# AIML-IfI/openset-imagenet

Hardware: AMD Instinct MI355X
Metric: images/sec (whole node) ResNet-50 + entropic-open-set, Protocol 2, 1/2/4/8 GPUs (higher is better)
Workload: dtype f32; 1 GPU; Protocol 2, ResNet-50, entropic open-set loss, batch 128/GPU; workload_key=p2, classes=30, batch_per_gpu=128, global_batch=128, image=3x224x224, loss=entropic, optimizer=adam lr=1e-3, parallelism=dp1

## Files before the change

__graft_entry__.py:

```python
import os
import subprocess
import sys

ROOT = os.path.dirname(os.path.abspath(__file__))
PKG = os.path.join(ROOT, "openset-imagenet_amd")
CSRC = os.path.join(PKG, "csrc")
for p in (ROOT, PKG):
    if p not in sys.path:
        sys.path.insert(0, p)


def build():
    subprocess.run(["make", "-C", CSRC, "-j8"], check=True)
    import openset_imagenet
    from openset_imagenet import _native
    lib = _native.lib()
    assert lib.osi_build_arch() == b"gfx950"
    assert lib.osi_abi_version() >= 7
    ops = _native.ops()
    assert hasattr(ops, "resnet50_forward") and hasattr(ops, "loss_fwd_bwd") and hasattr(ops, "adam_step") and hasattr(ops, "resnet50_grads_ready")
    assert hasattr(lib, "osi_conv_fwd_epilogue") and hasattr(lib, "osi_bn_eval_coeffs_multi")
    assert hasattr(ops, "resnet50_backward_adv") and hasattr(ops, "grad_accumulate") and hasattr(lib, "osi_stem_dgrad_fgsm")
    assert hasattr(ops, "adam_step_groups") and hasattr(ops, "sgd_step_groups") and hasattr(lib, "osi_adam_step_groups")
    assert hasattr(ops, "resnet50_forward_frozen") and hasattr(lib, "osi_conv_dgrad_fused_frozen") and hasattr(lib, "osi_bn_backward_frozen")
    assert lib.osi_abi_version() >= 13 and hasattr(lib, "osi_resnet50_set_trainable") and hasattr(lib, "osi_resnet50_tensor_unit")
    assert lib.osi_abi_version() >= 16 and hasattr(lib, "osi_auc_binary_f32") and hasattr(lib, "osi_auc_ovr_f32")
    assert lib.osi_abi_version() >= 17 and hasattr(lib, "osi_grad_clip_scale") and hasattr(ops, "grad_clip_scale")
    assert hasattr(ops, "adam_step_groups_dev") and hasattr(ops, "sgd_step_groups_dev")
    assert lib.osi_abi_version() >= 18 and hasattr(lib, "osi_eval_values_f32") and hasattr(lib, "osi_hist_f32")
    assert lib.osi_abi_version() >= 19 and hasattr(lib, "osi_stem_dgrad_pgd") and hasattr(ops, "resnet50_backward_attack")
    assert lib.osi_abi_version() >= 20 and hasattr(lib, "osi_average_update") and hasattr(lib, "osi_resnet50_set_bn_momentum")
    assert hasattr(ops, "average_update") and hasattr(ops, "resnet50_set_bn_momentum")
    assert lib.osi_abi_version() >= 21 and hasattr(lib, "osi_openmax_fit_tails") and hasattr(ops, "openmax_recalibrate")
    assert lib.osi_abi_version() >= 22 and hasattr(lib, "osi_evm_distances") and hasattr(ops, "evm_probs")
    assert lib.osi_abi_version() >= 23 and hasattr(lib, "osi_mix_rows_pairs") and hasattr(ops, "proser_loss_fwd_bwd")
    assert lib.osi_abi_version() >= 24 and hasattr(lib, "osi_knn_topk") and hasattr(ops, "knn_class_kth")
    assert lib.osi_abi_version() >= 25 and hasattr(lib, "osi_maha_scatter") and hasattr(ops, "maha_factor")
    assert lib.osi_abi_version() >= 26 and hasattr(lib, "osi_eigh_sweep") and hasattr(ops, "vim_scores")
    assert lib.osi_abi_version() >= 27 and hasattr(lib, "osi_shape_rows") and hasattr(ops, "order_stats") and hasattr(ops, "resnet50_pooled")


def smoke():
    import torch
    from openset_imagenet import ResNet50, EntropicOpensetLoss, optim, tools
    from oracle import resnet50_oracle as R, losses_oracle as L
    tools.set_device_gpu(0)
    torch.manual_seed(0)
    B, HW, C = 8, 96, 10
    model = tools.device(ResNet50(C, C, False))
    sd = {k: v.detach().cpu().clone() for k, v in model.state_dict().items()}
    x = torch.rand(B, 3, HW, HW)
    y = torch.tensor([0, -1, 3, 9, -1, 5, 2, 7])
    opt = optim.Adam(model.parameters(), lr=1e-3)
    model.train()
    opt.zero_grad()
    logits, feats = model(tools.device(x))
    j = EntropicOpensetLoss(C, 1.0)(logits, tools.device(y))
    j.backward()
    ref_logits, ref_feats, ref_loss, _ = R.forward_backward({k: v.clone() for k, v in sd.items()}, x, y,
                                                            lambda lg, t, f: L.entropic_openset_loss(lg, t, 1.0))
    sys.path.insert(0, os.path.join(ROOT, "tests"))
    from osi_testlib import hip_gates
    gates = hip_gates(model)
    sd64 = {k: (v.double() if v.is_floating_point() else v.clone()) for k, v in sd.items()}
    _, _, _, g64 = R.forward_backward(sd64, x.double(), y, lambda lg, t, f: L.entropic_openset_loss(lg, t, 1.0), gates=gates)
    opt.step()
    torch.cuda.synchronize()
    err = float((logits.detach().cpu() - ref_logits).abs().max())
    lerr = abs(float(j.detach()) - float(ref_loss))
    named = dict(model.named_parameters())
    gerr = max(float((named[k].grad.cpu().double() - g).norm() / (g.norm() + 1e-30)) for k, g in g64.items())
    print(f"smoke: max|dlogit|={err:.2e} |dloss|={lerr:.2e} max rel-L2 gradient error over {len(g64)} tensors (pinned gates)={gerr:.2e}")
    assert err < 1e-4 and lerr < 1e-4 and gerr < 5e-4, "HIP path disagrees with the CPU oracle"
    sd2 = {k: v.detach().cpu().clone() for k, v in model.state_dict().items()}
    model.eval()
    with torch.no_grad():
        lg_e, _ = model(tools.device(x))
    ref_e, _ = R.forward({k: (v.double() if v.is_floating_point() else v.clone()) for k, v in sd2.items()}, x.double(), False)
    eerr = float((lg_e.cpu().double() - ref_e).abs().max())
    print(f"smoke: inference forward max|dlogit|={eerr:.2e} (|logit| <= {float(ref_e.abs().max()):.2f})")
    assert eerr < 1e-4 * max(1.0, float(ref_e.abs().max())), "inference forward disagrees with the CPU oracle"


if __name__ == "__main__":
    build()
    print("build ok")
```

include/osi.h:

```cpp
#ifndef OSI_H
#define OSI_H

#include <stddef.h>

#ifdef __cplusplus
extern "C" {
#endif

#define OSI_OK 0
#define OSI_ERR_ARG (-1)
#define OSI_ERR_LAUNCH (-2)
#define OSI_ERR_STATE (-3)

typedef void* osi_stream_t;

int osi_abi_version(void);
const char* osi_build_arch(void);
const char* osi_strerror(int code);
int osi_set_tuning(const char* name, int value);
int osi_get_tuning(const char* name, int* value);
int osi_tuning_info(int i, const char** name, int* def, int* lo, int* hi, int* plan_relevant);

typedef struct {
    int B, H, W, Cin;
    int Ho, Wo, Cout;
    int R, S, stride, pad;
} osi_conv_desc;

enum { OSI_TILE_AUTO = 0, OSI_TILE_128x128 = 1, OSI_TILE_128x64 = 2, OSI_TILE_64x128 = 3, OSI_TILE_64x64 = 4,
       OSI_TILE_64x64_S1 = 5, OSI_TILE_64x128_S1 = 6, OSI_TILE_128x128_S1 = 7, OSI_TILE_128x64_S1 = 8  };

int osi_conv_fwd(const osi_conv_desc* d, const float* x, const float* w, float* y, int tile, osi_stream_t stream);
size_t osi_conv_fwd_bnstats_workspace(const osi_conv_desc* d);
int osi_conv_fwd_bnstats(const osi_conv_desc* d, const float* x, const float* w, float* y, int tile, float* pstats,
                         size_t pstats_bytes, int* P, int* rows_per_block, osi_stream_t stream);
int osi_conv_fwd_act(const osi_conv_desc* d, const float* x, const float* in_scale, const float* in_shift, const float* w, float* y,
                     int tile, float* pstats, size_t pstats_bytes, int* P, int* rows_per_block, osi_stream_t stream);
int osi_conv_fwd_act2(const osi_conv_desc* d, const float* x, const float* in_scale, const float* in_shift, const float* res,
                      const float* w, float* y, int tile, float* pstats, size_t pstats_bytes, int* P, int* rows_per_block,
                      osi_stream_t stream);
int osi_conv_wino_eligible(const osi_conv_desc* d, int input_gradient);
size_t osi_conv_wino_workspace(const osi_conv_desc* d);
size_t osi_conv_wino_weights_bytes(const osi_conv_desc* d);
size_t osi_conv_wino_slab_bytes(void);
int osi_conv_wino_transform_weights(const osi_conv_desc* d, const float* w, int input_gradient, float* u, size_t u_bytes, osi_stream_t stream);
int osi_conv_fwd_wino_pre(const osi_conv_desc* d, const float* x, const float* in_scale, const float* in_shift, const float* u, float* y,
                          void* slab, size_t slab_bytes, float* pstats, size_t pstats_bytes, int* P, int* rows_per_block, osi_stream_t stream);
int osi_conv_fwd_wino(const osi_conv_desc* d, const float* x, const float* in_scale, const float* in_shift, const float* w, float* y,
                      void* ws, size_t ws_bytes, float* pstats, size_t pstats_bytes, int* P, int* rows_per_block, osi_stream_t stream);
typedef struct {
    const float* scale;
    const float* shift;
    const float* residual;
    int relu;
} osi_conv_epilogue;
size_t osi_conv_fwd_epilogue_workspace(const osi_conv_desc* d);
int osi_conv_fwd_epilogue(const osi_conv_desc* d, const float* x, const float* w, float* out, const osi_conv_epilogue* e, void* ws,
                          size_t ws_bytes, osi_stream_t stream);
int osi_conv_fwd_wino_epilogue_pre(const osi_conv_desc* d, const float* x, const float* u, float* out, const osi_conv_epilogue* e, void* slab,
                                   size_t slab_bytes, osi_stream_t stream);
int osi_conv_dgrad(const osi_conv_desc* d, const float* dy, const float* w, float* dx, int accumulate, int tile,
                   osi_stream_t stream);
typedef struct {
    const void* relu_mask;
    const float* y0;
    const float* mean0;
    const float* invstd0;
    const float* y1;
    const float* mean1;
    const float* invstd1;
    float* partials;
    size_t partials_bytes;
    const float* scale0;
    const float* shift0;
    const void* pool_idx;
    int pool_H, pool_W;
    int addend_stride;
} osi_dgrad_fusion;
size_t osi_conv_dgrad_fused_workspace(const osi_conv_desc* d);
int osi_conv_dgrad_fused(const osi_conv_desc* d, const float* dy, const float* w, float* dx, const float* addend,
                         const osi_dgrad_fusion* f, int tile, int* P, osi_stream_t stream);
int osi_conv_dgrad_fused_frozen(const osi_conv_desc* d, const float* dy, const float* w, float* dx, const osi_dgrad_fusion* f, int tile,
                                int* P, osi_stream_t stream);
int osi_conv_dgrad_fused_wino(const osi_conv_desc* d, const float* dy, const float* w, float* dx, const osi_dgrad_fusion* f, void* ws,
                              size_t ws_bytes, int* P, osi_stream_t stream);
int osi_conv_dgrad_fused_wino_pre(const osi_conv_desc* d, const float* dy, const float* u, float* dx, const osi_dgrad_fusion* f, void* slab,
                                  size_t slab_bytes, int* P, osi_stream_t stream);
size_t osi_conv_wgrad_workspace(const osi_conv_desc* d);
int osi_conv_wgrad(const osi_conv_desc* d, const float* dy, const float* x, float* dw, void* ws, size_t ws_bytes,
                   osi_stream_t stream);
int osi_conv_wgrad_act(const osi_conv_desc* d, const float* dy, const float* x, const float* in_scale, const float* in_shift, float* dw,
                       void* ws, size_t ws_bytes, osi_stream_t stream);
size_t osi_conv_wgrad_wino_workspace(const osi_conv_desc* d);
int osi_conv_wgrad_wino(const osi_conv_desc* d, const float* dy, const float* x, const float* in_scale, const float* in_shift, float* dw,
                        void* ws, size_t ws_bytes, osi_stream_t stream);
int osi_stem_weight_pack(const float* w_krsc3, float* w_packed, int Cout, osi_stream_t stream);
size_t osi_stem_wgrad_direct_workspace(const osi_conv_desc* d);
int osi_stem_wgrad_direct(const osi_conv_desc* d, const float* dy, const float* x4, float* dw_krsc3, void* ws, size_t ws_bytes,
                          osi_stream_t stream);
size_t osi_stem_wgrad_fused_workspace(const osi_conv_desc* d);
int osi_stem_wgrad_fused(const osi_conv_desc* d, const float* gpool, const void* pool_idx, const float* y, const float* x4,
                         const float* gamma, const float* mean, const float* invstd, const float* dgamma, const float* dbeta,
                         float* dw_krsc3, void* ws, size_t ws_bytes, osi_stream_t stream);
int osi_stem_grad_unpack(const float* g_packed, float* g_krsc3, int Cout, osi_stream_t stream);
int osi_stem_dgrad(const float* dy, const float* w_krsc3, float* dx_nchw, int B, int H, int W, osi_stream_t stream);
int osi_stem_dgrad_fgsm(const float* dy, const float* w_krsc3, const float* x_nhwc4, float* x_adv_nhwc4, float eps, float lo, float hi,
                        int B, int H, int W, osi_stream_t stream);
int osi_stem_dgrad_pgd(const float* dy, const float* w_krsc3, const float* x_cur_nhwc4, const float* x_anchor_nhwc4, float* x_next_nhwc4,
                       float alpha, float eps, float lo, float hi, int B, int H, int W, osi_stream_t stream);

size_t osi_bn_workspace(int M, int C);
int osi_bn_train_stats(const float* y, int M, int C, const float* gamma, const float* beta, float eps, float momentum,
                       float* running_mean, float* running_var, float* mean, float* invstd, float* scale, float* shift,
                       void* ws, size_t ws_bytes, osi_stream_t stream);
int osi_bn_finalize_stats(float* pstats, size_t pstats_bytes, int P, int rows_per_block, int M, int C, const float* gamma,
                          const float* beta, float eps, float momentum, float* running_mean, float* running_var, float* mean,
                          float* invstd, float* scale, float* shift, osi_stream_t stream);
int osi_bn_eval_coeffs(const float* running_mean, const float* running_var, const float* gamma, const float* beta, float eps,
                       int C, float* scale, float* shift, osi_stream_t stream);
#define OSI_BN_MULTI_MAX 64
typedef struct {
    const float *running_mean, *running_var, *gamma, *beta;
    float *scale, *shift;
    int C;
} osi_bn_eval_layer;
int osi_bn_eval_coeffs_multi(const osi_bn_eval_layer* layers, int n, float eps, osi_stream_t stream);
#define OSI_BN_FROZEN_MAX 54
typedef struct {
    const float *running_mean, *running_var, *gamma, *beta;
    float *scale, *shift, *mean, *invstd;
    int C;
} osi_bn_frozen_layer;
int osi_bn_frozen_coeffs_multi(const osi_bn_frozen_layer* layers, int n, float eps, osi_stream_t stream);
int osi_bn_apply(const float* y, const float* residual, const float* scale, const float* shift, float* out, int M, int C,
                 int relu, osi_stream_t stream);
size_t osi_bn_backward_workspace(int M, int C);
int osi_bn_backward(const float* dout, const float* act, const float* y, const float* mean, const float* invstd,
                    const float* gamma, float* dy, float* gmasked, float* dgamma, float* dbeta, int M, int C, void* ws,
                    size_t ws_bytes, osi_stream_t stream);

size_t osi_bn_relu_mask_bytes(int M, int C);
int osi_bn_apply_relu_mask(const float* y, const float* residual, const float* scale, const float* shift, float* out,
                           void* relu_mask, int M, int C, osi_stream_t stream);
int osi_bn_apply_relu_mask2(const float* y, const float* scale, const float* shift, const float* res_y, const float* res_scale,
                            const float* res_shift, float* out, void* relu_mask, int M, int C, osi_stream_t stream);
int osi_bn_backward_relu_mask(const float* dout, const void* relu_mask, const float* y, const float* mean, const float* invstd,
                              const float* gamma, float* dy, float* gmasked, float* dgamma, float* dbeta, int M, int C, void* ws,
                              size_t ws_bytes, osi_stream_t stream);

int osi_bn_backward_fused(const float* g, const float* y, const float* mean, const float* invstd, const float* gamma,
                          const float* psum_g, const float* psum_gx, int P, float* dy, float* dgamma, float* dbeta, int M, int C,
                          void* ws, size_t ws_bytes, osi_stream_t stream);

typedef struct {
    const float *y, *mean, *invstd, *gamma;
    const float* psum_gx;
    float* dy;
    float *dgamma, *dbeta;
} osi_bn_fused_consumer;
size_t osi_bn_backward_fused2_workspace(int C);
int osi_bn_backward_fused2(const float* g, const osi_bn_fused_consumer* consumers, const float* psum_g, int P, int M, int C, void* ws,
                           size_t ws_bytes, osi_stream_t stream);

typedef struct {
    const float *y, *mean, *invstd;
    const float* scale;
    float* dy;
    float *dgamma, *dbeta;
} osi_bn_frozen_consumer;
int osi_bn_backward_frozen(const float* dout, const void* relu_mask, const osi_bn_frozen_consumer* consumers, int n, float* gmasked, int M,
                           int C, void* ws, size_t ws_bytes, osi_stream_t stream);

int osi_nchw3_to_nhwc4(const float* x_nchw, float* y_nhwc4, int B, int H, int W, osi_stream_t stream);
int osi_u8hwc3_to_nhwc4(const unsigned char* x_u8_nhwc, const unsigned char* flip, float* y_nhwc4, int B, int H, int W,
                        osi_stream_t stream);
// ... 275 lines not shown
```

openset-imagenet_amd/csrc/abi.hip:

```cpp
#include "osi_common.h"

#include <cstring>

OsiTuning g_osi_tuning;

namespace {
struct Knob { const char* name; int OsiTuning::*slot; int def, lo, hi, plan; };
const Knob kKnobs[] = {
#define OSI_KNOB_ROW(name, def, lo, hi, plan) {#name, &OsiTuning::name, def, lo, hi, plan},
    OSI_TUNING_KNOBS(OSI_KNOB_ROW)
#undef OSI_KNOB_ROW
};
const int kNumKnobs = (int)(sizeof(kKnobs) / sizeof(kKnobs[0]));
const Knob* find_knob(const char* name) {
    if (!name) return nullptr;
    for (const Knob& k : kKnobs)
        if (!strcmp(name, k.name)) return &k;
    return nullptr;
}
}

extern "C" {
int osi_abi_version(void) { return 27; }
int osi_set_tuning(const char* name, int value) {
    const Knob* k = find_knob(name);
    if (!k) return OSI_ERR_ARG;
    if (value < k->lo || value > k->hi) return OSI_ERR_ARG;
    if (k->slot == &OsiTuning::wgrad_tile && value != 0 && value != 64) return OSI_ERR_ARG;
    g_osi_tuning.*(k->slot) = value;
    return OSI_OK;
}
int osi_get_tuning(const char* name, int* value) {
    const Knob* k = find_knob(name);
    if (!k || !value) return OSI_ERR_ARG;
    *value = g_osi_tuning.*(k->slot);
    return OSI_OK;
}
int osi_tuning_info(int i, const char** name, int* def, int* lo, int* hi, int* plan_relevant) {
    if (i < 0 || i >= kNumKnobs) return OSI_ERR_ARG;
    const Knob& k = kKnobs[i];
    if (name) *name = k.name;
    if (def) *def = k.def;
    if (lo) *lo = k.lo;
    if (hi) *hi = k.hi;
    if (plan_relevant) *plan_relevant = k.plan;
    return OSI_OK;
}
const char* osi_build_arch(void) { return "gfx950"; }
const char* osi_strerror(int code) {
    switch (code) {
        case OSI_OK: return "ok";
        case OSI_ERR_ARG: return "invalid argument (shape, pointer or alignment precondition)";
        case OSI_ERR_LAUNCH: return "HIP launch failed";
        case OSI_ERR_STATE: return "executor called out of order, or a plan-relevant tuning knob changed after osi_resnet50_create";
        default: return "unknown error";
    }
}
}
```

openset-imagenet_amd/csrc/bn.hip:

```cpp
#include "osi_common.h"

namespace {

constexpr int NT = 256;

struct RowSplit { int CV, RL, G; };
__host__ __device__ inline RowSplit row_split(int C) {
    RowSplit s;
    int c4 = C / 4;
    s.CV = c4 < NT ? c4 : NT;
    s.RL = NT / s.CV;
    s.G = (c4 + s.CV - 1) / s.CV;
    return s;
}

__global__ __launch_bounds__(NT) void k_bn_stats_partial(const float* __restrict__ y, int M, int C, int rows_per_blk,
                                                        float* __restrict__ pmean, float* __restrict__ pm2) {
    const int P = gridDim.x;
    __shared__ f32x4 red[2][NT];
    const RowSplit sp = row_split(C);
    const int tid = threadIdx.x;
    const int cv = tid % sp.CV, rl = tid / sp.CV;
    const int r0 = blockIdx.x * rows_per_blk;
    const int r1 = min(M, r0 + rows_per_blk);
    const float n = (float)(r1 - r0);
    const bool active = rl < sp.RL;
    for (int g = 0; g < sp.G; ++g) {
        const int c4 = g * sp.CV + cv;
        const bool colok = active && c4 * 4 < C;
        f32x4 s1 = {0, 0, 0, 0}, s2 = {0, 0, 0, 0}, shift = {0, 0, 0, 0};
        if (colok) {
            const f32x4* base = reinterpret_cast<const f32x4*>(y) + c4;
            const size_t ld = C / 4;
            shift = base[(size_t)r0 * ld];
            int r = r0 + rl;
            for (; r + 3 * sp.RL < r1; r += 4 * sp.RL) {
                f32x4 v0 = base[(size_t)r * ld], v1 = base[(size_t)(r + sp.RL) * ld];
                f32x4 v2 = base[(size_t)(r + 2 * sp.RL) * ld], v3 = base[(size_t)(r + 3 * sp.RL) * ld];
                v0 -= shift; v1 -= shift; v2 -= shift; v3 -= shift;
                s1 += (v0 + v1) + (v2 + v3);
                s2 += (v0 * v0 + v1 * v1) + (v2 * v2 + v3 * v3);
            }
            for (; r < r1; r += sp.RL) {
                f32x4 v = base[(size_t)r * ld] - shift;
                s1 += v; s2 += v * v;
            }
        }
        red[0][tid] = s1; red[1][tid] = s2;
        __syncthreads();
        if (colok && rl == 0) {
            for (int k = 1; k < sp.RL; ++k) { s1 += red[0][k * sp.CV + cv]; s2 += red[1][k * sp.CV + cv]; }
            f32x4 mean = shift + s1 / n;
            f32x4 m2 = s2 - s1 * s1 / n;
#pragma unroll
            for (int k = 0; k < 4; ++k) {
                pmean[(size_t)(c4 * 4 + k) * P + blockIdx.x] = mean[k];
                pm2[(size_t)(c4 * 4 + k) * P + blockIdx.x] = m2[k];
            }
        }
        __syncthreads();
    }
}

__device__ __forceinline__ void bn_finish(int c, float mean, float m2, int M, const float* gamma, const float* beta, float eps,
                                          float momentum, float* running_mean, float* running_var, float* mean_out,
                                          float* invstd_out, float* scale_out, float* shift_out) {
    float var = m2 / (float)M;
    float invstd = 1.0f / sqrtf(var + eps);
    mean_out[c] = mean; invstd_out[c] = invstd;
    float sc = invstd * gamma[c];
    scale_out[c] = sc; shift_out[c] = beta[c] - mean * sc;
    if (running_mean) {
        float unb = M > 1 ? m2 / (float)(M - 1) : var;
        running_mean[c] = (1.f - momentum) * running_mean[c] + momentum * mean;
        running_var[c] = (1.f - momentum) * running_var[c] + momentum * unb;
    }
}
__global__ __launch_bounds__(NT) void k_bn_stats_final_rows(const float* __restrict__ pmean, const float* __restrict__ pm2, int P,
                                                           int rows_per_blk, int M, int C, const float* __restrict__ gamma,
                                                           const float* __restrict__ beta, float eps, float momentum,
                                                           float* running_mean, float* running_var, float* __restrict__ mean_out,
                                                           float* __restrict__ invstd_out, float* __restrict__ scale_out,
                                                           float* __restrict__ shift_out) {
// ... 418 lines not shown
    }
}

struct BwdCoef { f32x4 mu, is, c1, c2, gis; };
__device__ __forceinline__ BwdCoef bwd_coef(const f32x4* __restrict__ mean, const f32x4* __restrict__ invstd, const f32x4* __restrict__ gamma,
                                            const f32x4* __restrict__ c1, const f32x4* __restrict__ c2, int c4) {
    BwdCoef k;
    k.mu = mean[c4]; k.is = invstd[c4]; k.c1 = c1[c4]; k.c2 = c2[c4];
    k.gis = gamma[c4] * k.is;
    return k;
}
__device__ __forceinline__ f32x4 bwd_elem(f32x4 gv, f32x4 yv, const BwdCoef& k) {
    const f32x4 xh = (yv - k.mu) * k.is;
    return (gv - k.c1 - xh * k.c2) * k.gis;
}
template <int MODE, bool EMITG, int GEO>
__global__ __launch_bounds__(NT) void k_bn_bwd_apply(const f32x4* dA , const void* __restrict__ msk,
                                                    const f32x4* __restrict__ y, const f32x4* __restrict__ mean,
                                                    const f32x4* __restrict__ invstd, const f32x4* __restrict__ gamma,
                                                    const f32x4* __restrict__ c1, const f32x4* __restrict__ c2,
                                                    f32x4* dy, f32x4* __restrict__ gout, size_t n4, int c4n, PoolSrc ps) {
    const size_t nq = (n4 + NT - 1) / NT;
    const int tid = threadIdx.x;
    BwdCoef k0 = {}, k1 = {};
    if (GEO == 1) k0 = bwd_coef(mean, invstd, gamma, c1, c2, tid % c4n);
    if (GEO == 2) { k0 = bwd_coef(mean, invstd, gamma, c1, c2, tid); k1 = bwd_coef(mean, invstd, gamma, c1, c2, NT + tid); }
    for (size_t q = blockIdx.x; q < nq; q += gridDim.x) {
        const size_t t = (OSI_BN_REVERSE & 2) ? nq - 1 - q : q;
        const size_t i = t * NT + tid;
        if (i >= n4) continue;
        const int c4 = GEO == 1 ? tid % c4n : GEO == 2 ? (int)(t & 1) * NT + tid : (int)(i % (size_t)c4n);
        f32x4 gv = MODE == 3 ? pool_gather(dA, ps, (uint32_t)(i / (size_t)c4n), c4, c4n) : masked<MODE>(__builtin_nontemporal_load(dA + i), msk, i);
        const BwdCoef k = GEO == 1 ? k0 : GEO == 2 ? ((t & 1) ? k1 : k0) : bwd_coef(mean, invstd, gamma, c1, c2, c4);
        f32x4 r = bwd_elem(gv, __builtin_nontemporal_load(y + i), k);
        if (EMITG) gout[i] = gv;
        dy[i] = r;
    }
}

struct BwdApplyCons { const f32x4 *y, *mean, *invstd, *gamma, *c1, *c2; f32x4* dy; };
template <int GEO>
__global__ __launch_bounds__(NT) void k_bn_bwd_apply2(const f32x4* g, BwdApplyCons a, BwdApplyCons b, size_t n4, int c4n) {
    const size_t nq = (n4 + NT - 1) / NT;
    const int tid = threadIdx.x;
    const size_t tfirst = (OSI_BN_REVERSE & 2) ? nq - 1 - blockIdx.x : blockIdx.x;
    const int ck = GEO == 1 ? tid % c4n : (int)(tfirst & 1) * NT + tid;
    BwdCoef a0 = {}, b0 = {};
    if (GEO != 0) { a0 = bwd_coef(a.mean, a.invstd, a.gamma, a.c1, a.c2, ck); b0 = bwd_coef(b.mean, b.invstd, b.gamma, b.c1, b.c2, ck); }
    for (size_t q = blockIdx.x; q < nq; q += gridDim.x) {
        const size_t t = (OSI_BN_REVERSE & 2) ? nq - 1 - q : q;
        const size_t i = t * NT + tid;
        if (i >= n4) continue;
        const f32x4 gv = __builtin_nontemporal_load(g + i);
        const f32x4 ya = __builtin_nontemporal_load(a.y + i), yb = __builtin_nontemporal_load(b.y + i);
        const BwdCoef ka = GEO != 0 ? a0 : bwd_coef(a.mean, a.invstd, a.gamma, a.c1, a.c2, (int)(i % (size_t)c4n));
        const BwdCoef kb = GEO != 0 ? b0 : bwd_coef(b.mean, b.invstd, b.gamma, b.c1, b.c2, (int)(i % (size_t)c4n));
        const f32x4 ra = bwd_elem(gv, ya, ka), rb = bwd_elem(gv, yb, kb);
        b.dy[i] = rb;
        a.dy[i] = ra;
    }
}

template <int MODE, bool EMITG, bool TWO, int GEO>
__global__ __launch_bounds__(NT) void k_bn_frozen_apply(const f32x4* dA, const void* __restrict__ msk, const f32x4* __restrict__ scale0,
                                                       const f32x4* __restrict__ scale1, f32x4* dy0, f32x4* __restrict__ dy1,
                                                       f32x4* __restrict__ gout, size_t n4, int c4n, PoolSrc ps) {
    const size_t nq = (n4 + NT - 1) / NT;
    const int tid = threadIdx.x;
    f32x4 s00 = {}, s01 = {}, s10 = {}, s11 = {};
    if (GEO == 1) { s00 = scale0[tid % c4n]; if (TWO) s10 = scale1[tid % c4n]; }
    if (GEO == 2) { s00 = scale0[tid]; s01 = scale0[NT + tid]; if (TWO) { s10 = scale1[tid]; s11 = scale1[NT + tid]; } }
    for (size_t q = blockIdx.x; q < nq; q += gridDim.x) {
        const size_t t = (OSI_BN_REVERSE & 2) ? nq - 1 - q : q;
        const size_t i = t * NT + tid;
        if (i >= n4) continue;
        const int c4 = GEO == 1 ? tid % c4n : GEO == 2 ? (int)(t & 1) * NT + tid : (int)(i % (size_t)c4n);
        const f32x4 gv = MODE == 3 ? pool_gather(dA, ps, (uint32_t)(i / (size_t)c4n), c4, c4n) : masked<MODE>(__builtin_nontemporal_load(dA + i), msk, i);
        if (EMITG) gout[i] = gv;
        if (TWO) dy1[i] = gv * (GEO == 1 ? s10 : GEO == 2 ? ((t & 1) ? s11 : s10) : scale1[c4]);
        dy0[i] = gv * (GEO == 1 ? s00 : GEO == 2 ? ((t & 1) ? s01 : s00) : scale0[c4]);
    }
}

static int stream_geo(int c4n) { return NT % c4n == 0 ? 1 : c4n == 2 * NT ? 2 : 0; }

static int rows_per_block(int M, int C, int& P) {
    long rows = (256l * 1024) / ((long)C * 4);
    if (rows < 8) rows = 8;
    long minrows = (M + 1023) / 1024;
    if (rows < minrows) rows = minrows;
    if (rows > M) rows = M;
    P = (int)((M + rows - 1) / rows);
    return (int)rows;
}
static int stream_grid(size_t n4, bool backward = false) {
    const size_t cap = (size_t)(backward ? g_osi_tuning.bn_grid_bwd : g_osi_tuning.bn_grid);
    size_t g = (n4 + NT - 1) / NT;
    return (int)(g > cap ? cap : g);
}

static void bwd_groups(int P, int& S, int& Pc) {
    S = osi_cdiv(P, 64);
    if (S > OSI_BN_GROUPS) S = OSI_BN_GROUPS;
    Pc = osi_cdiv(P, S);
    S = osi_cdiv(P, Pc);
}
struct BwdWs { float *a, *b, *c1, *c2; };
static size_t ws_floats(int rows, int C, bool coef = true) { return (size_t)2 * rows * C + (coef ? 2 * (size_t)C : 0); }
static BwdWs carve_ws(void* ws, int rows, int C) {
    float* a = (float*)ws;
    const size_t n = (size_t)rows * C;
    return BwdWs{a, a + n, a + 2 * n, a + 2 * n + C};
}
static PoolSrc make_pool_src(const void* idx, int H, int W) {
    PoolSrc ps;
    ps.idx = (const uint32_t*)idx;
    ps.dW = make_fastdiv((uint32_t)W); ps.dH = make_fastdiv((uint32_t)H);
    ps.H = H; ps.W = W; ps.Ho = (H + 2 - 3) / 2 + 1; ps.Wo = (W + 2 - 3) / 2 + 1;
    return ps;
}

}

extern "C" {

size_t osi_bn_workspace(int M, int C) {
    if (M <= 0 || C <= 0) return 0;
    int P;
    rows_per_block(M, C, P);
    return ws_floats(P, C, false) * sizeof(float);
}

int osi_bn_train_stats(const float* y, int M, int C, const float* gamma, const float* beta, float eps, float momentum,
                       float* running_mean, float* running_var, float* mean, float* invstd, float* scale, float* shift,
                       void* ws, size_t ws_bytes, osi_stream_t stream) {
    OSI_REQUIRE(y && gamma && beta && mean && invstd && scale && shift && ws);
    OSI_REQUIRE(M > 0 && C > 0 && C % 4 == 0);
    OSI_REQUIRE((running_mean == nullptr) == (running_var == nullptr));
    int P;
    int rpb = rows_per_block(M, C, P);
    OSI_REQUIRE(ws_bytes >= ws_floats(P, C, false) * sizeof(float));
    hipStream_t st = (hipStream_t)stream;
    float* pmean = (float*)ws;
    float* pm2 = pmean + (size_t)P * C;
    hipLaunchKernelGGL(k_bn_stats_partial, dim3(P), dim3(NT), 0, st, y, M, C, rpb, pmean, pm2);
    OSI_LAUNCH_CHECK();
    hipLaunchKernelGGL(k_bn_stats_final, dim3(osi_cdiv(C, NT / 64)), dim3(NT), 0, st, pmean, pm2, P, rpb, M, C, gamma, beta, eps,
                       momentum, running_mean, running_var, mean, invstd, scale, shift);
    OSI_LAUNCH_CHECK();
    return OSI_OK;
}

int osi_bn_finalize_stats(float* pstats, size_t pstats_bytes, int P, int rows_per_block, int M, int C, const float* gamma,
                          const float* beta, float eps, float momentum, float* running_mean, float* running_var, float* mean,
                          float* invstd, float* scale, float* shift, osi_stream_t stream) {
    OSI_REQUIRE(pstats && gamma && beta && mean && invstd && scale && shift);
    OSI_REQUIRE(P > 0 && rows_per_block > 0 && M > 0 && C > 0 && (long)(P - 1) * rows_per_block < M && (long)P * rows_per_block >= M);
    OSI_REQUIRE((running_mean == nullptr) == (running_var == nullptr));
    OSI_REQUIRE(pstats_bytes >= bn_pstats_floats(P, C) * sizeof(float));
    hipStream_t st = (hipStream_t)stream;
    const float* pmean = pstats;
    const float* pm2 = pstats + (size_t)P * C;
    if (P <= g_osi_tuning.bn_single_p) {
        hipLaunchKernelGGL(k_bn_stats_final_rows, dim3(osi_cdiv(C, 16)), dim3(NT), 0, st, pmean, pm2, P, rows_per_block, M, C, gamma,
                           beta, eps, momentum, running_mean, running_var, mean, invstd, scale, shift);
        OSI_LAUNCH_CHECK();
// ... 106 lines not shown
    OSI_REQUIRE(relu_mask && res_y && res_scale && res_shift);
    return bn_apply_impl(y, res_y, scale, shift, out, relu_mask, M, C, 1, (hipStream_t)stream, res_scale, res_shift);
}

static BwdConsTable one_cons(const float* pa, const float* pb, float* ga, float* gb, float* dgamma, float* dbeta, float* c1, float* c2) {
    BwdConsTable t{};
    t.k[0] = BwdCons{pa, pb, ga, gb, dgamma, dbeta, c1, c2};
    return t;
}

static int launch_bwd_partial(int mode, const float* dout, const void* msk, const float* y, const float* mean, const float* invstd, float* dgamma,
                              float* dbeta, int M, int C, int rpb, int P, const BwdWs& w, const PoolSrc& ps, hipStream_t st) {
    if (int e = pick<0, 1, 2, 3>(mode, [&](auto MODE) -> int {
            hipLaunchKernelGGL(k_bn_bwd_partial<decltype(MODE)::value>, dim3(P), dim3(NT), 0, st, dout, msk, y, mean, invstd, M, C, rpb, w.a, w.b, ps);
            OSI_LAUNCH_CHECK();
            return OSI_OK;
        })) return e;
    hipLaunchKernelGGL(k_bn_bwd_final, dim3(osi_cdiv(C, NT / 64)), dim3(NT), 0, st, one_cons(w.a, w.b, nullptr, nullptr, dgamma, dbeta, w.c1, w.c2), false, P, M, C);
    OSI_LAUNCH_CHECK();
    return OSI_OK;
}
static int launch_bwd_apply(int mode, const float* dout, const void* msk, const float* y, const float* mean, const float* invstd, const float* gamma,
                            const BwdWs& w, float* dy, float* gmasked, int M, int C, const PoolSrc& ps, hipStream_t st) {
    const size_t n4 = (size_t)M * C / 4;
    const int grid = stream_grid(n4, true), c4n = C / 4;
    auto go = [&](auto MODE, auto EMITG, auto GEO) -> int {
        constexpr int md = decltype(MODE)::value, geo = decltype(GEO)::value;
        constexpr bool emit = decltype(EMITG)::value != 0;
        if constexpr (md != 3 || (geo == 0 && !emit)) {
            hipLaunchKernelGGL((k_bn_bwd_apply<md, emit, geo>), dim3(grid), dim3(NT), 0, st, (const f32x4*)dout, msk, (const f32x4*)y, (const f32x4*)mean,
                               (const f32x4*)invstd, (const f32x4*)gamma, (const f32x4*)w.c1, (const f32x4*)w.c2, (f32x4*)dy, (f32x4*)gmasked, n4, c4n, ps);
            OSI_LAUNCH_CHECK();
            return OSI_OK;
        } else return OSI_ERR_ARG;
    };
    return pick<0, 1, 2, 3>(mode, [&](auto MODE) {
        return pick<0, 1>(gmasked && mode != 3, [&](auto EMITG) {
            return pick<0, 1, 2>(mode == 3 ? 0 : stream_geo(c4n), [&](auto GEO) { return go(MODE, EMITG, GEO); });
        });
    });
}

static int bn_backward_impl(const float* dout, const void* msk, int mode, const float* y, const float* mean, const float* invstd,
                            const float* gamma, float* dy, float* gmasked, float* dgamma, float* dbeta, int M, int C, void* ws,
                            size_t ws_bytes, hipStream_t st, PoolSrc ps = PoolSrc{}) {
    OSI_REQUIRE(dout && y && mean && invstd && gamma && (dy || mode == 3) && dgamma && dbeta && ws);
    OSI_REQUIRE(M > 0 && C > 0 && C % 4 == 0);
    int P;
    const int rpb = rows_per_block(M, C, P);
    OSI_REQUIRE(ws_bytes >= ws_floats(P, C) * sizeof(float));
    const BwdWs w = carve_ws(ws, P, C);
    if (int e = launch_bwd_partial(mode, dout, msk, y, mean, invstd, dgamma, dbeta, M, C, rpb, P, w, ps, st)) return e;
    if (!dy) return OSI_OK;
    return launch_bwd_apply(mode, dout, msk, y, mean, invstd, gamma, w, dy, gmasked, M, C, ps, st);
}

static int bwd_reduce_partials(const BwdConsTable& t, int n, int P, int M, int C, int S, int Pc, hipStream_t st) {
    if (P <= g_osi_tuning.bn_wide_p) {
        hipLaunchKernelGGL(k_bn_bwd_final_wide, dim3(osi_cdiv(C, 16), n), dim3(16 * WPL), 0, st, t, P, M, C);
        OSI_LAUNCH_CHECK();
        return OSI_OK;
    }
    hipLaunchKernelGGL(k_colsum2_group, dim3(osi_cdiv(C, 16), S, n), dim3(NT), 0, st, t, P, Pc, C, S);
    OSI_LAUNCH_CHECK();
    hipLaunchKernelGGL(k_bn_bwd_final, dim3(osi_cdiv(C, NT / 64), n), dim3(NT), 0, st, t, true, S, M, C);
    OSI_LAUNCH_CHECK();
    return OSI_OK;
}

int osi_bn_backward_fused(const float* g, const float* y, const float* mean, const float* invstd, const float* gamma,
                          const float* psum_g, const float* psum_gx, int P, float* dy, float* dgamma, float* dbeta, int M, int C,
                          void* ws, size_t ws_bytes, osi_stream_t stream) {
    OSI_REQUIRE(g && y && mean && invstd && gamma && psum_g && psum_gx && dy && dgamma && dbeta && ws);
    OSI_REQUIRE(M > 0 && C > 0 && C % 4 == 0 && P > 0);
    int S, Pc;
    bwd_groups(P, S, Pc);
    OSI_REQUIRE(ws_bytes >= ws_floats(S, C) * sizeof(float));
    hipStream_t st = (hipStream_t)stream;
    const BwdWs w = carve_ws(ws, S, C);
    if (int e = bwd_reduce_partials(one_cons(psum_g, psum_gx, w.a, w.b, dgamma, dbeta, w.c1, w.c2), 1, P, M, C, S, Pc, st)) return e;
    return launch_bwd_apply(0, g, nullptr, y, mean, invstd, gamma, w, dy, nullptr, M, C, PoolSrc{}, st);
}

size_t osi_bn_backward_fused2_workspace(int C) {
    if (C <= 0) return 0;
    return 2 * ws_floats(OSI_BN_GROUPS, C) * sizeof(float);
}

int osi_bn_backward_fused2(const float* g, const osi_bn_fused_consumer* consumers, const float* psum_g, int P, int M, int C, void* ws,
                           size_t ws_bytes, osi_stream_t stream) {
    OSI_REQUIRE(g && consumers && psum_g && ws && M > 0 && C > 0 && C % 4 == 0 && P > 0);
    for (int k = 0; k < 2; ++k) {
        const osi_bn_fused_consumer& c = consumers[k];
        OSI_REQUIRE(c.y && c.mean && c.invstd && c.gamma && c.psum_gx && c.dy && c.dgamma && c.dbeta);
    }
    OSI_REQUIRE(consumers[1].dy != consumers[0].dy && consumers[1].dy != g);
    OSI_REQUIRE(ws_bytes >= osi_bn_backward_fused2_workspace(C));
    int S, Pc;
    bwd_groups(P, S, Pc);
    hipStream_t st = (hipStream_t)stream;
    const size_t per = ws_floats(OSI_BN_GROUPS, C);
    BwdConsTable t{};
    BwdApplyCons a[2];
    for (int k = 0; k < 2; ++k) {
        const osi_bn_fused_consumer& c = consumers[k];
        const BwdWs w = carve_ws((float*)ws + k * per, S, C);
        t.k[k] = BwdCons{psum_g, c.psum_gx, w.a, w.b, c.dgamma, c.dbeta, w.c1, w.c2};
        a[k] = BwdApplyCons{(const f32x4*)c.y, (const f32x4*)c.mean, (const f32x4*)c.invstd, (const f32x4*)c.gamma, (const f32x4*)w.c1,
                            (const f32x4*)w.c2, (f32x4*)c.dy};
    }
    if (int e = bwd_reduce_partials(t, 2, P, M, C, S, Pc, st)) return e;
    const size_t n4 = (size_t)M * C / 4;
    const int c4n = C / 4;
    const int grid = stream_grid(n4, true);
    int geo = stream_geo(c4n);
    if (geo == 2 && (grid & 1) && (size_t)grid < (n4 + NT - 1) / NT) geo = 0;
    return pick<0, 1, 2>(geo, [&](auto GEO) -> int {
        hipLaunchKernelGGL((k_bn_bwd_apply2<decltype(GEO)::value>), dim3(grid), dim3(NT), 0, st, (const f32x4*)g, a[0], a[1], n4, c4n);
        OSI_LAUNCH_CHECK();
        return OSI_OK;
    });
}

int osi_bn_backward_reduce(const float* psum_g, const float* psum_gx, int P, float* dgamma, float* dbeta, int M, int C, void* ws,
                           size_t ws_bytes, osi_stream_t stream) {
    OSI_REQUIRE(psum_g && psum_gx && dgamma && dbeta && ws && M > 0 && C > 0 && P > 0);
    int S, Pc;
    bwd_groups(P, S, Pc);
    OSI_REQUIRE(ws_bytes >= ws_floats(S, C) * sizeof(float));
    const BwdWs w = carve_ws(ws, S, C);
    return bwd_reduce_partials(one_cons(psum_g, psum_gx, w.a, w.b, dgamma, dbeta, w.c1, w.c2), 1, P, M, C, S, Pc, (hipStream_t)stream);
}

static int bn_frozen_impl(const float* dout, const void* msk, int mode, const osi_bn_frozen_consumer* cs, int n, float* gmasked, int M, int C,
                          void* ws, size_t ws_bytes, hipStream_t st, PoolSrc ps = PoolSrc{}) {
    OSI_REQUIRE(dout && cs && (n == 1 || n == 2) && M > 0 && C > 0 && C % 4 == 0);
    OSI_REQUIRE(mode != 3 || (n == 1 && !gmasked));
    for (int k = 0; k < n; ++k) {
        OSI_REQUIRE(cs[k].scale && cs[k].dy && (cs[k].dgamma == nullptr) == (cs[k].dbeta == nullptr));
        if (cs[k].dgamma) {
            int P;
            rows_per_block(M, C, P);
            OSI_REQUIRE(cs[k].y && cs[k].mean && cs[k].invstd && ws && ws_bytes >= ws_floats(P, C) * sizeof(float));
        }
    }
    OSI_REQUIRE(n == 1 || (cs[1].dy != cs[0].dy && cs[1].dy != dout));
    for (int k = 0; k < n; ++k) {
        if (!cs[k].dgamma) continue;
        int P;
        const int rpb = rows_per_block(M, C, P);
        if (int e = launch_bwd_partial(mode, dout, msk, cs[k].y, cs[k].mean, cs[k].invstd, cs[k].dgamma, cs[k].dbeta, M, C, rpb, P, carve_ws(ws, P, C),
                                       ps, st)) return e;
    }
    const size_t n4 = (size_t)M * C / 4;
    const int grid = stream_grid(n4, true), c4n = C / 4;
    auto D = (const f32x4*)dout; auto S0 = (const f32x4*)cs[0].scale; auto S1 = (const f32x4*)(n == 2 ? cs[1].scale : nullptr);
    auto DY0 = (f32x4*)cs[0].dy; auto DY1 = (f32x4*)(n == 2 ? cs[1].dy : nullptr); auto GO = (f32x4*)gmasked;
    auto go = [&](auto MODE, auto EMITG, auto TWO, auto GEO) -> int {
        constexpr int md = decltype(MODE)::value, geo = decltype(GEO)::value;
        constexpr bool emit = decltype(EMITG)::value != 0, two = decltype(TWO)::value != 0;
        if constexpr (md != 3 || (geo == 0 && !emit && !two)) {
            hipLaunchKernelGGL((k_bn_frozen_apply<md, emit, two, geo>), dim3(grid), dim3(NT), 0, st, D, msk, S0, S1, DY0, DY1, GO, n4, c4n, ps);
            OSI_LAUNCH_CHECK();
            return OSI_OK;
        } else return OSI_ERR_ARG;
    };
// ... 54 lines not shown
```

openset-imagenet_amd/csrc/conv_common.h:

```cpp
#pragma once
#include "osi_common.h"

namespace osi_conv {

__device__ __forceinline__ f32x4 ld4(const float* p) { return *reinterpret_cast<const f32x4*>(p); }

constexpr uint32_t OOB = 0x80000000u;
__device__ __forceinline__ __amdgpu_buffer_rsrc_t make_rsrc(const float* p, int bytes) {
    return __builtin_amdgcn_make_buffer_rsrc((void*)p, 0, bytes, 0x00020000);
}
__device__ __forceinline__ f32x4 bld4(__amdgpu_buffer_rsrc_t r, uint32_t voff, uint32_t soff) {
    return __builtin_bit_cast(f32x4, __builtin_amdgcn_raw_buffer_load_b128(r, voff, soff, 0));
}
typedef uint32_t u32x4 __attribute__((ext_vector_type(4)));
__device__ __forceinline__ u32x4 bld4u(__amdgpu_buffer_rsrc_t r, uint32_t voff, uint32_t soff) {
    return __builtin_bit_cast(u32x4, __builtin_amdgcn_raw_buffer_load_b128(r, voff, soff, 0));
}
__device__ __forceinline__ void bst4(__amdgpu_buffer_rsrc_t r, f32x4 v, uint32_t voff, uint32_t soff) {
    __builtin_amdgcn_raw_buffer_store_b128(__builtin_bit_cast(u32x4, v), r, voff, soff, 0);
}
typedef float f32x3 __attribute__((ext_vector_type(3)));
typedef float f32x4acc __attribute__((ext_vector_type(4)));
__device__ __forceinline__ f32x3 bld3(__amdgpu_buffer_rsrc_t r, uint32_t voff, uint32_t soff) {
    return __builtin_bit_cast(f32x3, __builtin_amdgcn_raw_buffer_load_b96(r, voff, soff, 0));
}

__device__ __forceinline__ int acc_row(int r, int lane) { return (r & 3) + 8 * (r >> 2) + 4 * (lane >> 5); }


int hw_cus();
int chip_cus();
bool conv_desc_ok(const osi_conv_desc* d);
bool conv_is_stem(const osi_conv_desc* d);
int launch_slab_reduce(const float* slab, float* out, size_t n4, size_t stride4, int splits, hipStream_t st);
bool stem_direct_geometry(const osi_conv_desc* d);
int launch_stem_fwd_direct(const osi_conv_desc* d, const float* x4, const float* wpacked, float* y, float* pmean, float* pm2, int ntiles,
                           hipStream_t st);
constexpr int STEM_TILE_PIXELS = 128;

}
```

openset-imagenet_amd/csrc/conv_igemm.hip:

```cpp
#include "conv_common.h"
#include <algorithm>
#include <type_traits>

using namespace osi_conv;

namespace {

constexpr int BK = 32;
constexpr int LDR = BK + 4;

struct ConvP {
    const float* x;
    const float* w;
    float* y;
    int B, H, W, Cin, Ho, Wo, Cout, R, S, stride, pad;
    int M;
    int Ktot;
    int MT, NT;
    int accumulate;
    int x_bytes, w_bytes;
    FastDiv dHoWo, dWo;
    FastDiv cHW[4], cW[4];
    int unit;
    float* pmean;
    float* pm2;
    const float* addend;
    const unsigned long long* ebits;
    const float* ey0;
    const float* ey1;
    const float *emean0, *einv0, *emean1, *einv1;
    const float *escale0, *eshift0;
    int skip_empty;
    int eadd_even;
    const uint32_t* epool;
    int epH, epW;
    float* esum;
    int eP;
    int kchunk;
    int wtbl;
    int wgroup, splits;
    int gkind, gkeys, ginner;
    const float* in_scale;
    const float* in_shift;
    const float* res;
    const float* osc;
    const float* osh;
    const float* ores;
    int orelu;
    size_t slab_stride;
    int MT1, g1, ks_S, ks_T;
    float* ks_slab;
#ifdef OSI_STAMPS
    unsigned long long* stamps;
#endif
};

#ifdef OSI_STAMPS
#define OSI_STAMP(p, idx, slot)                                                                                        \
    do {                                                                                                               \
        if (threadIdx.x == 0 && (p).stamps) (p).stamps[(size_t)(idx) * 8 + (slot)] = __builtin_amdgcn_s_memrealtime(); \
    } while (0)
#define OSI_STAMP_ID(p, idx)                                                                   \
    do {                                                                                       \
        if (threadIdx.x == 0 && (p).stamps) {                                                  \
            (p).stamps[(size_t)(idx) * 8 + 4] = __builtin_amdgcn_s_getreg(63492);   \
            (p).stamps[(size_t)(idx) * 8 + 5] = __builtin_amdgcn_s_getreg(63508);  \
        }                                                                                      \
    } while (0)
unsigned long long* g_osi_stamps = nullptr;
#else
#define OSI_STAMP(p, idx, slot) do {} while (0)
#define OSI_STAMP_ID(p, idx) do {} while (0)
#endif

__device__ __forceinline__ bool tile_of_block(int bid, int MT, int NT, int& mt, int& nt) {
    int xcd = bid & 7, slot = bid >> 3;
    nt = slot % NT;
    mt = (slot / NT) * 8 + xcd;
    return mt < MT;
}

__device__ __forceinline__ bool tile_of_block_split(const ConvP& p, int bid, int& mt, int& nt, int& ks) {
    ks = -1;
    if (p.ks_S <= 1) return tile_of_block(bid, p.MT, p.NT, mt, nt);
    if (bid < p.g1) return tile_of_block(bid, p.MT1, p.NT, mt, nt);
    const int pb = bid - p.g1;
    const int xcd = pb & 7, slot = pb >> 3;
    nt = slot % p.NT;
    const int key = (slot / p.NT) * 8 + xcd;
    const int mt2 = key / p.ks_S;
    ks = key - mt2 * p.ks_S;
    mt = p.MT1 + mt2;
    return mt < p.MT;
}

#ifndef OSI_ABLATE
#define OSI_ABLATE 0
#endif

template <int WM, int WN, int J0 = 0, int J1 = 4>
__device__ __forceinline__ void mma_RR(const float* sA, const float* sB, int arow, int brow, int lane,
                                       f32x16 (&acc)[WM][WN]) {
    const int h4 = (lane >> 5) * 4, l31 = lane & 31;
#pragma unroll
    for (int j = J0; j < J1; ++j) {
        f32x4 a[WM], b[WN];
#pragma unroll
        for (int i = 0; i < WM; ++i) a[i] = *reinterpret_cast<const f32x4*>(sA + (arow + i * 32 + l31) * LDR + 8 * j + h4);
#pragma unroll
        for (int i = 0; i < WN; ++i) b[i] = *reinterpret_cast<const f32x4*>(sB + (brow + i * 32 + l31) * LDR + 8 * j + h4);
#pragma unroll
        for (int e = 0; e < 4; ++e)
#pragma unroll
            for (int i = 0; i < WM; ++i)
#pragma unroll
                for (int n = 0; n < WN; ++n)
                    acc[i][n] = __builtin_amdgcn_mfma_f32_32x32x2f32(a[i][e], b[n][e], acc[i][n], 0, 0, 0);
    }
}
template <int WM, int WN, int LDC>
__device__ __forceinline__ void mma_RC(const float* sA, const float* sB, int arow, int bcol, int lane,
                                       f32x16 (&acc)[WM][WN]) {
    const int h4 = (lane >> 5) * 4, l31 = lane & 31;
#pragma unroll
    for (int j = 0; j < 4; ++j) {
        f32x4 a[WM];
#pragma unroll
        for (int i = 0; i < WM; ++i) a[i] = *reinterpret_cast<const f32x4*>(sA + (arow + i * 32 + l31) * LDR + 8 * j + h4);
#pragma unroll
        for (int e = 0; e < 4; ++e) {
            float b[WN];
#pragma unroll
            for (int n = 0; n < WN; ++n) b[n] = sB[(8 * j + h4 + e) * LDC + bcol + n * 32 + l31];
#pragma unroll
            for (int i = 0; i < WM; ++i)
#pragma unroll
                for (int n = 0; n < WN; ++n)
                    acc[i][n] = __builtin_amdgcn_mfma_f32_32x32x2f32(a[i][e], b[n], acc[i][n], 0, 0, 0);
        }
    }
}
template <int WM, int WN, int LDA, int LDB, int K0 = 0, int K1 = BK / 2>
__device__ __forceinline__ void mma_CC(const float* sA, const float* sB, int acol, int bcol, int lane,
                                       f32x16 (&acc)[WM][WN]) {
    static_assert(WM <= 2 && WN <= 2 && LDA % 2 == 0 && LDB % 2 == 0, "interleaved pairs");
    const int h = lane >> 5, l31 = lane & 31;
    const float* pa = sA + h * LDA + acol + (WM == 2 ? 2 * l31 : l31);
    const float* pb = sB + h * LDB + bcol + (WN == 2 ? 2 * l31 : l31);
#pragma unroll
    for (int ks = K0; ks < K1; ++ks) {
        float a[WM], b[WN];
        if constexpr (WM == 2) { const f32x2 v = *reinterpret_cast<const f32x2*>(pa + 2 * ks * LDA); a[0] = v[0]; a[1] = v[1]; }
        else a[0] = pa[2 * ks * LDA];
        if constexpr (WN == 2) { const f32x2 v = *reinterpret_cast<const f32x2*>(pb + 2 * ks * LDB); b[0] = v[0]; b[1] = v[1]; }
        else b[0] = pb[2 * ks * LDB];
#pragma unroll
        for (int i = 0; i < WM; ++i)
#pragma unroll
            for (int n = 0; n < WN; ++n)
                acc[i][n] = __builtin_amdgcn_mfma_f32_32x32x2f32(a[i], b[n], acc[i][n], 0, 0, 0);
    }
}

constexpr int LDT = 64 + 4;

template <bool LIVE = false>
__device__ __forceinline__ void tile64_to_lds(float* tile, const f32x16& acc, int wm, int wn, int lane, int m0 = 0, int M = 0) {
#pragma unroll
    for (int rr = 0; rr < 16; ++rr) {
        const bool live = !LIVE || m0 + wm * 32 + acc_row(rr, lane) < M;
        tile[(wm * 32 + acc_row(rr, lane)) * LDT + wn * 32 + (lane & 31)] = live ? acc[rr] : 0.f;
    }
}
__device__ __forceinline__ void tile64_to_slab(const ConvP& p, const float* tile, int mt, int nt, int ks) {
    float* dst = p.ks_slab + ((size_t)((mt - p.MT1) * p.NT + nt) * p.ks_S + ks) * 4096;
    const int tid = threadIdx.x, c4 = tid & 15, rg = tid >> 4;
#pragma unroll
    for (int k = 0; k < 4; ++k) {
        const int rl = rg + 16 * k;
        *reinterpret_cast<f32x4*>(dst + rl * 64 + c4 * 4) = *reinterpret_cast<const f32x4*>(tile + rl * LDT + c4 * 4);
    }
}
template <typename RD>
__device__ __forceinline__ void fwd_store64(const ConvP& p, int m0, int n0, bool oe, RD rd) {
    const int tid = threadIdx.x, c4 = tid & 15, rg = tid >> 4;
    float* const y = p.y + n0 + c4 * 4;
    if (oe) {
        const __amdgpu_buffer_rsrc_t ro = make_rsrc(p.ores ? p.ores : p.y, p.ores ? p.M * p.Cout * 4 : 0);
        const f32x4 sc = ld4(p.osc + n0 + c4 * 4), sh = ld4(p.osh + n0 + c4 * 4);
        f32x4 rv[4];
#pragma unroll
        for (int k = 0; k < 4; ++k) {
            const int m = m0 + rg + 16 * k;
            rv[k] = bld4(ro, m < p.M ? (uint32_t)((m * p.Cout + n0 + c4 * 4) * 4) : OOB, 0);
        }
#pragma unroll
        for (int k = 0; k < 4; ++k) {
            const int rl = rg + 16 * k, m = m0 + rl;
            const f32x4 a = rd(rl, c4);
            f32x4 v;
#pragma unroll
            for (int e = 0; e < 4; ++e) { const float t = __builtin_fmaf(a[e], sc[e], sh[e]) + rv[k][e]; v[e] = p.orelu ? osi_relu(t) : t; }
            if (m < p.M) *reinterpret_cast<f32x4*>(y + (size_t)m * p.Cout) = v;
        }
    } else {
#pragma unroll
        for (int k = 0; k < 4; ++k) {
            const int rl = rg + 16 * k, m = m0 + rl;
            if (m < p.M) *reinterpret_cast<f32x4*>(y + (size_t)m * p.Cout) = rd(rl, c4);
        }
    }
}

struct BnPart { float cnt, mu, q; };
template <bool FULL>
__device__ __forceinline__ BnPart bn_block32(const f32x16& acc, int row0, int M, int lane) {
    const float cnt = FULL ? 32.f : (float)min(32, max(0, M - row0));
    float s = 0.f;
#pragma unroll
    for (int rr = 0; rr < 16; ++rr) s += (FULL || row0 + acc_row(rr, lane) < M) ? acc[rr] : 0.f;
    s += __shfl_xor(s, 32, 64);
    const float mu = cnt > 0.f ? s / cnt : 0.f;
    float q = 0.f;
#pragma unroll
    for (int rr = 0; rr < 16; ++rr) {
        const float dlt = acc[rr] - mu;
        if constexpr (FULL) q = __builtin_fmaf(dlt, dlt, q);
        else q += (row0 + acc_row(rr, lane) < M) ? dlt * dlt : 0.f;
    }
    q += __shfl_xor(q, 32, 64);
    return {cnt, mu, q};
}
__device__ __forceinline__ void bn_put(float* st, int slot, float cnt, float mu, float q) {
    float* dst = st + slot * 3;
    dst[0] = cnt; dst[1] = mu; dst[2] = q;
}
template <int BN>
__device__ __forceinline__ void bn_merge_rows(const ConvP& p, const float* st, int mt, int n0) {
    const int tid = threadIdx.x;
    if (tid < BN) {
        const float* a = st + tid * 3;
        const float* b = st + (BN + tid) * 3;
        float cn = a[0], cm = a[1], cs = a[2];
        chan_merge(cn, cm, cs, b[0], b[1], b[2]);
        p.pmean[(size_t)mt * p.Cout + n0 + tid] = cm;
        p.pm2[(size_t)mt * p.Cout + n0 + tid] = cs;
    }
}

__device__ __forceinline__ void load_in_tables(const ConvP& p, float* s_sc, float* s_sh) {
    const int tid = threadIdx.x;
    for (int c = tid * 4; c < p.Cin; c += 1024) {
        *reinterpret_cast<f32x4*>(s_sc + c) = ld4(p.in_scale + c);
        *reinterpret_cast<f32x4*>(s_sh + c) = ld4(p.in_shift + c);
// ... 369 lines not shown
            s0 += (v * (y0v[k] - mu0)) * is0;
            if constexpr (FUSED == 4) v *= gsc;
            bst4(r_out, v, offb[k], 0);
        }
    } else {
        const __amdgpu_buffer_rsrc_t r_add = make_rsrc(p.addend, (USE_ADD && p.addend) ? FULL : 0);
        const __amdgpu_buffer_rsrc_t r_bits = make_rsrc(reinterpret_cast<const float*>(p.ebits), has_bits ? FULL : 0);
        const __amdgpu_buffer_rsrc_t r_y1 = make_rsrc(p.ey1, has_y1 ? FULL : 0);
#pragma unroll
        for (int k = 0; k < 4; ++k) {
            const int rl = rg + 16 * k;
            f32x4 v = rd(rl, c4);
            const uint32_t apix = (uint32_t)(m0 + rl), ab = fdiv(apix, dHW), arem = apix - ab * dHW.d, ah = fdiv(arem, dW), aw = arem - ah * dW.d;
            const uint32_t aoff = (((ah | aw) & (uint32_t)p.eadd_even) != 0u) ? OOB : offb[k];
            v += bld4(r_add, aoff, 0);
            if constexpr (FUSED && POOL) {
                if (offb[k] != OOB) {
                    const uint32_t pix = pixv[k], off = offb[k] >> 2;
                    const uint32_t bb = fdiv(pix, dHW), rem = pix - bb * dHW.d, ho = fdiv(rem, dW), wo = rem - ho * dW.d;
                    const uint32_t idw = p.epool[off >> 2];
#pragma unroll
                    for (int e = 0; e < 4; ++e) {
                        const uint32_t byte = (idw >> (8 * e)) & 0xffu, t = byte & 0x7fu, r = t / 3u, sx = t - 3u * r;
                        const uint32_t apix = (bb * p.epH + 2u * ho - 1u + r) * p.epW + 2u * wo - 1u + sx;
                        const float gv = (byte & 0x80u) ? v[e] : 0.f;
                        sg[e] += gv;
                        s0[e] += (gv * (p.ey0[(size_t)apix * p.Cin + col + e] - mu0[e])) * is0[e];
                    }
                }
            } else if constexpr (FUSED != 0) {
                const uint32_t i4 = offb[k] >> 4, bit = i4 & 63u;
                const uint32_t boff = offb[k] != OOB ? (i4 >> 6) * 32u + (bit >> 5) * 4u : OOB;
                uint32_t wb[4];
#pragma unroll
                for (int e = 0; e < 4; ++e) wb[e] = __builtin_amdgcn_raw_buffer_load_b32(r_bits, boff, 8 * e, 0);
                const f32x4 y0v = bld4(r_y0, offb[k], 0), y1v = bld4(r_y1, offb[k], 0);
#pragma unroll
                for (int e = 0; e < 4; ++e) {
                    const bool keep = (((wb[e] >> (bit & 31u)) & 1u) != 0) | !has_bits;
                    const bool open = !USE_GATE || (__builtin_fmaf(y0v[e], gsc[e], gsh[e]) > 0.f) | !has_gate;
                    v[e] = (keep & open) ? v[e] : 0.f;
                }
                sg += v;
                s0 += (v * (y0v - mu0)) * is0;
                s1 += v * y1v;
            }
            bst4(r_out, v, offb[k], 0);
            if (FUSED == 1) __builtin_amdgcn_sched_barrier(0);
        }
        if (USE_Y1) {
            const uint32_t cb = (uint32_t)col * 4u;
            const f32x4 mu1 = bld4(make_rsrc(p.emean1, has_y1 ? FULL : 0), cb, 0), is1 = bld4(make_rsrc(p.einv1, has_y1 ? FULL : 0), cb, 0);
            s1 = (s1 - mu1 * sg) * is1;
        }
    }
    if (FUSED && p.esum) {
#pragma unroll
        for (int e = 0; e < 4; ++e) {
            sg[e] += __shfl_xor(sg[e], 16, 64); s0[e] += __shfl_xor(s0[e], 16, 64); s1[e] += __shfl_xor(s1[e], 16, 64);
            sg[e] += __shfl_xor(sg[e], 32, 64); s0[e] += __shfl_xor(s0[e], 32, 64); s1[e] += __shfl_xor(s1[e], 32, 64);
        }
        __syncthreads();
        if (lane < 16) {
#pragma unroll
            for (int e = 0; e < 4; ++e) {
                float* dst = smem + (wave * BN + c4 * 4 + e) * 3;
                dst[0] = sg[e]; dst[1] = s0[e]; dst[2] = s1[e];
            }
        }
        __syncthreads();
        if (tid < BN) {
            float a0 = 0.f, a1 = 0.f, a2 = 0.f;
#pragma unroll
            for (int wv = 0; wv < 4; ++wv) { const float* s = smem + (wv * BN + tid) * 3; a0 += s[0]; a1 += s[1]; a2 += s[2]; }
            const size_t prow = (size_t)(cls * p.MT + mt) * p.Cin + n0 + tid;
            const size_t pstride = (size_t)p.eP * p.Cin;
            p.esum[prow] = a0;
            p.esum[pstride + prow] = a1;
            if (p.ey1) p.esum[2 * pstride + prow] = a2;
        }
    }
}

template <int WM, int WN, int NST, int FUSED, bool KS = false, bool POOL = false, bool W3 = false>
__global__ __launch_bounds__(256, NST == 1 ? (WM * WN >= 4 ? 3 : (WM * WN == 1 ? 8 : 4)) : 2) void k_conv_dgrad(ConvP p, int Hc0, int Wc0) {
    static_assert(!KS || (WM == 1 && WN == 1 && NST == 1), "the K-split tail is built for the single-buffered 64x64 tile");
    static_assert(!W3 || (WM == 1 && WN == 1 && NST == 1 && !POOL), "row windows: the single-buffered 64x64 tile");
    constexpr int BM = 64 * WM, BN = 64 * WN;
    constexpr int AROWS = W3 ? W3_WROWS : BM;
    constexpr int AR = W3 ? 3 : BM / 32;
    constexpr int LDC = BN + 4;
    constexpr int BV = BN / 4;
    constexpr int BRP = 256 / BV;
    constexpr int BRN = BK / BRP;
    constexpr int STAGE = AROWS * LDR + BK * LDC;
    extern __shared__ __attribute__((aligned(16))) float smem[];
#ifdef OSI_STAMPS
    const size_t sidx = (size_t)blockIdx.y * gridDim.x + blockIdx.x;
#endif
    OSI_STAMP(p, sidx, 0); OSI_STAMP_ID(p, sidx);

    int mt, nt, ks = -1;
    if (KS) { if (!tile_of_block_split(p, blockIdx.x, mt, nt, ks)) return; }
    else if (!tile_of_block(blockIdx.x, p.MT, p.NT, mt, nt)) return;
    const int st = p.stride;
    const int cls = blockIdx.y, ph = cls / st, pw = cls - ph * st;
    const int Hc = (p.H - ph + st - 1) / st, Wc = (p.W - pw + st - 1) / st;
    const int Mc = p.B * Hc * Wc;
    const int tid = threadIdx.x, lane = tid & 63, wave = tid >> 6;
    const int wm = wave >> 1, wn = wave & 1;
    const int m0 = mt * BM, n0 = nt * BN;
    if (m0 >= Mc) {
        if (p.esum && tid < BN) {
            const size_t prow = (size_t)(cls * p.MT + mt) * p.Cin + n0 + tid, pstride = (size_t)p.eP * p.Cin;
            p.esum[prow] = 0.f; p.esum[pstride + prow] = 0.f;
            if (p.ey1) p.esum[2 * pstride + prow] = 0.f;
        }
        return;
    }
    const int kq = tid & 7, lr = tid >> 3;

    const int rb = (ph + p.pad) % st, sb = (pw + p.pad) % st;
    const int nR = rb < p.R ? (p.R - rb + st - 1) / st : 0;
    const int nS = sb < p.S ? (p.S - sb + st - 1) / st : 0;
    if (p.skip_empty && nR * nS == 0) return;

    const FastDiv dHW = p.cHW[cls], dW = p.cW[cls];
    int a_base[AR];
    unsigned a_taps[AR];
    bool a_ok[AR];
    const __amdgpu_buffer_rsrc_t rx = make_rsrc(p.x, p.x_bytes), rw = make_rsrc(p.w, p.w_bytes);
    if constexpr (W3) {
        w3_slots<2>(a_base, a_ok, m0, lr, kq, p.H, p.W, p.Cout, Mc, p.cW[1], dHW, dW);
#pragma unroll
        for (int i = 0; i < AR; ++i) a_taps[i] = 0;
    } else
#pragma unroll
    for (int i = 0; i < AR; ++i) {
        int m = m0 + lr + 32 * i;
        a_ok[i] = m < Mc;
        uint32_t mm = a_ok[i] ? (uint32_t)m : 0u;
        if (p.unit) {
            a_base[i] = a_ok[i] ? ((int)mm * p.Cout + kq * 4) * 4 : (int)OOB; a_taps[i] = a_ok[i] ? 1u : 0u;
        } else {
            uint32_t b = fdiv(mm, dHW);
            uint32_t rem = mm - b * dHW.d;
            uint32_t h2 = fdiv(rem, dW), w2 = rem - h2 * dW.d;
            const int hb = (ph + st * (int)h2 + p.pad - rb) / st, wb = (pw + st * (int)w2 + p.pad - sb) / st;
            a_base[i] = ((((int)b * p.Ho + hb) * p.Wo + wb) * p.Cout + kq * 4) * 4;
            a_taps[i] = 0;
            for (int j = 0; j < nR; ++j)
                for (int k = 0; k < nS; ++k)
                    if ((unsigned)(hb - j) < (unsigned)p.Ho && (unsigned)(wb - k) < (unsigned)p.Wo) a_taps[i] |= 1u << (j * nS + k);
            if (!a_ok[i]) a_taps[i] = 0;
        }
    }
    (void)Hc0; (void)Wc0;

    f32x16 acc[WM][WN];
#pragma unroll
    for (int i = 0; i < WM; ++i)
#pragma unroll
        for (int n = 0; n < WN; ++n)
#pragma unroll
            for (int r = 0; r < 16; ++r) acc[i][n][r] = 0.f;

    const int KC = p.Cout / BK;
    const int Tall = nR * nS * KC;
    const int t0 = (!KS || ks < 0) ? 0 : ks * p.ks_T;
    const int T = (!KS || ks < 0) ? Tall : min(Tall, t0 + p.ks_T);
    int jr = 0, js = 0, c0 = 0;
    if (KS && ks > 0) ksplit_start<W3>(t0, KC, nS, jr, js, c0);
    int cjs = js;
    bool ld_new = false, first = true;
    int prow = 0;
    if constexpr (W3) prow = w3_prow(m0, wm, lane, Mc, dW);
    f32x4 ra[AR], rbv[BRN];
    const int bk_row = tid / BV, bk_col = (tid % BV) * 4;

    auto gload = [&]() {
        const int r = rb + st * jr, s = sb + st * js;
        if constexpr (W3) {
            ld_new = js == 0 || first;
            first = false;
            if (ld_new) {
#pragma unroll
                for (int i = 0; i < AR; ++i) {
                    const bool ok = ((uint32_t)a_base[i] >> jr) & 1;
                    ra[i] = bld4(rx, ok ? (uint32_t)((a_base[i] & ~15) + ((1 - jr) * p.W * p.Cout + c0) * 4) : OOB, 0);
                }
            }
        } else
        if (p.unit) {
#pragma unroll
            for (int i = 0; i < AR; ++i) ra[i] = bld4(rx, (uint32_t)a_base[i], (uint32_t)(c0 * 4));
        } else {
#pragma unroll
            for (int i = 0; i < AR; ++i) {
                const bool ok = (a_taps[i] >> (jr * nS + js)) & 1;
                ra[i] = bld4(rx, ok ? (uint32_t)(a_base[i] + (c0 - (jr * p.Wo + js) * p.Cout) * 4) : OOB, 0);
            }
        }
        const uint32_t wsoff = (uint32_t)((c0 * p.Ktot + (r * p.S + s) * p.Cin) * 4);
#pragma unroll
        for (int i = 0; i < BRN; ++i)
            rbv[i] = bld4(rw, (uint32_t)(((bk_row + BRP * i) * p.Ktot + n0 + bk_col) * 4), wsoff);
    };
    auto advance = [&]() {
        if constexpr (W3) {
            if (++js == 3) { js = 0; c0 += BK; if (c0 == p.Cout) { c0 = 0; ++jr; } }
        } else {
            c0 += BK;
            if (c0 == p.Cout) { c0 = 0; if (++js == nS) { js = 0; ++jr; } }
        }
    };
    auto sstore = [&](int buf) {
        float* sA = smem + buf * STAGE;
        float* sB = sA + AROWS * LDR;
        if constexpr (W3) {
            if (ld_new) {
#pragma unroll
                for (int i = 0; i < AR; ++i)
                    if (lr + 32 * i < W3_WROWS) *reinterpret_cast<f32x4*>(sA + (lr + 32 * i) * LDR + kq * 4) = ra[i];
            }
        } else
#pragma unroll
        for (int i = 0; i < AR; ++i) *reinterpret_cast<f32x4*>(sA + (lr + 32 * i) * LDR + kq * 4) = ra[i];
#pragma unroll
        for (int i = 0; i < BRN; ++i) *reinterpret_cast<f32x4*>(sB + (bk_row + BRP * i) * LDC + bk_col) = rbv[i];
    };

    if (T > t0) {
        gload(); advance();
        sstore(0);
        __syncthreads();
        OSI_STAMP(p, sidx, 1);
            for (int t = t0; t < T; ++t) {
            const int buf = NST == 2 ? ((t - t0) & 1) : 0;
                if (!(OSI_ABLATE & 1)) if (t + 1 < T) { gload(); advance(); }
            const float* sA = smem + buf * STAGE;
            if (OSI_ABLATE & 16) {
#pragma unroll
                for (int j = 0; j < 16; ++j)
#pragma unroll
                    for (int i = 0; i < WM; ++i)
#pragma unroll
                        for (int n = 0; n < WN; ++n) acc[i][n] = __builtin_amdgcn_mfma_f32_32x32x2f32(ra[i % AR][j & 3], rbv[n % BRN][j & 3], acc[i][n], 0, 0, 0);
            } else if constexpr (W3) {
                const int h4 = (lane >> 5) * 4;
                const float* pa = sA + (prow + 2 - cjs) * LDR + h4;
                const float* pb = sA + AROWS * LDR + h4 * LDC + wn * 32 + (lane & 31);
#pragma unroll
                for (int j = 0; j < 4; ++j) {
                    const f32x4 a = *reinterpret_cast<const f32x4*>(pa + 8 * j);
#pragma unroll
                    for (int e = 0; e < 4; ++e) acc[0][0] = __builtin_amdgcn_mfma_f32_32x32x2f32(a[e], pb[(8 * j + e) * LDC], acc[0][0], 0, 0, 0);
                }
                if (++cjs == 3) cjs = 0;
            } else
            mma_RC<WM, WN, LDC>(sA, sA + BM * LDR, wm * 32 * WM, wn * 32 * WN, lane, acc);
            if (!(OSI_ABLATE & 4)) if (NST == 1) __syncthreads();
            if (!(OSI_ABLATE & 2)) if (t + 1 < T) sstore(NST == 2 ? (buf ^ 1) : 0);
            if (!(OSI_ABLATE & 4)) __syncthreads();
        }
        OSI_STAMP(p, sidx, 2);
    }
    if (OSI_ABLATE & 32) { if (acc[0][0][0] == 123.456f) p.y[tid] = acc[0][0][1]; return; }

    if constexpr (WM == 1 && WN == 1) {
        static_assert(BM * LDT <= STAGE, "transposed tile must fit the operand stage");
        float* tile = smem;
        tile64_to_lds<W3>(tile, acc[0][0], wm, wn, lane, m0, Mc);
        __syncthreads();
        if (KS && ks >= 0) {
            tile64_to_slab(p, tile, mt, nt, ks);
            OSI_STAMP(p, sidx, 3);
            return;
        }
        dgrad_epilogue64<FUSED, POOL>(p, smem, cls, mt, m0, n0, Mc, st, ph, pw, dHW, dW,
                                [&](int rl, int c4) { return *reinterpret_cast<const f32x4*>(tile + rl * LDT + c4 * 4); });
        OSI_STAMP(p, sidx, 3);
        return;
    }

    float esg[WN], es0[WN], es1[WN];
#pragma unroll
    for (int n = 0; n < WN; ++n) { esg[n] = 0.f; es0[n] = 0.f; es1[n] = 0.f; }
#pragma unroll
    for (int i = 0; i < WM; ++i) {
#pragma unroll
        for (int q = 0; q < 4; ++q) {
            uint32_t roff[4];
            bool rok[4];
#pragma unroll
            for (int e = 0; e < 4; ++e) {
                int m = m0 + wm * 32 * WM + i * 32 + acc_row(4 * q + e, lane);
                rok[e] = m < Mc;
                uint32_t mm = rok[e] ? (uint32_t)m : 0u;
                uint32_t pix;
                if (st == 1) pix = mm;
                else {
                    uint32_t b = fdiv(mm, dHW);
                    uint32_t rem = mm - b * dHW.d;
                    uint32_t h2 = fdiv(rem, dW), w2 = rem - h2 * dW.d;
                    pix = (b * p.H + (ph + st * h2)) * p.W + (pw + st * w2);
                }
                roff[e] = pix * p.Cin;
            }
#pragma unroll
            for (int n = 0; n < WN; ++n) {
                const int col = n0 + wn * 32 * WN + n * 32 + (lane & 31);
                float v[4];
#pragma unroll
                for (int e = 0; e < 4; ++e) v[e] = acc[i][n][4 * q + e];
                if (p.addend) {
#pragma unroll
                    for (int e = 0; e < 4; ++e) v[e] += rok[e] ? p.addend[roff[e] + col] : 0.f;
                }
                if (FUSED) {
                    if (p.ebits) {
#pragma unroll
                        for (int e = 0; e < 4; ++e) {
                            const uint32_t i4 = (roff[e] + col) >> 2;
                            const unsigned long long w = rok[e] ? p.ebits[(size_t)(i4 >> 6) * 4 + (col & 3)] : 0ull;
                            v[e] = (w >> (i4 & 63)) & 1 ? v[e] : 0.f;
                        }
                    }
                    if (p.escale0) {
                        const float gsc = p.escale0[col], gsh = p.eshift0[col];
#pragma unroll
                        for (int e = 0; e < 4; ++e)
                            v[e] = (rok[e] && __builtin_fmaf(p.ey0[roff[e] + col], gsc, gsh) > 0.f) ? v[e] : 0.f;
                    }
                    if (p.esum) {
                        const float mu0 = p.emean0[col], is0 = p.einv0[col];
#pragma unroll
                        for (int e = 0; e < 4; ++e) {
                            const float gv = rok[e] ? v[e] : 0.f;
                            esg[n] += gv;
                            es0[n] += gv * ((rok[e] ? p.ey0[roff[e] + col] : mu0) - mu0) * is0;
                        }
                        if (p.ey1) {
                            const float mu1 = p.emean1[col], is1 = p.einv1[col];
#pragma unroll
                            for (int e = 0; e < 4; ++e)
                                es1[n] += (rok[e] ? v[e] : 0.f) * ((rok[e] ? p.ey1[roff[e] + col] : mu1) - mu1) * is1;
                        }
                    }
                }
#pragma unroll
                for (int e = 0; e < 4; ++e)
                    if (rok[e]) p.y[roff[e] + col] = v[e];
            }
        }
// ... 539 lines not shown
            for (int k = 0; k < 4; ++k) t[j][k] = bld4(rs, off + (uint32_t)k * 4096u + (uint32_t)(s0 + j) * 16384u, 0);
#pragma unroll
        for (int j = 0; j < 4; ++j)
#pragma unroll
            for (int k = 0; k < 4; ++k) v[k] += t[j][k];
    }
    fwd_store64(p, m0, n0, p.osc != nullptr, [&](int rl, int) { return v[(rl - rg) >> 4]; });
    if (!p.pmean) return;
    const float cnt = (float)min(64, p.M - m0);
    f32x4 sm = {0, 0, 0, 0};
#pragma unroll
    for (int k = 0; k < 4; ++k) if (m0 + rg + 16 * k < p.M) sm += v[k];
#pragma unroll
    for (int e = 0; e < 4; ++e) red[rg][c4 * 4 + e] = sm[e];
    __syncthreads();
    if (tid < 64) {
        float a = 0.f;
#pragma unroll
        for (int g = 0; g < 16; ++g) a += red[g][tid];
        smean[tid] = a / cnt;
    }
    __syncthreads();
    const f32x4 mu = *reinterpret_cast<const f32x4*>(smean + c4 * 4);
    f32x4 q = {0, 0, 0, 0};
#pragma unroll
    for (int k = 0; k < 4; ++k) if (m0 + rg + 16 * k < p.M) { const f32x4 d = v[k] - mu; q += d * d; }
#pragma unroll
    for (int e = 0; e < 4; ++e) red[rg][c4 * 4 + e] = q[e];
    __syncthreads();
    if (tid < 64) {
        float a = 0.f;
#pragma unroll
        for (int g = 0; g < 16; ++g) a += red[g][tid];
        p.pmean[(size_t)mt * p.Cout + n0 + tid] = smean[tid];
        p.pm2[(size_t)mt * p.Cout + n0 + tid] = a;
    }
}

template <int FUSED>
__global__ __launch_bounds__(256) void k_conv_dgrad_tail_fixup(ConvP p) {
    __shared__ float red[4 * 64 * 3];
    const int tile = blockIdx.x;
    const int mt = p.MT1 + tile / p.NT, nt = tile - (tile / p.NT) * p.NT;
    const int nsp = p.ks_S;
    const __amdgpu_buffer_rsrc_t rs = make_rsrc(p.ks_slab + (size_t)tile * nsp * 4096, nsp * 16384);
    dgrad_epilogue64<FUSED, false>(p, red, 0, mt, mt * 64, nt * 64, p.B * p.H * p.W, 1, 0, 0, p.cHW[0], p.cW[0], [&](int rl, int c4) {
        const uint32_t off = (uint32_t)(rl * 64 + c4 * 4) * 4u;
        f32x4 a = bld4(rs, off, 0);
        for (int s0 = 1; s0 < nsp; s0 += 8) {
            f32x4 t[8];
#pragma unroll
            for (int j = 0; j < 8; ++j) t[j] = bld4(rs, off + (uint32_t)(s0 + j) * 16384u, 0);
#pragma unroll
            for (int j = 0; j < 8; ++j) a += t[j];
        }
        return a;
    });
}

__global__ __launch_bounds__(256) void k_slab_reduce(const float* slab, float* out, size_t n4, size_t stride4, int splits) {
    __shared__ f32x4 red[16][16];
    const int o = threadIdx.x & 15, l = threadIdx.x >> 4;
    const size_t i = (size_t)blockIdx.x * 16 + o;
    const f32x4* s = reinterpret_cast<const f32x4*>(slab);
    f32x4 a0 = {0, 0, 0, 0}, a1 = a0, a2 = a0, a3 = a0;
    if (i < n4) {
        int k = l;
        for (; k + 48 < splits; k += 64) {
            a0 += s[i + (size_t)k * stride4]; a1 += s[i + (size_t)(k + 16) * stride4];
            a2 += s[i + (size_t)(k + 32) * stride4]; a3 += s[i + (size_t)(k + 48) * stride4];
        }
        for (; k < splits; k += 16) a0 += s[i + (size_t)k * stride4];
    }
    red[l][o] = (a0 + a1) + (a2 + a3);
    __syncthreads();
    if (l == 0 && i < n4) {
        f32x4 a = red[0][o];
#pragma unroll
        for (int k = 1; k < 16; ++k) a += red[k][o];
        reinterpret_cast<f32x4*>(out)[i] = a;
    }
}

__global__ void k_stem_pack(const float* w, float* wp, int Cout) {
    int i = blockIdx.x * blockDim.x + threadIdx.x;
    if (i >= Cout * 224) return;
    int n = i / 224, k = i - n * 224, tap = k >> 2, c = k & 3;
    wp[i] = (tap < 49 && c < 3) ? w[(n * 49 + tap) * 3 + c] : 0.f;
}
__global__ void k_stem_unpack(const float* gp, float* g, int Cout) {
    int i = blockIdx.x * blockDim.x + threadIdx.x;
    if (i >= Cout * 147) return;
    int n = i / 147, k = i - n * 147, tap = k / 3, c = k - tap * 3;
    g[i] = gp[n * 224 + tap * 4 + c];
}

template <typename K>
static int set_smem(K kern, size_t bytes) {
    if (bytes > 64 * 1024) {
        if (hipFuncSetAttribute(reinterpret_cast<const void*>(kern), hipFuncAttributeMaxDynamicSharedMemorySize, (int)bytes) != hipSuccess)
            return OSI_ERR_LAUNCH;
    }
    return OSI_OK;
}

static bool desc_ok(const osi_conv_desc* d) {
    if (!d) return false;
    if (d->B <= 0 || d->H <= 0 || d->W <= 0 || d->Cin <= 0 || d->Cout <= 0) return false;
    if (d->R <= 0 || d->S <= 0 || d->stride <= 0 || d->pad < 0) return false;
    if (d->Ho != (d->H + 2 * d->pad - d->R) / d->stride + 1) return false;
    if (d->Wo != (d->W + 2 * d->pad - d->S) / d->stride + 1) return false;
    if (d->Ho <= 0 || d->Wo <= 0) return false;
    if ((long)d->B * d->H * d->W * d->Cin >= (1l << 29)) return false;
    if ((long)d->B * d->Ho * d->Wo * d->Cout >= (1l << 29)) return false;
    if ((long)d->Cout * d->R * d->S * (d->Cin < 4 ? 4 : d->Cin) >= (1l << 29)) return false;
    return true;
}
static bool is_stem(const osi_conv_desc* d) { return d->Cin == 4 && d->R == 7 && d->S == 7; }

enum ConvDir { DIR_FWD , DIR_DGRAD , DIR_WGRAD  };
static ConvP make_p(const osi_conv_desc* d, ConvDir dir) {
    ConvP p{};
    p.B = d->B; p.H = d->H; p.W = d->W; p.Cin = d->Cin; p.Ho = d->Ho; p.Wo = d->Wo; p.Cout = d->Cout;
    p.R = d->R; p.S = d->S; p.stride = d->stride; p.pad = d->pad;
    p.M = d->B * d->Ho * d->Wo;
    p.Ktot = is_stem(d) ? 224 : d->R * d->S * d->Cin;
    p.dHoWo = make_fastdiv((uint32_t)(d->Ho * d->Wo));
    p.dWo = make_fastdiv((uint32_t)d->Wo);
    p.unit = (d->R == 1 && d->S == 1 && d->stride == 1 && d->pad == 0) ? 1 : 0;
    const int in_bytes = (int)((size_t)d->B * d->H * d->W * d->Cin * 4), out_bytes = (int)((size_t)d->B * d->Ho * d->Wo * d->Cout * 4);
    p.x_bytes = dir == DIR_DGRAD ? out_bytes : in_bytes;
    p.w_bytes = dir == DIR_WGRAD ? out_bytes : (int)((size_t)d->Cout * p.Ktot * 4);
#ifdef OSI_STAMPS
    p.stamps = g_osi_stamps;
#endif
    return p;
}

struct TailPlan { int MT1, S, ksT, tiles; };
static TailPlan plan_tail_split(long MT, int NT, int T) {
    TailPlan t{(int)MT, 1, T, 0};
    if (!g_osi_tuning.tail_split || T < 4 || g_osi_tuning.tail_mint < 1) return t;
    const long ncu = chip_cus(), V = MT * NT;
    const long q = V / ncu, r = V - q * ncu;
    if (r == 0 || q > g_osi_tuning.tail_qmax) return t;
    if ((double)(ncu - r) / (double)ncu / (double)(q + 1) * 100.0 < (double)g_osi_tuning.tail_gain) return t;
    long MT1 = q * ncu / NT;
    long rem = (MT - MT1) * NT;
    long S = ncu / rem;
    if (S > T / g_osi_tuning.tail_mint) S = T / g_osi_tuning.tail_mint;
    if (S > g_osi_tuning.tail_smax) S = g_osi_tuning.tail_smax;
    if (q <= 2) {
        const long smax = std::min<long>(g_osi_tuning.tail_smax, T / g_osi_tuning.tail_mint);
        double best = S >= 2 ? 1.0 / (double)S : 1.0;
        for (long c = 2; c <= smax; ++c) {
            const double cost = (double)((rem * c + ncu - 1) / ncu) / (double)c;
            if (cost < best - 1e-9) { best = cost; S = c; }
        }
        if ((1.0 - best) / (double)(q + 1) * 100.0 < (double)g_osi_tuning.tail_gain) return t;
    }
    if (S <= 1) return t;
    const int ksT = (int)((T + S - 1) / S);
    S = (T + ksT - 1) / ksT;
    if (S <= 1) return t;
    t.MT1 = (int)MT1; t.S = (int)S; t.ksT = ksT; t.tiles = (int)rem;
    return t;
}
static size_t tail_slab_floats(const TailPlan& t) { return t.S > 1 ? (size_t)t.tiles * t.S * 4096 : 0; }

static int set_tail_split(ConvP& p, const TailPlan& tp, float* slab) {
    p.MT1 = tp.MT1; p.ks_S = tp.S; p.ks_T = tp.ksT; p.ks_slab = slab;
    p.g1 = osi_cdiv(p.MT1, 8) * 8 * p.NT;
    const int keys = (p.MT - p.MT1) * tp.S;
    return p.g1 + osi_cdiv(keys, 8) * 8 * p.NT;
}

template <int WM, int WN, bool STEM, int NST = 2, int XF = 0, bool W3 = false, bool OE = false, bool SPLIT = false>
static int launch_fwd(ConvP p, hipStream_t st, const TailPlan* tp = nullptr, float* slab = nullptr) {
    constexpr int BM = 64 * WM, BN = 64 * WN;
    p.MT = osi_cdiv(p.M, BM); p.NT = p.Cout / BN;
    size_t smem = NST * (size_t)((W3 ? W3_WROWS : BM) + BN) * LDR * sizeof(float);
    if (XF) smem += (size_t)2 * p.Cin * sizeof(float);
    if (W3) p.cW[0] = make_fastdiv((uint32_t)p.W + 1);
    if (int e = set_smem(k_conv_fwd<WM, WN, STEM, NST, XF, SPLIT, W3, OE>, smem)) return e;
    const int grid = SPLIT ? set_tail_split(p, *tp, slab) : osi_cdiv(p.MT, 8) * 8 * p.NT;
    hipLaunchKernelGGL((k_conv_fwd<WM, WN, STEM, NST, XF, SPLIT, W3, OE>), dim3(grid), dim3(256), smem, st, p);
    OSI_LAUNCH_CHECK();
    if constexpr (SPLIT) {
        hipLaunchKernelGGL(k_conv_fwd_tail_fixup, dim3(tp->tiles), dim3(256), 0, st, p);
        OSI_LAUNCH_CHECK();
    }
    return OSI_OK;
}
template <int KT, int XF, bool OE = false>
static int launch_fwd_rows(ConvP p, hipStream_t st) {
    p.MT = osi_cdiv(p.M, 64); p.NT = p.Cout / 64;
    int walkers = (4 * hw_cus() / p.NT + 7) / 8 * 8;
    if (walkers < 8) walkers = 8;
    if (walkers > p.MT) walkers = (p.MT + 7) / 8 * 8;
    const size_t smem = ((size_t)2 * KT * 64 * LDR + 2 * p.Cin + 2 * 64 * 3) * sizeof(float);
    if (int e = set_smem(k_conv1x1_rows<KT, XF, OE>, smem)) return e;
    hipLaunchKernelGGL((k_conv1x1_rows<KT, XF, OE>), dim3(walkers * p.NT), dim3(256), smem, st, p, walkers);
    OSI_LAUNCH_CHECK();
    return OSI_OK;
}
static bool rows_rule(const osi_conv_desc* d, bool shortcut) {
    const int m = g_osi_tuning.fwd_rows;
    const bool unit = d->R == 1 && d->S == 1 && d->stride == 1 && d->pad == 0;
    if (!m || !unit || shortcut || d->Cout % 64 || (d->Cin != 64 && d->Cin != 128)) return false;
    return m == 2 || (d->Cin == 64 && (long)d->B * d->Ho * d->Wo >= 64L * 8 * hw_cus());
}

template <int WM, int WN, int NST, int FUSED, bool POOL = false, bool W3 = false, bool SPLIT = false>
static int launch_dgrad(ConvP p, hipStream_t st, const TailPlan* tp = nullptr, float* slab = nullptr) {
    constexpr int BM = 64 * WM, BN = 64 * WN;
    const int s = p.stride;
    for (int ph = 0; ph < s; ++ph)
        for (int pw = 0; pw < s; ++pw) {
            const int hc = (p.H - ph + s - 1) / s, wc = (p.W - pw + s - 1) / s;
            p.cHW[ph * s + pw] = make_fastdiv((uint32_t)(hc * wc > 0 ? hc * wc : 1));
            p.cW[ph * s + pw] = make_fastdiv((uint32_t)(wc > 0 ? wc : 1));
        }
    p.unit = (p.R == 1 && p.S == 1 && s == 1 && p.pad == 0) ? 1 : 0;
    const int Hc = osi_cdiv(p.H, s), Wc = osi_cdiv(p.W, s);
    p.MT = osi_cdiv((long)p.B * Hc * Wc, BM); p.NT = p.Cin / BN;
    size_t smem = 2 * (size_t)((W3 ? W3_WROWS : BM) * LDR + BK * (BN + 4)) * sizeof(float);
    smem = smem / 2 * NST;
    if (W3) p.cW[1] = make_fastdiv((uint32_t)p.W + 1);
    if (int e = set_smem(k_conv_dgrad<WM, WN, NST, FUSED, SPLIT, POOL, W3>, smem)) return e;
    const int grid = SPLIT ? set_tail_split(p, *tp, slab) : osi_cdiv(p.MT, 8) * 8 * p.NT;
    hipLaunchKernelGGL((k_conv_dgrad<WM, WN, NST, FUSED, SPLIT, POOL, W3>), dim3(grid, s * s), dim3(256), smem, st, p, Hc, Wc);
    OSI_LAUNCH_CHECK();
    if constexpr (SPLIT) {
        hipLaunchKernelGGL(k_conv_dgrad_tail_fixup<FUSED>, dim3(tp->tiles), dim3(256), 0, st, p);
        OSI_LAUNCH_CHECK();
    }
    return OSI_OK;
}

template <int WM, int WN, bool STEM, int NST = 2, bool XF = false>
static int launch_wgrad(ConvP p, int splits, hipStream_t st) {
    constexpr int BM = 64 * WM, BN = 64 * WN;
    p.MT = p.Cout / BM;
    p.NT = STEM ? osi_cdiv(p.Ktot, BN) : p.R * p.S * (p.Cin / BN);
    size_t smem = 2 * (size_t)BK * (BM + 4 + BN + 4) * sizeof(float);
    smem = smem / 2 * NST;
    p.wtbl = (!STEM && !p.unit) ? 1 : 0;
    smem += 32 * BK * sizeof(uint32_t);
    if (XF) smem += 2 * BN * sizeof(float);
    if (int e = set_smem(k_conv_wgrad<WM, WN, STEM, NST, XF>, smem)) return e;
    p.splits = splits;
    p.wgroup = g_osi_tuning.wgrad_group;
    if (p.wgroup) {
        const int taps = STEM ? 1 : p.R * p.S;
        const int ctiles = p.NT / taps;
        if (p.wgroup == 1) { p.gkind = 3; p.gkeys = p.MT * ctiles * splits; p.ginner = taps; }
        else if (splits >= 8) { p.gkind = 0; p.gkeys = splits; p.ginner = p.MT * ctiles * taps; }
        else {
            const double dy_bytes = (double)p.Cout, x_bytes = (double)p.Cin;
            const double cost_rows = x_bytes * (p.MT < 8 ? p.MT : 8) + dy_bytes, cost_cols = dy_bytes * (ctiles < 8 ? ctiles : 8) + x_bytes;
            if (cost_rows <= cost_cols) { p.gkind = 1; p.gkeys = splits * p.MT; p.ginner = ctiles * taps; }
            else { p.gkind = 2; p.gkeys = splits * ctiles; p.ginner = p.MT * taps; }
        }
        const long grid = ((long)p.gkeys + 7) / 8 * 8 * p.ginner;
        hipLaunchKernelGGL((k_conv_wgrad<WM, WN, STEM, NST, XF>), dim3((unsigned)grid), dim3(256), smem, st, p);
    } else {
        hipLaunchKernelGGL((k_conv_wgrad<WM, WN, STEM, NST, XF>), dim3(p.MT * p.NT, splits), dim3(256), smem, st, p);
    }
    OSI_LAUNCH_CHECK();
    return OSI_OK;
}

static bool wgrad3_ok(const osi_conv_desc* d) {
    if (!g_osi_tuning.wgrad3 || d->R != 3 || d->S != 3 || d->pad != 1 || d->Cin % 32 || d->Cout % 64) return false;
    if (d->stride == 1) return d->W <= 63;
    return d->stride == 2 && g_osi_tuning.wgrad3 >= 2 && d->H % 2 == 0 && d->W % 2 == 0 && 130 + 2 * d->Wo <= 192;
}
template <int NWIN, bool XF, bool S2 = false>
static int launch_wgrad3_n(ConvP p, int splits, hipStream_t st) {
    p.MT = p.Cout / 64;
    const int ctiles = p.Cin / 32;
    p.splits = splits;
    if (splits >= 8) { p.gkind = 0; p.gkeys = splits; p.ginner = p.MT * ctiles; }
    else { p.gkind = 3; p.gkeys = p.MT * ctiles * splits; p.ginner = 1; }
    const size_t smem = ((size_t)W3_BKP * W3_LDA + (size_t)NWIN * 32 * W3_LDB + 32) * sizeof(float);
    if (int e = set_smem(k_conv_wgrad3<NWIN, XF, S2>, smem)) return e;
    const long grid = ((long)p.gkeys + 7) / 8 * 8 * p.ginner;
    hipLaunchKernelGGL((k_conv_wgrad3<NWIN, XF, S2>), dim3((unsigned)grid), dim3(256), smem, st, p);
    OSI_LAUNCH_CHECK();
    return OSI_OK;
}
template <bool XF>
static int launch_wgrad3(const ConvP& p, int splits, hipStream_t st) {
    if (p.stride == 2) return 130 + 2 * p.Wo <= 160 ? launch_wgrad3_n<5, XF, true>(p, splits, st) : launch_wgrad3_n<6, XF, true>(p, splits, st);
    const int win = W3_BKP + 2 * p.W + 2;
    if (win <= 64) return launch_wgrad3_n<2, XF>(p, splits, st);
    if (win <= 96) return launch_wgrad3_n<3, XF>(p, splits, st);
    return launch_wgrad3_n<5, XF>(p, splits, st);
}

struct TileShape { int wm, wn, nst; };
static TileShape tile_shape(int tile) {
    static const TileShape ids[9] = {{0, 0, 0}, {2, 2, 2}, {2, 1, 2}, {1, 2, 2}, {1, 1, 2}, {1, 1, 1}, {1, 2, 1}, {2, 2, 1}, {2, 1, 1}};
    return tile >= 1 && tile <= 8 ? ids[tile] : ids[0];
}
static int tile_rows(int tile) { return tile_shape(tile).wm == 2 ? 128 : 64; }
template <class F>
static int with_shape(TileShape s, F&& f) {
    return pick<1, 2>(s.wm, [&](auto WM) {
        return pick<1, 2>(s.wn, [&](auto WN) {
            return pick<1, 2>(s.nst, [&](auto NST) { return f(WM, WN, NST); });
        });
    });
}
// ... 295 lines not shown
            OSI_REQUIRE(f->partials_bytes >= (size_t)3 * p.eP * d->Cin * sizeof(float));
            p.ey0 = f->y0; p.ey1 = f->y1; p.esum = f->partials;
            *P = p.eP;
        }
    }
    return launch_dgrad_plan(pl, p, pl.split ? f->partials + dgrad_partial_floats(d) : nullptr, (hipStream_t)stream);
}

int osi_conv_dgrad(const osi_conv_desc* d, const float* dy, const float* w, float* dx, int accumulate, int tile,
                   osi_stream_t stream) {
    OSI_REQUIRE(accumulate >= 0 && accumulate <= 2);
    return conv_dgrad_impl(d, dy, w, dx, accumulate == 1 ? dx : nullptr, nullptr, tile, nullptr, stream, accumulate == 2);
}

size_t osi_conv_dgrad_fused_workspace(const osi_conv_desc* d) {
    if (!desc_ok(d)) return 0;
    return (dgrad_partial_floats(d) + tail_slab_floats(tail_plan(d, true))) * sizeof(float);
}

int osi_conv_dgrad_fused(const osi_conv_desc* d, const float* dy, const float* w, float* dx, const float* addend,
                         const osi_dgrad_fusion* f, int tile, int* P, osi_stream_t stream) {
    OSI_REQUIRE(f && P);
    return conv_dgrad_impl(d, dy, w, dx, addend, f, tile, P, stream);
}

int osi_conv_dgrad_fused_frozen(const osi_conv_desc* d, const float* dy, const float* w, float* dx, const osi_dgrad_fusion* f, int tile,
                                int* P, osi_stream_t stream) {
    OSI_REQUIRE(f && f->scale0 && f->shift0 && f->y0 && !f->relu_mask && !f->y1 && !f->pool_idx && f->addend_stride <= 1);
    OSI_REQUIRE(!f->partials || P);
    OSI_REQUIRE(tile == OSI_TILE_AUTO || tile == OSI_TILE_64x64_S1);
    return conv_dgrad_impl(d, dy, w, dx, nullptr, f, OSI_TILE_64x64_S1, P, stream, false, true);
}

static bool wgrad_shape_ok(const osi_conv_desc* d) {
    return d->Cout % 64 == 0 && (is_stem(d) || d->Cin % 64 == 0 || wgrad3_ok(d));
}

size_t osi_conv_wgrad_workspace(const osi_conv_desc* d) {
    if (!desc_ok(d) || !wgrad_shape_ok(d)) return 0;
    const WgradPlan w = plan_wgrad(d);
    const size_t n = (size_t)d->Cout * (is_stem(d) ? 224 : d->R * d->S * d->Cin);
    return w.splits > 1 ? (size_t)w.splits * n * sizeof(float) : 0;
}

static int conv_wgrad_impl(const osi_conv_desc* d, const float* dy, const float* x, float* dw, void* ws, size_t ws_bytes,
                           osi_stream_t stream, const float* in_scale, const float* in_shift) {
    OSI_REQUIRE(desc_ok(d) && dy && x && dw);
    OSI_REQUIRE(!in_scale || !is_stem(d));
    OSI_REQUIRE(wgrad_shape_ok(d));
    hipStream_t st = (hipStream_t)stream;
    const WgradPlan w = plan_wgrad(d);
    ConvP p = make_p(d, DIR_WGRAD);
    const size_t n = (size_t)d->Cout * p.Ktot;
    OSI_REQUIRE(n % 4 == 0);
    if (w.splits > 1) OSI_REQUIRE(ws && ws_bytes >= (size_t)w.splits * n * sizeof(float));
    p.x = x; p.w = dy; p.y = w.splits > 1 ? (float*)ws : dw;
    p.kchunk = w.kchunk; p.slab_stride = n;
    p.in_scale = in_scale; p.in_shift = in_shift;
    int e;
    if (w.all_taps) e = in_scale ? launch_wgrad3<true>(p, w.splits, st) : launch_wgrad3<false>(p, w.splits, st);
    else if (is_stem(d)) e = launch_wgrad<1, 1, true>(p, w.splits, st);
    else {
        e = with_shape({w.wm, w.wn, in_scale ? 1 : g_osi_tuning.wgrad_nst}, [&](auto WM, auto WN, auto NST) -> int {
            constexpr int wm = decltype(WM)::value, wn = decltype(WN)::value, nst = decltype(NST)::value;
            if constexpr (nst == 1) { if (in_scale) return launch_wgrad<wm, wn, false, 1, true>(p, w.splits, st); }
            return launch_wgrad<wm, wn, false, nst>(p, w.splits, st);
        });
    }
    if (e) return e;
    return w.splits > 1 ? launch_slab_reduce((const float*)ws, dw, n / 4, n / 4, w.splits, st) : OSI_OK;
}

int osi_conv_wgrad(const osi_conv_desc* d, const float* dy, const float* x, float* dw, void* ws, size_t ws_bytes,
                   osi_stream_t stream) {
    return conv_wgrad_impl(d, dy, x, dw, ws, ws_bytes, stream, nullptr, nullptr);
}

int osi_conv_wgrad_act(const osi_conv_desc* d, const float* dy, const float* x, const float* in_scale, const float* in_shift, float* dw,
                       void* ws, size_t ws_bytes, osi_stream_t stream) {
    OSI_REQUIRE(in_scale && in_shift);
    return conv_wgrad_impl(d, dy, x, dw, ws, ws_bytes, stream, in_scale, in_shift);
}

int osi_stem_weight_pack(const float* w_krsc3, float* w_packed, int Cout, osi_stream_t stream) {
    OSI_REQUIRE(w_krsc3 && w_packed && Cout > 0);
    hipLaunchKernelGGL(k_stem_pack, dim3(osi_cdiv(Cout * 224, 256)), dim3(256), 0, (hipStream_t)stream, w_krsc3, w_packed, Cout);
    OSI_LAUNCH_CHECK();
    return OSI_OK;
}
int osi_stem_grad_unpack(const float* g_packed, float* g_krsc3, int Cout, osi_stream_t stream) {
    OSI_REQUIRE(g_packed && g_krsc3 && Cout > 0);
    hipLaunchKernelGGL(k_stem_unpack, dim3(osi_cdiv(Cout * 147, 256)), dim3(256), 0, (hipStream_t)stream, g_packed, g_krsc3, Cout);
    OSI_LAUNCH_CHECK();
    return OSI_OK;
}

}
```

openset-imagenet_amd/csrc/osi_common.h:

```cpp
#pragma once
#include <hip/hip_runtime.h>
#include <stdint.h>
#include <type_traits>
#include "../../include/osi.h"

typedef float f32x4 __attribute__((ext_vector_type(4)));
typedef float f32x2 __attribute__((ext_vector_type(2)));
typedef float f32x16 __attribute__((ext_vector_type(16)));

#define OSI_LAUNCH_CHECK()                                     \
    do {                                                       \
        hipError_t e__ = hipGetLastError();                    \
        if (e__ != hipSuccess) return OSI_ERR_LAUNCH;          \
    } while (0)

#define OSI_REQUIRE(cond)                                      \
    do {                                                       \
        if (!(cond)) return OSI_ERR_ARG;                       \
    } while (0)

#define OSI_TUNING_KNOBS(X)                                                                                                              \
    X(wgrad_tile, 0, 0, 64, 1)         \
    X(wgrad_blocks, 2048, 1, 1 << 20, 1)          \
    X(wgrad_nst, 1, 1, 2, 0)                                                     \
    X(bn_grid, 1024, 1, 1 << 20, 0)                                                       \
    X(bn_single_p, 128, 1, 1 << 20, 0)      \
    X(wgrad3, 2, 0, 2, 1)              \
    X(wgrad3_blocks, 768, 1, 1 << 20, 1)                         \
    X(fwd_wide, 0, 0, 1, 0)                 \
    X(dgrad_wide, 0, 0, 1, 0)                                                                 \
    X(wgrad_group, 2, 0, 2, 1)         \
    X(tail_split, 1, 0, 1, 1)          \
    X(tail_cus, 0, 0, 4096, 1)                             \
    X(tail_smax, 8, 1, 64, 1)                                                           \
    X(tail_mint, 16, 1, 4096, 1)                                                              \
    X(stem_direct, 1, 0, 1, 1)         \
    X(tail_gain, 8, 0, 100, 1)         \
    X(tail_qmax, 8, 0, 4096, 1)                                                         \
    X(bn_grid_bwd, 1024, 1, 1 << 20, 0)     \
    X(bn_wide_p, 2048, 0, 2048, 0)     \
    X(fwd_rows, 1, 0, 2, 0)            \
    X(fwd_w3, 1, 0, 1, 0)              \
    X(dgrad_w3, 1, 0, 1, 0)            \
    X(fwd_wino, 1, 0, 1, 1)            \
    X(dgrad_wino, 1, 0, 1, 1)                                  \
    X(wgrad_wino, 1, 0, 1, 1)          \
    X(wino_wide, 1, 0, 1, 0)           \
    X(wino_streamk, 2, 0, 3, 0)        \
    X(dp_reserved_cus, 0, 0, 128, 1)

struct OsiTuning {
#define OSI_KNOB_FIELD(name, def, lo, hi, plan) int name = def;
    OSI_TUNING_KNOBS(OSI_KNOB_FIELD)
#undef OSI_KNOB_FIELD
};
extern OsiTuning g_osi_tuning;

static inline int osi_cdiv(long a, long b) { return (int)((a + b - 1) / b); }

template <int V> using Int = std::integral_constant<int, V>;
template <int... Vs, class F>
static int pick(int v, F&& f) {
    int r = OSI_ERR_ARG;
    (void)((v == Vs && ((r = f(Int<Vs>{})), true)) || ...);
    return r;
}

constexpr int OSI_BN_GROUPS = 32;
static inline size_t bn_pstats_floats(int P, int C) { return (size_t)2 * P * C + (size_t)2 * OSI_BN_GROUPS * C; }

struct FastDiv {
    uint32_t mul, sh, d;
};
static inline FastDiv make_fastdiv(uint32_t d) {
    FastDiv f;
    f.d = d;
    if (d == 1) { f.mul = 0; f.sh = 0; return f; }
    uint32_t l = 0;
    while ((1ull << l) < d) ++l;
    uint64_t m = ((1ull << (32 + l)) + d - 1) / d;
    f.mul = (uint32_t)(m - (1ull << 32));
    f.sh = l;
    return f;
}
__device__ __forceinline__ uint32_t fdiv(uint32_t n, const FastDiv& f) {
    uint32_t t = __umulhi(n, f.mul);
    const uint32_t q = (((n - t) >> 1) + t) >> ((f.sh - 1) & 31);
    return f.d == 1 ? n : q;
}

__device__ __forceinline__ void chan_merge(float& na, float& ma, float& sa, float nb, float mb, float sb) {
    if (nb == 0.f) return;
    if (na == 0.f) { na = nb; ma = mb; sa = sb; return; }
    const float n = na + nb, d = mb - ma;
    ma += d * (nb / n);
    sa += sb + d * d * (na * nb / n);
    na = n;
}

__device__ __forceinline__ float osi_max(float a, float b) { return __builtin_elementwise_maximum(a, b); }
__device__ __forceinline__ float osi_relu(float t) { return __builtin_elementwise_maximum(t, 0.f); }
__device__ __forceinline__ f32x4 osi_relu(f32x4 t) { return __builtin_elementwise_maximum(t, f32x4{0.f, 0.f, 0.f, 0.f}); }

__device__ __forceinline__ float wave_sum(float v) {
#pragma unroll
    for (int o = 32; o > 0; o >>= 1) v += __shfl_xor(v, o, 64);
    return v;
}
__device__ __forceinline__ double wave_sum(double v) {
#pragma unroll
    for (int o = 32; o > 0; o >>= 1) v += __shfl_xor(v, o, 64);
    return v;
}
__device__ __forceinline__ unsigned wave_sum(unsigned v) {
#pragma unroll
    for (int o = 32; o > 0; o >>= 1) v += __shfl_xor(v, o, 64);
    return v;
}
__device__ __forceinline__ float wave_max(float v) {
#pragma unroll
    for (int o = 32; o > 0; o >>= 1) v = osi_max(v, __shfl_xor(v, o, 64));
    return v;
}
__device__ __forceinline__ double wave_fmax(double v) {
#pragma unroll
    for (int o = 32; o > 0; o >>= 1) v = fmax(v, __shfl_xor(v, o, 64));
    return v;
}
__device__ __forceinline__ double wave_fmin(double v) {
#pragma unroll
    for (int o = 32; o > 0; o >>= 1) v = fmin(v, __shfl_xor(v, o, 64));
    return v;
// ... 2 lines not shown
```

openset-imagenet_amd/csrc/resnet50_exec.hip:

```cpp
#include "osi_common.h"
#include <string>
#include <vector>
#include <cstring>
#include <cstdio>

#define OSI_TRY(x)                 \
    do {                           \
        int e__ = (x);             \
        if (e__ != OSI_OK) return e__; \
    } while (0)

namespace {

constexpr size_t WS_NONE = (size_t)-1;

struct Tensor {
    std::string name;
    int ndim; int shape[4];
    size_t off, numel;
    int unit;
};
struct BN {
    std::string prefix;
    int C, M;
    size_t g_off, b_off;
    size_t rm_off, rv_off;
    size_t mean, invstd, scale, shift;
    size_t dsink;
    int unit;
};
struct Conv {
    osi_conv_desc d;
    size_t w_off;
    int bn;
    size_t y;
    size_t a;
    size_t mask;
    size_t u_fw = WS_NONE, u_bw = WS_NONE;
    int unit;
};
struct Block {
    int c1, c2, c3, ds;
    size_t x_in;
    size_t out;
    int stage;
};

constexpr size_t ALIGN_F = 64;
constexpr unsigned EV_FLAGS = hipEventDisableTiming | hipEventDisableSystemFence;
constexpr unsigned EV_FLAGS_HANDOFF = hipEventDisableTiming;
static size_t up(size_t v, size_t a) { return (v + a - 1) / a * a; }
static void grow(size_t& m, size_t v) { if (v > m) m = v; }
static int device_cus() {
    int v = 0, dev = 0;
    if (hipGetDevice(&dev) != hipSuccess || hipDeviceGetAttribute(&v, hipDeviceAttributeMultiprocessorCount, dev) != hipSuccess) return 0;
    return v;
}

struct BwRequest {
    float* dimage = nullptr;
    int param_grads = 1;
    float* x_adv = nullptr;
    float eps = 0.f, lo = 0.f, hi = 0.f;
    const float* x_anchor = nullptr;
    float alpha = 0.f;
    bool operator==(const BwRequest& o) const {
        return dimage == o.dimage && param_grads == o.param_grads && x_adv == o.x_adv && eps == o.eps && lo == o.lo && hi == o.hi &&
               x_anchor == o.x_anchor && alpha == o.alpha;
    }
};

}

struct osi_resnet50 {
    int B, H, W, F, O, logit_bias;
    std::vector<Tensor> tensors;
    std::vector<BN> bns;
    std::vector<Conv> convs;
    std::vector<Block> blocks;
    size_t param_floats = 0, buffer_floats = 0, ws_floats = 0;
    int t_fc_w, t_fc_b, t_lg_w, t_lg_b;
    int Hs, Ws, Hp, Wp;
    size_t x4, wpack, gpack, a_pool, pool_idx, pooled, feat;
// ... 20 lines not shown
    int cur_grad = -1;
    bool go_fused = false;
    int fused_P = 0;
    int stem_stats_P = 0;
    std::vector<int> free_list;
    bool prof_on = false;
    bool prof_timeline = false;
    std::vector<int> prof_side;
    std::vector<hipEvent_t> prof_ev;
    std::vector<int> prof_cls;
    int prof_n = 0;
    int mark(int cls, hipStream_t st) {
        if (!prof_on) return OSI_OK;
        if (prof_n == (int)prof_ev.size()) {
            hipEvent_t e;
            if (hipEventCreate(&e) != hipSuccess) return OSI_ERR_LAUNCH;
            prof_ev.push_back(e); prof_cls.push_back(0); prof_side.push_back(0);
        }
        prof_cls[prof_n] = cls;
        prof_side[prof_n] = (side != nullptr && st == side) ? 1 : 0;
        if (hipEventRecord(prof_ev[prof_n], st) != hipSuccess) return OSI_ERR_LAUNCH;
        ++prof_n;
        return OSI_OK;
    }

    static constexpr int NUNITS = 18;
    int cur_unit = 0;
    unsigned unit_mask = (1u << NUNITS) - 1;
    int eval_prefix = 0;
    float bn_momentum = 0.1f;
    bool trainable(int unit) const { return (unit_mask >> unit) & 1u; }
    int cut() const { int c = 0; while (!((unit_mask >> c) & 1u)) ++c; return c; }
    int bw_stop() const { return (rq.param_grads && !rq.dimage && !rq.x_adv) ? cut() : 0; }

    size_t add_tensor(const std::string& name, int ndim, const int* shape) {
        Tensor t; t.name = name; t.ndim = ndim; t.numel = 1;
        for (int i = 0; i < 4; ++i) t.shape[i] = i < ndim ? shape[i] : 1;
        for (int i = 0; i < ndim; ++i) t.numel *= (size_t)shape[i];
        t.off = param_floats;
        t.unit = cur_unit;
        param_floats = up(param_floats + t.numel, 4);
        tensors.push_back(t);
        return t.off;
    }
    size_t ws_alloc(size_t floats) {
        size_t o = ws_floats;
        ws_floats = up(ws_floats + floats, ALIGN_F);
        return o;
    }
    int add_conv_bn(const std::string& cname, const std::string& bname, int Bn, int Hin, int Win, int Cin, int Cout, int k, int s,
                    int pad, bool keep_act) {
        Conv c{};
        c.d.B = Bn; c.d.H = Hin; c.d.W = Win; c.d.Cin = Cin; c.d.Cout = Cout; c.d.R = k; c.d.S = k; c.d.stride = s; c.d.pad = pad;
        c.d.Ho = (Hin + 2 * pad - k) / s + 1; c.d.Wo = (Win + 2 * pad - k) / s + 1;
        int shp[4] = {Cout, Cin == 4 && k == 7 ? 3 : Cin, k, k};
        c.w_off = add_tensor(cname + ".weight", 4, shp);
        BN b; b.prefix = bname; b.C = Cout; b.M = Bn * c.d.Ho * c.d.Wo;
        int s1[1] = {Cout};
        b.g_off = add_tensor(bname + ".weight", 1, s1);
        b.b_off = add_tensor(bname + ".bias", 1, s1);
        b.rm_off = buffer_floats; buffer_floats += up(Cout, 4);
        b.rv_off = buffer_floats; buffer_floats += up(Cout, 4);
        b.mean = ws_alloc(Cout); b.invstd = ws_alloc(Cout); b.scale = ws_alloc(Cout); b.shift = ws_alloc(Cout);
        b.unit = c.unit = cur_unit;
        c.bn = (int)bns.size();
        bns.push_back(b);
        size_t n = (size_t)b.M * Cout;
        c.y = ws_alloc(n);
        c.a = keep_act ? ws_alloc(n) : WS_NONE;
        c.mask = keep_act ? ws_alloc(osi_bn_relu_mask_bytes(b.M, Cout) / sizeof(float)) : WS_NONE;
        convs.push_back(c);
        return (int)convs.size() - 1;
    }
    void* staged_ws = nullptr;
    bool overlap = true;
    bool fwd_fork = true;
    bool side_prio_normal = false;
    const float* x4_ext = nullptr;
    bool wants_grads(int unit) const { return rq.param_grads && trainable(unit); }
    float* dgam(float* grads, float* ws, const BN& b) const { return wants_grads(b.unit) ? grads + b.g_off : ws + b.dsink; }
    float* dbet(float* grads, float* ws, const BN& b) const { return wants_grads(b.unit) ? grads + b.b_off : ws + b.dsink + b.C; }
    const float* dg_col(const float* ws, int col, int P, int C) const { return ws + dg_ws + (size_t)col * P * C; }
    bool stem_tail_fused() const { return !frozen && !rq.dimage && !rq.x_adv && stem_ws_bytes > 0; }
    bool eval_fused = true;
    bool stage_join = true;
    OsiTuning plan_knobs;
    int plan_hw_cus = 0;
    bool plan_unchanged() const {
        const OsiTuning &a = plan_knobs, &b = g_osi_tuning;
        bool same = plan_hw_cus == device_cus();
#define OSI_KNOB_SAME(name, def, lo, hi, plan) same = same && (!(plan) || a.name == b.name);
        OSI_TUNING_KNOBS(OSI_KNOB_SAME)
#undef OSI_KNOB_SAME
        return same;
    }
    hipStream_t side = nullptr;
    hipEvent_t ev_fork = nullptr, ev_join = nullptr, ev_rmain = nullptr, ev_rside = nullptr, ev_wt = nullptr;
    bool wt_pending = false;
    hipEvent_t buf_ev[NSCR] = {};
    bool buf_pending[NSCR] = {};
    bool side_dirty = false;
    int ensure_side() {
        if (side) return OSI_OK;
        int lo = 0, hi = 0;
        if (hipDeviceGetStreamPriorityRange(&lo, &hi) != hipSuccess) return OSI_ERR_LAUNCH;
        const int prio = side_prio_normal ? 0 : lo;
        if (hipStreamCreateWithPriority(&side, hipStreamNonBlocking, prio) != hipSuccess) return OSI_ERR_LAUNCH;
        if (hipEventCreateWithFlags(&ev_fork, EV_FLAGS) != hipSuccess) return OSI_ERR_LAUNCH;
        if (hipEventCreateWithFlags(&ev_join, EV_FLAGS) != hipSuccess) return OSI_ERR_LAUNCH;
        if (hipEventCreateWithFlags(&ev_wt, EV_FLAGS) != hipSuccess) return OSI_ERR_LAUNCH;
        for (int i = 0; i < NSCR; ++i)
            if (hipEventCreateWithFlags(&buf_ev[i], EV_FLAGS) != hipSuccess) return OSI_ERR_LAUNCH;
        return OSI_OK;
    }
    bool wants_side() const { return overlap && (!prof_on || prof_timeline); }
    bool async_wgrad() const { return wants_side() && side != nullptr; }
    int take(hipStream_t st, int* idx) {
        if (free_list.empty()) return OSI_ERR_STATE;
        int i = free_list.front(); free_list.erase(free_list.begin());
        if (buf_pending[i]) {
            if (hipStreamWaitEvent(st, buf_ev[i], 0) != hipSuccess) return OSI_ERR_LAUNCH;
            buf_pending[i] = false;
        }
        *idx = i;
        return OSI_OK;
    }
    void give(int i) { free_list.push_back(i); }
    int fork_side(hipStream_t st) {
        if (hipEventRecord(ev_fork, st) != hipSuccess) return OSI_ERR_LAUNCH;
        if (hipStreamWaitEvent(side, ev_fork, 0) != hipSuccess) return OSI_ERR_LAUNCH;
        return OSI_OK;
    }
    int wait_weight_transforms(hipStream_t st) {
        if (!wt_pending) return OSI_OK;
        if (hipStreamWaitEvent(st, ev_wt, 0) != hipSuccess) return OSI_ERR_LAUNCH;
        wt_pending = false;
        return OSI_OK;
    }
    int join_side(hipStream_t st) {
        if (!side_dirty) return OSI_OK;
        if (hipEventRecord(ev_join, side) != hipSuccess) return OSI_ERR_LAUNCH;
        if (hipStreamWaitEvent(st, ev_join, 0) != hipSuccess) return OSI_ERR_LAUNCH;
        for (int i = 0; i < NSCR; ++i) buf_pending[i] = false;
        side_dirty = false;
        return OSI_OK;
    }
    ~osi_resnet50() {
        for (hipEvent_t e : prof_ev) (void)hipEventDestroy(e);
        if (side) {
            (void)hipStreamSynchronize(side);
            (void)hipEventDestroy(ev_fork); (void)hipEventDestroy(ev_join); (void)hipEventDestroy(ev_wt);
            for (int i = 0; i < NSCR; ++i) (void)hipEventDestroy(buf_ev[i]);
            (void)hipStreamDestroy(side);
        }
        if (ev_rmain) (void)hipEventDestroy(ev_rmain);
        if (ev_rside) (void)hipEventDestroy(ev_rside);
    }
};

extern "C" {

int osi_resnet50_create(osi_resnet50_t* out, int B, int H, int W, int fc_dim, int out_features, int logit_bias) {
    OSI_REQUIRE(out && B > 0 && H >= 32 && W >= 32 && fc_dim > 0 && out_features > 0);
    osi_resnet50* n = new osi_resnet50();
    n->B = B; n->H = H; n->W = W; n->F = fc_dim; n->O = out_features; n->logit_bias = logit_bias ? 1 : 0;
    const std::string rb = "resnet_base.";
// ... 427 lines not shown
        n->fwd_done = true;
        n->next_stage = 0;
    }
    return n->mark(OSI_PROF_OTHER, st);
}

int osi_resnet50_forward(osi_resnet50_t n, const float* params, float* buffers, long long* nbt, const float* image,
                         void* workspace, float* logits, float* features, int training, osi_stream_t stream) {
    OSI_REQUIRE(n && params && buffers && workspace && logits && features);
    OSI_REQUIRE(!training || nbt);
    return forward_impl(n, params, buffers, nbt, image, workspace, logits, features, training ? BnMode::Batch : BnMode::Inference, stream);
}

int osi_resnet50_forward_frozen(osi_resnet50_t n, const float* params, const float* buffers, const float* image, void* workspace,
                                float* logits, float* features, osi_stream_t stream) {
    OSI_REQUIRE(n && params && buffers && workspace && logits && features);
    return forward_impl(n, params, const_cast<float*>(buffers), nullptr, image, workspace, logits, features, BnMode::Frozen, stream);
}

static int wgrad_launch(osi_resnet50* n, int ci, float* grads, float* ws, int gi, const float* conv_in, hipStream_t st, int in_bn,
                        bool async) {
    Conv& c = n->convs[ci];
    const float* dy = ws + n->scratch[gi];
    hipStream_t ws_st = st;
    if (async) {
        OSI_TRY(n->fork_side(st));
        ws_st = n->side;
    }
    if (ci == 0) {
        if (osi_stem_wgrad_direct_workspace(&c.d) > 0) {
            OSI_TRY(osi_stem_wgrad_direct(&c.d, dy, conv_in, grads + c.w_off, ws + n->wg_ws, n->wg_ws_bytes, ws_st));
        } else {
            OSI_TRY(osi_conv_wgrad(&c.d, dy, conv_in, ws + n->gpack, ws + n->wg_ws, n->wg_ws_bytes, ws_st));
            OSI_TRY(osi_stem_grad_unpack(ws + n->gpack, grads + c.w_off, 64, ws_st));
        }
    } else if (in_bn >= 0 && n->plan_knobs.wgrad_wino && osi_conv_wgrad_wino_workspace(&c.d) > 0) {
        OSI_TRY(osi_conv_wgrad_wino(&c.d, dy, conv_in, ws + n->bns[in_bn].scale, ws + n->bns[in_bn].shift, grads + c.w_off, ws + n->wg_ws,
                                    n->wg_ws_bytes, ws_st));
    } else if (in_bn >= 0) {
        OSI_TRY(osi_conv_wgrad_act(&c.d, dy, conv_in, ws + n->bns[in_bn].scale, ws + n->bns[in_bn].shift, grads + c.w_off, ws + n->wg_ws,
                                   n->wg_ws_bytes, ws_st));
    } else {
        OSI_TRY(osi_conv_wgrad(&c.d, dy, conv_in, grads + c.w_off, ws + n->wg_ws, n->wg_ws_bytes, ws_st));
    }
    if (async) {
        if (hipEventRecord(n->buf_ev[gi], n->side) != hipSuccess) return OSI_ERR_LAUNCH;
        n->buf_pending[gi] = true;
        n->side_dirty = true;
    }
    OSI_TRY(n->mark(OSI_PROF_CONV_WGRAD, ws_st));
    return OSI_OK;
}

static int wgrad(osi_resnet50* n, int ci, float* grads, float* ws, int gi, const float* conv_in, hipStream_t st, int in_bn = -1) {
    if (!n->wants_grads(n->convs[ci].unit)) return OSI_OK;
    return wgrad_launch(n, ci, grads, ws, gi, conv_in, st, in_bn, n->async_wgrad());
}

static int dgrad_plain(osi_resnet50* n, const osi_conv_desc* d, const float* dy, const float* w, float* dx, int accumulate, hipStream_t st) {
    OSI_TRY(osi_conv_dgrad(d, dy, w, dx, accumulate, OSI_TILE_AUTO, st));
    return n->mark(OSI_PROF_CONV_DGRAD, st);
}

static int bn_bwd_raw(osi_resnet50* n, int ci, const float* params, float* grads, float* ws, int gi, int gmasked, hipStream_t st) {
    Conv& c = n->convs[ci];
    BN& b = n->bns[c.bn];
    float* g = ws + n->scratch[gi];
    OSI_TRY(osi_bn_backward_relu_mask(g, ws + c.mask, ws + c.y, ws + b.mean, ws + b.invstd, params + b.g_off, g, ws + n->scratch[gmasked],
                                      n->dgam(grads, ws, b), n->dbet(grads, ws, b), b.M, b.C, ws + n->bn_ws, n->bn_ws_bytes, st));
    return n->mark(OSI_PROF_BN_BWD, st);
}

static int bn_bwd_fused(osi_resnet50* n, int ci, const float* params, float* grads, float* ws, int gi, int dyi, int which,
                        hipStream_t st) {
    Conv& c = n->convs[ci];
    BN& b = n->bns[c.bn];
    const int P = n->fused_P;
    OSI_TRY(osi_bn_backward_fused(ws + n->scratch[gi], ws + c.y, ws + b.mean, ws + b.invstd, params + b.g_off, n->dg_col(ws, 0, P, b.C),
                                  n->dg_col(ws, 1 + which, P, b.C), P, ws + n->scratch[dyi], n->dgam(grads, ws, b), n->dbet(grads, ws, b),
                                  b.M, b.C, ws + n->bn_ws, n->bn_ws_bytes, st));
    return n->mark(OSI_PROF_BN_BWD, st);
}

static int bn_bwd_fused_pair(osi_resnet50* n, int ci, int cj, const float* params, float* grads, float* ws, int gi, int dyi, int dyj,
                             hipStream_t st) {
    osi_bn_fused_consumer cs[2];
    const int idx[2] = {ci, cj}, out[2] = {dyi, dyj};
    for (int k = 0; k < 2; ++k) {
        Conv& c = n->convs[idx[k]];
        BN& b = n->bns[c.bn];
        cs[k] = osi_bn_fused_consumer{ws + c.y, ws + b.mean, ws + b.invstd, params + b.g_off, n->dg_col(ws, 1 + k, n->fused_P, b.C),
                                      ws + n->scratch[out[k]], n->dgam(grads, ws, b), n->dbet(grads, ws, b)};
    }
    BN& b = n->bns[n->convs[ci].bn];
    OSI_TRY(osi_bn_backward_fused2(ws + n->scratch[gi], cs, n->dg_col(ws, 0, n->fused_P, b.C), n->fused_P, b.M, b.C, ws + n->bn_ws,
                                   n->bn_ws_bytes, st));
    return n->mark(OSI_PROF_BN_BWD, st);
}

static int bn_reduce_frozen(osi_resnet50* n, int ci, float* grads, float* ws, int which, hipStream_t st) {
    BN& b = n->bns[n->convs[ci].bn];
    if (!n->wants_grads(b.unit)) return OSI_OK;
    const int P = n->fused_P;
    OSI_TRY(osi_bn_backward_reduce(n->dg_col(ws, 0, P, b.C), n->dg_col(ws, 1 + which, P, b.C), P, grads + b.g_off, grads + b.b_off, b.M, b.C,
                                   ws + n->bn_ws, n->bn_ws_bytes, st));
    return n->mark(OSI_PROF_BN_BWD, st);
}
static int bn_bwd_frozen(osi_resnet50* n, int ci, int cj, float* grads, float* ws, int gi, int dyi, int dyj, int gmasked, bool masked,
                         hipStream_t st) {
    osi_bn_frozen_consumer cs[2];
    const int idx[2] = {ci, cj}, out[2] = {dyi, dyj};
    const int nc = cj >= 0 ? 2 : 1;
    for (int k = 0; k < nc; ++k) {
        Conv& c = n->convs[idx[k]];
        BN& b = n->bns[c.bn];
        const bool red = masked && n->wants_grads(b.unit);
        cs[k] = osi_bn_frozen_consumer{ws + c.y, ws + b.mean, ws + b.invstd, ws + b.scale, ws + n->scratch[out[k]],
                                       red ? grads + b.g_off : nullptr, red ? grads + b.b_off : nullptr};
    }
    Conv& c = n->convs[ci];
    BN& b = n->bns[c.bn];
    OSI_TRY(osi_bn_backward_frozen(ws + n->scratch[gi], masked ? ws + c.mask : nullptr, cs, nc, gmasked >= 0 ? ws + n->scratch[gmasked] : nullptr,
                                   b.M, b.C, ws + n->bn_ws, n->bn_ws_bytes, st));
    return n->mark(OSI_PROF_BN_BWD, st);
}
static int dgrad_frozen(osi_resnet50* n, int ci, const float* params, float* grads, float* ws, int dyi, int dxi, int pc, hipStream_t st) {
    Conv& c = n->convs[ci];
    Conv& p0 = n->convs[pc];
    BN& b0 = n->bns[p0.bn];
    osi_dgrad_fusion f{};
    f.scale0 = ws + b0.scale; f.shift0 = ws + b0.shift;
    f.y0 = ws + p0.y; f.mean0 = ws + b0.mean; f.invstd0 = ws + b0.invstd;
    f.partials = ws + n->dg_ws; f.partials_bytes = n->dg_ws_bytes;
    int P = 0;
    OSI_TRY(osi_conv_dgrad_fused_frozen(&c.d, ws + n->scratch[dyi], params + c.w_off, ws + n->scratch[dxi], &f, OSI_TILE_AUTO, &P, st));
    n->fused_P = P;
    OSI_TRY(n->mark(OSI_PROF_CONV_DGRAD, st));
    return bn_reduce_frozen(n, pc, grads, ws, 0, st);
}

static int dgrad_fused(osi_resnet50* n, int ci, const float* params, float* ws, int dyi, int dxi, int addi, int pc, int pd,
                       hipStream_t st, bool add_even = false) {
    Conv& c = n->convs[ci];
    Conv& p0 = n->convs[pc];
    BN& b0 = n->bns[p0.bn];
    osi_dgrad_fusion f{};
    if (p0.mask != WS_NONE) f.relu_mask = ws + p0.mask;
    else { f.scale0 = ws + b0.scale; f.shift0 = ws + b0.shift; }
    f.y0 = ws + p0.y; f.mean0 = ws + b0.mean; f.invstd0 = ws + b0.invstd;
    if (pd >= 0) {
        Conv& p1 = n->convs[pd];
        BN& b1 = n->bns[p1.bn];
        f.y1 = ws + p1.y; f.mean1 = ws + b1.mean; f.invstd1 = ws + b1.invstd;
    }
    f.partials = ws + n->dg_ws; f.partials_bytes = n->dg_ws_bytes;
    f.addend_stride = add_even ? 2 : 1;
    int P = 0;
    OSI_TRY(n->wait_weight_transforms(st));
    if (n->plan_knobs.dgrad_wino && f.scale0 && pd < 0 && addi < 0 && c.u_bw != WS_NONE)
        OSI_TRY(osi_conv_dgrad_fused_wino_pre(&c.d, ws + n->scratch[dyi], ws + c.u_bw, ws + n->scratch[dxi], &f, ws + n->wino_ws,
                                              n->wino_ws_bytes, &P, st));
    else
    OSI_TRY(osi_conv_dgrad_fused(&c.d, ws + n->scratch[dyi], params + c.w_off, ws + n->scratch[dxi],
                                 addi >= 0 ? ws + n->scratch[addi] : nullptr, &f, OSI_TILE_AUTO, &P, st));
    n->fused_P = P;
    return n->mark(OSI_PROF_CONV_DGRAD, st);
}

static int dgrad_bn_inblock(osi_resnet50* n, int ci, int pc, const float* params, float* grads, float* ws, int dyi, int dxi, hipStream_t st) {
    if (n->frozen) return dgrad_frozen(n, ci, params, grads, ws, dyi, dxi, pc, st);
    OSI_TRY(dgrad_fused(n, ci, params, ws, dyi, dxi, -1, pc, -1, st));
    return bn_bwd_fused(n, pc, params, grads, ws, dxi, dxi, 0, st);
}

static int block_bwd_entry(osi_resnet50* n, const Block& k, const float* params, float* grads, float* ws, hipStream_t st, int* d3, int* t1,
                           int* dxbase) {
    const int go = n->cur_grad;
    const bool has_ds = k.ds >= 0;
    if (!n->go_fused) {
        if (has_ds) return OSI_ERR_STATE;
        OSI_TRY(n->take(st, dxbase));
        if (n->frozen) OSI_TRY(bn_bwd_frozen(n, k.c3, -1, grads, ws, go, go, -1, *dxbase, true, st));
        else OSI_TRY(bn_bwd_raw(n, k.c3, params, grads, ws, go, *dxbase, st));
        *d3 = go;
        return OSI_OK;
    }
    if (has_ds) OSI_TRY(n->take(st, t1));
    if (n->frozen) {
        OSI_TRY(bn_reduce_frozen(n, k.c3, grads, ws, 0, st));
        if (has_ds) OSI_TRY(bn_reduce_frozen(n, k.ds, grads, ws, 1, st));
    }
    OSI_TRY(n->take(st, d3));
    if (n->frozen) OSI_TRY(bn_bwd_frozen(n, k.c3, k.ds, grads, ws, go, *d3, *t1, -1, false, st));
    else if (has_ds) OSI_TRY(bn_bwd_fused_pair(n, k.c3, k.ds, params, grads, ws, go, *d3, *t1, st));
    else OSI_TRY(bn_bwd_fused(n, k.c3, params, grads, ws, go, *d3, 0, st));
    if (has_ds) n->give(go);
    else *dxbase = go;
    return OSI_OK;
}

static int block_bwd_exit(osi_resnet50* n, int bi, const float* params, float* ws, hipStream_t st, int t3, int dxbase, bool no_dx,
                          bool ds_sparse) {
    const Block& k = n->blocks[bi];
    Conv& c1 = n->convs[k.c1];
    auto S = [&](int i) { return ws + n->scratch[i]; };
    if (no_dx) {
        if (dxbase >= 0) n->give(dxbase);
        n->cur_grad = -1;
        n->go_fused = false;
    } else if (bi > 0) {
        const Block& pk = n->blocks[bi - 1];
        int dxn = dxbase;
        if (k.ds < 0) OSI_TRY(n->take(st, &dxn));
        OSI_TRY(dgrad_fused(n, k.c1, params, ws, t3, dxn, dxbase, pk.c3, pk.ds, st, ds_sparse));
        if (dxn != dxbase) n->give(dxbase);
        n->cur_grad = dxn;
        n->go_fused = true;
    } else {
        if (n->stem_tail_fused()) {
            Conv& c0 = n->convs[0];
            BN& b0 = n->bns[c0.bn];
            osi_dgrad_fusion f{};
            f.y0 = ws + c0.y; f.mean0 = ws + b0.mean; f.invstd0 = ws + b0.invstd;
            f.partials = ws + n->dg_ws; f.partials_bytes = n->dg_ws_bytes;
            f.pool_idx = ws + n->pool_idx; f.pool_H = n->Hs; f.pool_W = n->Ws;
            int P = 0;
            OSI_TRY(osi_conv_dgrad_fused(&c1.d, S(t3), params + c1.w_off, S(dxbase), S(dxbase), &f, OSI_TILE_AUTO, &P, st));
            n->stem_stats_P = P;
            OSI_TRY(n->mark(OSI_PROF_CONV_DGRAD, st));
        } else {
            OSI_TRY(dgrad_plain(n, &c1.d, S(t3), params + c1.w_off, S(dxbase), 1, st));
        }
        n->cur_grad = dxbase;
        n->go_fused = false;
    }
    return OSI_OK;
}

static int block_backward(osi_resnet50* n, int bi, const float* params, float* grads, float* ws, hipStream_t st, bool no_dx) {
    const Block& k = n->blocks[bi];
    Conv &c1 = n->convs[k.c1], &c2 = n->convs[k.c2];
    const float* x = ws + k.x_in;
    int d3 = -1, t1 = -1, dxbase = -1, t2 = -1, t3 = -1;
    OSI_TRY(block_bwd_entry(n, k, params, grads, ws, st, &d3, &t1, &dxbase));
    const bool ds_sparse = k.ds >= 0 && bi > 0 && n->convs[k.ds].d.stride == 2 && n->convs[k.ds].d.R == 1;
    if (k.ds >= 0) {
        Conv& cd = n->convs[k.ds];
        OSI_TRY(wgrad(n, k.ds, grads, ws, t1, x, st));
        if (!no_dx) {
            OSI_TRY(n->take(st, &dxbase));
            OSI_TRY(dgrad_plain(n, &cd.d, ws + n->scratch[t1], params + cd.w_off, ws + n->scratch[dxbase], ds_sparse ? 2 : 0, st));
        }
        n->give(t1);
    }
    OSI_TRY(wgrad(n, k.c3, grads, ws, d3, ws + c2.y, st, c2.bn));
    OSI_TRY(n->take(st, &t2));
    OSI_TRY(dgrad_bn_inblock(n, k.c3, k.c2, params, grads, ws, d3, t2, st));
    n->give(d3);
    OSI_TRY(wgrad(n, k.c2, grads, ws, t2, ws + c1.y, st, c1.bn));
    OSI_TRY(n->take(st, &t3));
    OSI_TRY(dgrad_bn_inblock(n, k.c2, k.c1, params, grads, ws, t2, t3, st));
    n->give(t2);
    OSI_TRY(wgrad(n, k.c1, grads, ws, t3, x, st));
    OSI_TRY(block_bwd_exit(n, bi, params, ws, st, t3, dxbase, no_dx, ds_sparse));
    n->give(t3);
    return OSI_OK;
}

static int head_backward(osi_resnet50* n, const float* params, float* grads, float* ws, const float* dlogits, const float* dfeatures,
                         hipStream_t st) {
    OSI_REQUIRE(dlogits);
    const int head = osi_resnet50::NUNITS - 1;
    n->free_list.clear();
    for (int i = 0; i < osi_resnet50::NSCR; ++i) { n->free_list.push_back(i); n->buf_pending[i] = false; }
    const Tensor& fw = n->tensors[n->t_fc_w]; const Tensor& fb = n->tensors[n->t_fc_b]; const Tensor& lw = n->tensors[n->t_lg_w];
    float* dfeat = ws + n->dfeat;
    int acc = 0;
    if (dfeatures) {
        if (hipMemcpyAsync(dfeat, dfeatures, (size_t)n->B * n->F * sizeof(float), hipMemcpyDeviceToDevice, st) != hipSuccess)
            return OSI_ERR_LAUNCH;
        acc = 1;
    }
    const bool pg = n->wants_grads(head);
    float* dlb = pg && n->t_lg_b >= 0 ? grads + n->tensors[n->t_lg_b].off : nullptr;
    OSI_TRY(osi_linear_bwd(dlogits, ws + n->feat, params + lw.off, dfeat, acc, pg ? grads + lw.off : nullptr, dlb, n->B, n->F, n->O, st));
    const bool below = n->bw_stop() < head;
    OSI_TRY(osi_linear_bwd(dfeat, ws + n->pooled, params + fw.off, below ? ws + n->dpooled : nullptr, 0, pg ? grads + fw.off : nullptr,
                           pg ? grads + fb.off : nullptr, n->B, 2048, n->F, st));
    n->cur_grad = -1;
    n->go_fused = false;
    if (below) {
        OSI_TRY(n->take(st, &n->cur_grad));
        OSI_TRY(osi_avgpool_bwd(ws + n->dpooled, ws + n->scratch[n->cur_grad], n->B, n->Hf * n->Wf, 2048, st));
    }
    return n->mark(OSI_PROF_OTHER, st);
}

static int stem_tail(osi_resnet50* n, const float* params, float* grads, float* ws, hipStream_t st) {
    auto S = [&](int i) { return ws + n->scratch[i]; };
    Conv& c0 = n->convs[0];
    BN& b0 = n->bns[c0.bn];
    const BwRequest& rq = n->rq;
    const int go = n->cur_grad;
    int t = -1;
    OSI_TRY(n->take(st, &t));
    const float* x4c = n->x4_cur ? n->x4_cur : ws + n->x4;
    if (n->stem_tail_fused()) {
        n->give(t);
        const int P = n->stem_stats_P;
        OSI_TRY(osi_bn_backward_reduce(n->dg_col(ws, 0, P, 64), n->dg_col(ws, 1, P, 64), P, grads + b0.g_off, grads + b0.b_off,
                                       n->B * n->Hs * n->Ws, 64, ws + n->bn_ws, n->bn_ws_bytes, st));
        OSI_TRY(n->mark(OSI_PROF_BN_BWD, st));
        OSI_TRY(osi_stem_wgrad_fused(&c0.d, S(go), ws + n->pool_idx, ws + c0.y, x4c, params + b0.g_off, ws + b0.mean, ws + b0.invstd,
                                     grads + b0.g_off, grads + b0.b_off, grads + c0.w_off, ws + n->stem_ws, n->stem_ws_bytes, st));
        OSI_TRY(n->mark(OSI_PROF_CONV_WGRAD, st));
        n->give(go);
        return OSI_OK;
    }
    if (n->frozen) {
        const bool red = n->wants_grads(0);
        OSI_TRY(osi_bn_relu_maxpool_bwd_frozen(S(go), ws + n->pool_idx, ws + c0.y, ws + b0.mean, ws + b0.invstd, ws + b0.scale, S(t),
                                               red ? grads + b0.g_off : nullptr, red ? grads + b0.b_off : nullptr, n->B, n->Hs, n->Ws, 64,
                                               ws + n->bn_ws, n->bn_ws_bytes, st));
    } else {
        OSI_TRY(osi_bn_relu_maxpool_bwd(S(go), ws + n->pool_idx, ws + c0.y, ws + b0.mean, ws + b0.invstd, params + b0.g_off, S(t),
                                        n->dgam(grads, ws, b0), n->dbet(grads, ws, b0), n->B, n->Hs, n->Ws, 64, ws + n->bn_ws,
                                        n->bn_ws_bytes, st));
    }
    OSI_TRY(n->mark(OSI_PROF_BN_BWD, st));
    n->give(go);
    OSI_TRY(wgrad(n, 0, grads, ws, t, x4c, st));
    if (rq.dimage) {
        OSI_TRY(osi_stem_dgrad(S(t), params + c0.w_off, rq.dimage, n->B, n->H, n->W, st));
        OSI_TRY(n->mark(OSI_PROF_CONV_DGRAD, st));
    } else if (rq.x_adv && !rq.x_anchor && rq.alpha == rq.eps) {
        OSI_TRY(osi_stem_dgrad_fgsm(S(t), params + c0.w_off, x4c, rq.x_adv, rq.eps, rq.lo, rq.hi, n->B, n->H, n->W, st));
        OSI_TRY(n->mark(OSI_PROF_CONV_DGRAD, st));
    } else if (rq.x_adv) {
        OSI_TRY(osi_stem_dgrad_pgd(S(t), params + c0.w_off, x4c, rq.x_anchor ? rq.x_anchor : x4c, rq.x_adv, rq.alpha, rq.eps, rq.lo, rq.hi,
                                   n->B, n->H, n->W, st));
// ... 221 lines not shown
```

openset-imagenet_amd/openset_imagenet/_native.py:

```python
import ctypes
import os
from ctypes import c_char_p, c_double, c_float, c_int, c_longlong, c_size_t, c_void_p, POINTER, Structure

_HERE = os.path.dirname(os.path.abspath(__file__))
CSRC_DIR = os.path.normpath(os.path.join(_HERE, "..", "csrc"))
LIB_PATH = os.path.join(CSRC_DIR, "libosi_hip.so")
TORCH_LIB_PATH = os.path.join(CSRC_DIR, "libosi_torch.so")

OSI_OK = 0
TILE_AUTO, TILE_128x128, TILE_128x64, TILE_64x128, TILE_64x64 = 0, 1, 2, 3, 4
LOSS_ENTROPIC, LOSS_SOFTMAX, LOSS_GARBAGE = 0, 1, 2


class ConvDesc(Structure):
    _fields_ = [(n, c_int) for n in ("B", "H", "W", "Cin", "Ho", "Wo", "Cout", "R", "S", "stride", "pad")]

    @classmethod
    def make(cls, B, H, W, Cin, Cout, k, stride, pad):
        Ho = (H + 2 * pad - k) // stride + 1
        Wo = (W + 2 * pad - k) // stride + 1
        return cls(B, H, W, Cin, Ho, Wo, Cout, k, k, stride, pad)


class ConvEpilogue(Structure):
# ... 160 lines not shown
    "osi_hist_f64": (c_int, [P, P, c_int, c_int, P, c_int, P, P]),
    "osi_openmax_workspace": (c_size_t, [c_int, c_int, c_int]),
    "osi_openmax_class_means": (c_int, [P, P, P, c_int, c_int, c_int, P, P, P, P, c_size_t, P]),
    "osi_openmax_distances": (c_int, [P, P, P, c_int, c_int, c_int, c_int, P, P]),
    "osi_openmax_fit_tails": (c_int, [P, P, P, c_int, c_int, c_int, P, P, P, P, P, P, P, c_size_t, P]),
    "osi_openmax_wscores": (c_int, [P, c_int, c_int, P, P, P, P, P, P]),
    "osi_openmax_recalibrate": (c_int, [P, P, c_int, c_int, c_int, P, P]),
    "osi_evm_workspace": (c_size_t, [c_int, c_int, c_int]),
    "osi_evm_distances": (c_int, [P, c_int, P, c_int, c_int, c_int, P, P, c_size_t, P]),
    "osi_evm_fit_rows": (c_int, [P, c_int, c_int, c_longlong, P, c_longlong, c_int, c_float, P, P, P, P, P, P, P, c_size_t, P]),
    "osi_evm_set_cover": (c_int, [P, c_int, P, P, P, P, c_float, c_float, P, P, P, c_size_t, P]),
    "osi_evm_probs": (c_int, [P, c_int, c_int, c_longlong, P, P, P, P, c_int, c_float, P, P]),
    "osi_knn_workspace": (c_size_t, [c_int, c_int, c_int]),
    "osi_knn_topk": (c_int, [P, c_int, c_int, c_longlong, c_int, P, P, P, P, c_size_t, P]),
    "osi_knn_class_kth": (c_int, [P, c_int, c_int, c_longlong, P, c_int, c_int, P, c_int, P, P, c_size_t, P]),
    "osi_maha_workspace": (c_size_t, [c_int, c_int, c_int]),
    "osi_maha_class_means": (c_int, [P, P, c_int, c_int, c_int, P, P, P, c_size_t, P]),
    "osi_maha_scatter": (c_int, [P, P, P, c_int, c_int, c_int, c_int, c_int, P, P, c_size_t, P]),
    "osi_maha_factor": (c_int, [P, c_int, c_double, c_double, P, P, P, P, P, c_size_t, P]),
    "osi_maha_whiten_f32": (c_int, [P, c_int, c_int, P, P, P, c_size_t, P]),
    "osi_maha_whiten_f64": (c_int, [P, c_int, c_int, P, P, P, c_size_t, P]),
    "osi_maha_sqdist": (c_int, [P, c_int, P, c_int, c_int, P, c_int, P, P, P, c_size_t, P]),
    "osi_vim_workspace": (c_size_t, [c_int, c_int, c_int]),
    "osi_eigh_begin": (c_int, [P, c_int, P, P, P, P, P, c_size_t, P]),
    "osi_eigh_sweep": (c_int, [P, P, c_int, P, P, P, P, c_size_t, P]),
    "osi_eigh_finish": (c_int, [P, P, c_int, P, P, P, P, c_size_t, P]),
    "osi_vim_project_f32": (c_int, [P, P, c_int, c_int, P, c_int, P, P, c_size_t, P]),
    "osi_vim_scores": (c_int, [P, c_int, c_int, P, c_int, c_double, c_int, P, P, P, c_size_t, P]),
    "osi_order_stats_workspace": (c_size_t, [c_longlong, c_int]),
    "osi_order_stats_f32": (c_int, [P, c_longlong, POINTER(c_longlong), c_int, P, P, c_size_t, P]),
    "osi_shape_rows_workspace": (c_size_t, [c_int, c_int]),
    "osi_shape_rows": (c_int, [P, c_int, c_int, c_int, c_int, c_float, P, P, c_size_t, P]),
    "osi_logit_scores": (c_int, [P, c_int, c_int, c_int, P, P]),
    "osi_resnet50_pooled": (c_int, [c_void_p, P, P, POINTER(c_size_t), P]),
    "osi_mix_rows_pairs": (c_int, [P, P, P, c_int, c_size_t, P]),
    "osi_proser_loss_fwd_bwd": (c_int, [P, P, P, c_int, c_int, c_int, c_int, c_float, c_float, c_float, P, P, P, P]),
    "osi_proser_scores": (c_int, [P, P, c_float, c_int, c_int, c_int, P, P]),
    "osi_resnet50_set_mix": (c_int, [c_void_p, P, P]),
    "osi_resnet50_debug_unit_input": (c_int, [c_void_p, P, c_int, P, POINTER(c_size_t), P]),
    "osi_adam_step": (c_int, [P, P, P, P, c_size_t, c_double, c_double, c_double, c_double, c_longlong, c_float, P]),
    "osi_sgd_step": (c_int, [P, P, P, c_size_t, c_float, c_float, c_int, c_float, P]),
    "osi_adam_step_groups": (c_int, [P, P, P, P, P, c_size_t, POINTER(OptSegment), c_int, POINTER(AdamGroup), c_int, c_float, P]),
    "osi_sgd_step_groups": (c_int, [P, P, P, c_size_t, POINTER(OptSegment), c_int, POINTER(SgdGroup), c_int, c_float, P]),
    "osi_grad_norm_workspace": (c_size_t, [c_size_t]),
    "osi_grad_clip_scale": (c_int, [P, c_size_t, POINTER(GradSpan), c_int, c_int, c_float, c_float, P, c_size_t, P, P]),
    "osi_adam_step_groups_dev": (c_int, [P, P, P, P, P, c_size_t, POINTER(OptSegment), c_int, POINTER(AdamGroup), c_int, P, P]),
    "osi_sgd_step_groups_dev": (c_int, [P, P, P, c_size_t, POINTER(OptSegment), c_int, POINTER(SgdGroup), c_int, P, P]),
    "osi_fill_f32": (c_int, [P, c_size_t, c_float, P]),
    "osi_scale_f32": (c_int, [P, c_size_t, c_float, P]),
    "osi_grad_accumulate": (c_int, [P, P, c_size_t, P]),
    "osi_i64_add": (c_int, [P, c_int, c_longlong, P]),
    "osi_average_update": (c_int, [POINTER(AvgSpan), c_int, c_float, P]),
    "osi_resnet50_create": (c_int, [POINTER(c_void_p), c_int, c_int, c_int, c_int, c_int, c_int]),
    "osi_resnet50_destroy": (None, [c_void_p]),
    "osi_resnet50_num_tensors": (c_int, [c_void_p]),
    "osi_resnet50_tensor_info": (c_int, [c_void_p, c_int, c_char_p, c_int, POINTER(c_int), POINTER(c_int), POINTER(c_size_t), POINTER(c_size_t)]),
    "osi_resnet50_param_floats": (c_size_t, [c_void_p]),
    "osi_resnet50_num_bn": (c_int, [c_void_p]),
    "osi_resnet50_bn_info": (c_int, [c_void_p, c_int, c_char_p, c_int, POINTER(c_int), POINTER(c_size_t), POINTER(c_size_t)]),
    "osi_resnet50_buffer_floats": (c_size_t, [c_void_p]),
    "osi_resnet50_workspace_bytes": (c_size_t, [c_void_p]),
    "osi_resnet50_num_stages": (c_int, [c_void_p]),
    "osi_resnet50_geometry": (c_int, [c_void_p, POINTER(c_int), POINTER(c_int), POINTER(c_int)]),
    "osi_resnet50_stage_grad_range": (c_int, [c_void_p, c_int, POINTER(c_size_t), POINTER(c_size_t)]),
    "osi_resnet50_grads_ready": (c_int, [c_void_p, P, P]),
    "osi_resnet50_num_units": (c_int, [c_void_p]),
    "osi_resnet50_tensor_unit": (c_int, [c_void_p, c_int]),
    "osi_resnet50_bn_unit": (c_int, [c_void_p, c_int]),
    "osi_resnet50_set_trainable": (c_int, [c_void_p, ctypes.c_uint, c_int]),
    "osi_resnet50_get_trainable": (c_int, [c_void_p, POINTER(ctypes.c_uint), POINTER(c_int)]),
    "osi_resnet50_set_bn_momentum": (c_int, [c_void_p, c_float]),
    "osi_resnet50_get_bn_momentum": (c_int, [c_void_p, POINTER(c_float)]),
    "osi_resnet50_set_option":(c_int, [c_void_p, c_char_p, c_int]),
    "osi_resnet50_profile": (c_int, [c_void_p, c_int]),
    "osi_resnet50_profile_read": (c_int, [c_void_p, POINTER(ctypes.c_double), POINTER(c_int)]),
    "osi_resnet50_timeline_read": (c_int, [c_void_p, POINTER(ctypes.c_double), POINTER(c_int), POINTER(c_int), c_int, POINTER(c_int)]),
    "osi_resnet50_debug_num_gates": (c_int, [c_void_p]),
    "osi_resnet50_debug_gate_shape": (c_int, [c_void_p, c_int, POINTER(c_int), POINTER(c_int), POINTER(c_int)]),
    "osi_resnet50_debug_gate": (c_int, [c_void_p, P, c_int, P, P, P]),
    "osi_resnet50_forward": (c_int, [c_void_p, P, P, P, P, P, P, P, c_int, P]),
    "osi_bn_frozen_coeffs_multi": (c_int, [POINTER(BnFrozenLayer), c_int, c_float, P]),
    "osi_conv_dgrad_fused_frozen": (c_int, [_PD, P, P, P, P, c_int, POINTER(c_int), P]),
    "osi_bn_backward_frozen": (c_int, [P, P, POINTER(BnFrozenConsumer), c_int, P, c_int, c_int, P, c_size_t, P]),
    "osi_bn_relu_maxpool_bwd_frozen": (c_int, [P, P, P, P, P, P, P, P, P, c_int, c_int, c_int, c_int, P, c_size_t, P]),
    "osi_resnet50_forward_frozen": (c_int, [c_void_p, P, P, P, P, P, P, P]),
    "osi_resnet50_backward": (c_int, [c_void_p, P, P, P, P, P, c_int, c_int, P]),
    "osi_resnet50_backward_ex": (c_int, [c_void_p, P, P, P, P, P, P, c_int, c_int, c_int, P]),
    "osi_resnet50_backward_adv": (c_int, [c_void_p, P, P, P, P, P, P, c_float, c_float, c_float, c_int, c_int, P]),
    "osi_resnet50_backward_attack": (c_int, [c_void_p, P, P, P, P, P, POINTER(Attack), c_int, c_int, c_int, P]),
}

_lib = None
DIAGNOSTIC_LIB = None


class NativeLibraryMissing(RuntimeError):
    pass


def lib():
    global _lib, LIB_PATH
    if _lib is None:
        global DIAGNOSTIC_LIB
        if os.environ.get("OSI_HIP_LIB"):
            if os.environ.get("OSI_DEV") != "1":
                raise NativeLibraryMissing("OSI_HIP_LIB selects a diagnostic build of the native library and is only honoured with OSI_DEV=1")
            LIB_PATH = os.environ["OSI_HIP_LIB"]
            DIAGNOSTIC_LIB = LIB_PATH
            import warnings
            warnings.warn(f"openset_imagenet: DIAGNOSTIC native library {LIB_PATH} (OSI_HIP_LIB + OSI_DEV=1): results may be wrong by design",
                          RuntimeWarning, stacklevel=2)
        if not os.path.isfile(LIB_PATH):
            raise NativeLibraryMissing(
                f"{LIB_PATH} not found: build the gfx950 HIP library first (python __graft_entry__.py, or make -C {CSRC_DIR}). "
                "There is no CPU fallback for the training hot path.")
        handle = ctypes.CDLL(LIB_PATH)
        for name, (res, args) in _SIGS.items():
            fn = getattr(handle, name)
            fn.restype = res
            fn.argtypes = args
        _lib = handle
        for name, _, _, _, _ in tuning_knobs(handle):
            env = "OSI_" + name.upper()
            if os.environ.get(env):
                check(handle.osi_set_tuning(name.encode(), int(os.environ[env])), f"osi_set_tuning({name})")
    return _lib


def tuning_knobs(handle=None):
    handle = handle or lib()
    rows, name, v = [], c_char_p(), [c_int() for _ in range(4)]
    while handle.osi_tuning_info(len(rows), ctypes.byref(name), *(ctypes.byref(x) for x in v)) == OSI_OK:
        rows.append((name.value.decode(), v[0].value, v[1].value, v[2].value, bool(v[3].value)))
    return rows


_ops = None


def ops():
    global _ops
    if _ops is None:
        lib()
        if not os.path.isfile(TORCH_LIB_PATH):
            raise NativeLibraryMissing(f"{TORCH_LIB_PATH} not found: build it first (python __graft_entry__.py, or make -C {CSRC_DIR}).")
        import torch
        torch.ops.load_library(TORCH_LIB_PATH)
        _ops = torch.ops.osi
    return _ops


def declared_symbols():
    return sorted(_SIGS)


def check(code, what=""):
    if code != OSI_OK:
        msg = lib().osi_strerror(code).decode()
        raise RuntimeError(f"libosi_hip {what} failed: {msg} (code {code})")


def ptr(t):
    return None if t is None else t.data_ptr()


def stream_of(t):
# ... 15 lines not shown
```

Baseline: 4526 images/sec.

## Add low-rank BN backward path for expansion 1x1 convs in final stage

Adds a low-rank formulation of the BN backward for bottleneck c3 and downsample 1x1 convs where Cout = 4*Cin. The BN-corrected gradient is never materialised. Instead, dgrad runs on the raw upstream gradient concatenated with a small K-dimension tail built from the scaled weights and the input activations, and wgrad is assembled from a Gram matrix of the activations plus corrections. The goal is to skip the full-size BN-backward apply pass and its memory traffic in stage 3, which is on by default (bn_lowrank=1). In exchange it adds Gram-matrix kernels, extra GEMM K-tiles and workspace demands, and it may change numerical rounding.

New measurement: 4571 images/sec (median of 6 runs). Within noise of the previous version (+1.0%).

```diff
diff --git a/__graft_entry__.py b/__graft_entry__.py
--- a/__graft_entry__.py
+++ b/__graft_entry__.py
@@ -38,6 +38,7 @@
     assert lib.osi_abi_version() >= 25 and hasattr(lib, "osi_maha_scatter") and hasattr(ops, "maha_factor")
     assert lib.osi_abi_version() >= 26 and hasattr(lib, "osi_eigh_sweep") and hasattr(ops, "vim_scores")
     assert lib.osi_abi_version() >= 27 and hasattr(lib, "osi_shape_rows") and hasattr(ops, "order_stats") and hasattr(ops, "resnet50_pooled")
+    assert lib.osi_abi_version() >= 28 and hasattr(lib, "osi_bn_backward_lowrank") and hasattr(lib, "osi_conv_dgrad_lowrank")
 
 
 def smoke():
diff --git a/include/osi.h b/include/osi.h
--- a/include/osi.h
+++ b/include/osi.h
@@ -91,6 +91,15 @@
                    osi_stream_t stream);
 int osi_conv_wgrad_act(const osi_conv_desc* d, const float* dy, const float* x, const float* in_scale, const float* in_shift, float* dw,
                        void* ws, size_t ws_bytes, osi_stream_t stream);
+size_t osi_conv_lowrank_workspace(const osi_conv_desc* d);
+int osi_bn_backward_lowrank(const osi_conv_desc* d, const float* w, const float* mean, const float* invstd, const float* gamma,
+                            const float* psum_g, const float* psum_gx, int P, float* dgamma, float* dbeta, void* ws, size_t ws_bytes,
+                            void* lr_ws, size_t lr_ws_bytes, osi_stream_t stream);
+int osi_conv_dgrad_lowrank(const osi_conv_desc* d, const float* g, const float* a, const float* a_scale, const float* a_shift,
+                           const void* lr_ws, size_t lr_ws_bytes, float* dx, int accumulate, const osi_dgrad_fusion* f, int* P,
+                           osi_stream_t stream);
+int osi_conv_wgrad_lowrank(const osi_conv_desc* d, const float* g, const float* a, const float* a_scale, const float* a_shift,
+                           const float* w, void* lr_ws, size_t lr_ws_bytes, float* dw, void* ws, size_t ws_bytes, osi_stream_t stream);
 size_t osi_conv_wgrad_wino_workspace(const osi_conv_desc* d);
 int osi_conv_wgrad_wino(const osi_conv_desc* d, const float* dy, const float* x, const float* in_scale, const float* in_shift, float* dw,
                         void* ws, size_t ws_bytes, osi_stream_t stream);
diff --git a/openset-imagenet_amd/csrc/abi.hip b/openset-imagenet_amd/csrc/abi.hip
--- a/openset-imagenet_amd/csrc/abi.hip
+++ b/openset-imagenet_amd/csrc/abi.hip
@@ -21,7 +21,7 @@
 }
 
 extern "C" {
-int osi_abi_version(void) { return 27; }
+int osi_abi_version(void) { return 28; }
 int osi_set_tuning(const char* name, int value) {
     const Knob* k = find_knob(name);
     if (!k) return OSI_ERR_ARG;
diff --git a/openset-imagenet_amd/csrc/bn.hip b/openset-imagenet_amd/csrc/bn.hip
--- a/openset-imagenet_amd/csrc/bn.hip
+++ b/openset-imagenet_amd/csrc/bn.hip
@@ -1,4 +1,4 @@
-#include "osi_common.h"
+#include "conv_common.h"
 
 namespace {
 
@@ -583,6 +583,44 @@
     }
 }
 
+struct LrCoef { float al, ka, be; };
+__device__ __forceinline__ LrCoef lr_coef(const float* mean, const float* invstd, const float* gamma, const float* c1, const float* c2, int n) {
+    const float r = invstd[n], al = gamma[n] * r, ka = al * c2[n] * r;
+    return LrCoef{al, ka, al * c1[n] - ka * mean[n]};
+}
+__global__ __launch_bounds__(NT) void k_bn_lowrank_prep(const float* __restrict__ w, const float* __restrict__ mean, const float* __restrict__ invstd,
+                                                       const float* __restrict__ gamma, const float* __restrict__ c1, const float* __restrict__ c2,
+                                                       int Cout, int Cin, float* alpha, float* kappa, float* beta, float* wcat, float* bw) {
+    __shared__ float red[NT];
+    const int b = blockIdx.x, tid = threadIdx.x;
+    if (b < Cout) {
+        const LrCoef k = lr_coef(mean, invstd, gamma, c1, c2, b);
+        if (tid == 0) { alpha[b] = k.al; kappa[b] = k.ka; beta[b] = k.be; }
+        for (int c = tid; c < Cin; c += NT) wcat[(size_t)b * Cin + c] = k.al * w[(size_t)b * Cin + c];
+        return;
+    }
+    const bool is_bw = b == Cout + Cin;
+    const int kk = is_bw ? 0 : b - Cout;
+    const int lanes = Cin < NT ? Cin : NT, G = NT / lanes, g = tid / lanes, cl = tid % lanes;
+    for (int c0 = 0; c0 < Cin; c0 += lanes) {
+        const int c = c0 + cl;
+        float acc = 0.f;
+        if (g < G)
+            for (int n = g; n < Cout; n += G) {
+                const LrCoef k = lr_coef(mean, invstd, gamma, c1, c2, n);
+                acc = __builtin_fmaf(is_bw ? k.be : w[(size_t)n * Cin + kk] * k.ka, w[(size_t)n * Cin + c], acc);
+            }
+        red[tid] = acc;
+        __syncthreads();
+        if (g == 0) {
+            for (int j = 1; j < G; ++j) acc += red[j * lanes + cl];
+            if (is_bw) bw[c] = acc;
+            else wcat[(size_t)(Cout + kk) * Cin + c] = -acc;
+        }
+        __syncthreads();
+    }
+}
+
 static int stream_geo(int c4n) { return NT % c4n == 0 ? 1 : c4n == 2 * NT ? 2 : 0; }
 
 static int rows_per_block(int M, int C, int& P) {
@@ -855,6 +893,27 @@
     return launch_bwd_apply(0, g, nullptr, y, mean, invstd, gamma, w, dy, nullptr, M, C, PoolSrc{}, st);
 }
 
+int osi_bn_backward_lowrank(const osi_conv_desc* d, const float* w, const float* mean, const float* invstd, const float* gamma,
+                            const float* psum_g, const float* psum_gx, int P, float* dgamma, float* dbeta, void* ws, size_t ws_bytes,
+                            void* lr_ws, size_t lr_ws_bytes, osi_stream_t stream) {
+    OSI_REQUIRE(osi_conv::conv_desc_ok(d) && osi_conv::lowrank_shape(d));
+    OSI_REQUIRE(w && mean && invstd && gamma && psum_g && psum_gx && dgamma && dbeta && ws && lr_ws && P > 0);
+    const osi_conv::LowRankWs L = osi_conv::lowrank_layout(d);
+    OSI_REQUIRE(lr_ws_bytes >= L.total * sizeof(float));
+    const int M = d->B * d->H * d->W, C = d->Cout;
+    int S, Pc;
+    bwd_groups(P, S, Pc);
+    OSI_REQUIRE(ws_bytes >= ws_floats(S, C) * sizeof(float));
+    hipStream_t st = (hipStream_t)stream;
+    const BwdWs bw = carve_ws(ws, S, C);
+    if (int e = bwd_reduce_partials(one_cons(psum_g, psum_gx, bw.a, bw.b, dgamma, dbeta, bw.c1, bw.c2), 1, P, M, C, S, Pc, st)) return e;
+    float* lw = (float*)lr_ws;
+    hipLaunchKernelGGL(k_bn_lowrank_prep, dim3(C + d->Cin + 1), dim3(NT), 0, st, w, mean, invstd, gamma, (const float*)bw.c1, (const float*)bw.c2, C,
+                       d->Cin, lw + L.alpha, lw + L.kappa, lw + L.beta, lw + L.wcat, lw + L.bw);
+    OSI_LAUNCH_CHECK();
+    return OSI_OK;
+}
+
 size_t osi_bn_backward_fused2_workspace(int C) {
     if (C <= 0) return 0;
     return 2 * ws_floats(OSI_BN_GROUPS, C) * sizeof(float);
diff --git a/openset-imagenet_amd/csrc/conv_common.h b/openset-imagenet_amd/csrc/conv_common.h
--- a/openset-imagenet_amd/csrc/conv_common.h
+++ b/openset-imagenet_amd/csrc/conv_common.h
@@ -38,4 +38,28 @@
                            hipStream_t st);
 constexpr int STEM_TILE_PIXELS = 128;
 
+static inline bool lowrank_shape(const osi_conv_desc* d) {
+    return d && d->R == 1 && d->S == 1 && d->stride == 1 && d->pad == 0 && d->Cin % 64 == 0 && d->Cout == 4 * d->Cin && d->Ho == d->H && d->Wo == d->W;
 }
+struct LowRankWs { size_t alpha, kappa, beta, wcat, bw, Ss, slab, total; int splits, kchunk; };
+static inline LowRankWs lowrank_layout(const osi_conv_desc* d) {
+    auto up64 = [](size_t v) { return (v + 63) / 64 * 64; };
+    const size_t C = (size_t)d->Cout, K = (size_t)d->Cin;
+    const long M = (long)d->B * d->H * d->W;
+    LowRankWs w{};
+    w.alpha = 0; w.kappa = up64(C); w.beta = 2 * up64(C);
+    w.wcat = 3 * up64(C);
+    w.bw = w.wcat + up64((C + K) * K);
+    w.Ss = w.bw + up64(K);
+    w.slab = w.Ss + up64((K + 1) * K);
+    const long tiles = (long)(K / 64) * (long)(K / 64);
+    long s = 512 / tiles, maxs = (M + 255) / 256;
+    if (s > maxs) s = maxs;
+    if (s < 1) s = 1;
+    const long chunk = ((M + s - 1) / s + 31) / 32 * 32;
+    w.kchunk = (int)chunk; w.splits = (int)((M + chunk - 1) / chunk);
+    w.total = w.slab + (size_t)w.splits * (K + 1) * K;
+    return w;
+}
+
+}
diff --git a/openset-imagenet_amd/csrc/conv_igemm.hip b/openset-imagenet_amd/csrc/conv_igemm.hip
--- a/openset-imagenet_amd/csrc/conv_igemm.hip
+++ b/openset-imagenet_amd/csrc/conv_igemm.hip
@@ -50,6 +50,9 @@
     size_t slab_stride;
     int MT1, g1, ks_S, ks_T;
     float* ks_slab;
+    const float* lr_a;
+    const float* lr_bw;
+    int lr_a_bytes, lr_tiles;
 #ifdef OSI_STAMPS
     unsigned long long* stamps;
 #endif
@@ -164,12 +167,12 @@
 
 constexpr int LDT = 64 + 4;
 
-template <bool LIVE = false>
-__device__ __forceinline__ void tile64_to_lds(float* tile, const f32x16& acc, int wm, int wn, int lane, int m0 = 0, int M = 0) {
+template <bool LIVE = false, bool SUB = false>
+__device__ __forceinline__ void tile64_to_lds(float* tile, const f32x16& acc, int wm, int wn, int lane, int m0 = 0, int M = 0, float sub = 0.f) {
 #pragma unroll
     for (int rr = 0; rr < 16; ++rr) {
         const bool live = !LIVE || m0 + wm * 32 + acc_row(rr, lane) < M;
-        tile[(wm * 32 + acc_row(rr, lane)) * LDT + wn * 32 + (lane & 31)] = live ? acc[rr] : 0.f;
+        tile[(wm * 32 + acc_row(rr, lane)) * LDT + wn * 32 + (lane & 31)] = live ? (SUB ? acc[rr] - sub : acc[rr]) : 0.f;
     }
 }
 __device__ __forceinline__ void tile64_to_slab(const ConvP& p, const float* tile, int mt, int nt, int ks) {
@@ -705,8 +708,9 @@
     }
 }
 
-template <int WM, int WN, int NST, int FUSED, bool KS = false, bool POOL = false, bool W3 = false>
+template <int WM, int WN, int NST, int FUSED, bool KS = false, bool POOL = false, bool W3 = false, bool LR = false>
 __global__ __launch_bounds__(256, NST == 1 ? (WM * WN >= 4 ? 3 : (WM * WN == 1 ? 8 : 4)) : 2) void k_conv_dgrad(ConvP p, int Hc0, int Wc0) {
+    static_assert(!LR || (WM == 1 && WN == 1 && NST == 1 && !KS && !POOL && !W3 && (FUSED == 0 || FUSED == 2)), "low-rank tail: the single-pass 64x64 tile");
     static_assert(!KS || (WM == 1 && WN == 1 && NST == 1), "the K-split tail is built for the single-buffered 64x64 tile");
     static_assert(!W3 || (WM == 1 && WN == 1 && NST == 1 && !POOL), "row windows: the single-buffered 64x64 tile");
     constexpr int BM = 64 * WM, BN = 64 * WN;
@@ -788,7 +792,8 @@
 #pragma unroll
             for (int r = 0; r < 16; ++r) acc[i][n][r] = 0.f;
 
-    const int KC = p.Cout / BK;
+    const int KC = p.Cout / BK + (LR ? p.lr_tiles : 0);
+    const int Kw = LR ? KC * BK : p.Cout;
     const int Tall = nR * nS * KC;
     const int t0 = (!KS || ks < 0) ? 0 : ks * p.ks_T;
     const int T = (!KS || ks < 0) ? Tall : min(Tall, t0 + p.ks_T);
@@ -800,6 +805,16 @@
     if constexpr (W3) prow = w3_prow(m0, wm, lane, Mc, dW);
     f32x4 ra[AR], rbv[BRN];
     const int bk_row = tid / BV, bk_col = (tid % BV) * 4;
+    bool ld_tail = false;
+    int ld_ct = 0;
+    float* s_sc = smem + NST * STAGE;
+    if constexpr (LR) {
+        if (p.in_scale)
+            for (int c = tid * 4; c < p.Cin; c += 1024) {
+                *reinterpret_cast<f32x4*>(s_sc + c) = ld4(p.in_scale + c);
+                *reinterpret_cast<f32x4*>(s_sc + p.Cin + c) = ld4(p.in_shift + c);
+            }
+    }
 
     auto gload = [&]() {
         const int r = rb + st * jr, s = sb + st * js;
@@ -813,6 +828,17 @@
                     ra[i] = bld4(rx, ok ? (uint32_t)((a_base[i] & ~15) + ((1 - jr) * p.W * p.Cout + c0) * 4) : OOB, 0);
                 }
             }
+        } else
+        if constexpr (LR) {
+            if (c0 == p.Cout) {
+#pragma unroll
+                for (int i = 0; i < AR; ++i) a_base[i] = a_base[i] >= 0 ? (a_base[i] >> 2) + kq * 12 : (int)OOB;
+                ld_tail = true;
+            }
+            ld_ct = c0 - p.Cout;
+            const __amdgpu_buffer_rsrc_t rc = make_rsrc(ld_tail ? p.lr_a : p.x, ld_tail ? p.lr_a_bytes : p.x_bytes);
+#pragma unroll
+            for (int i = 0; i < AR; ++i) ra[i] = bld4(rc, (uint32_t)a_base[i], (uint32_t)((ld_tail ? ld_ct : c0) * 4));
         } else
         if (p.unit) {
 #pragma unroll
@@ -834,7 +860,7 @@
             if (++js == 3) { js = 0; c0 += BK; if (c0 == p.Cout) { c0 = 0; ++jr; } }
         } else {
             c0 += BK;
-            if (c0 == p.Cout) { c0 = 0; if (++js == nS) { js = 0; ++jr; } }
+            if (c0 == Kw) { c0 = 0; if (++js == nS) { js = 0; ++jr; } }
         }
     };
     auto sstore = [&](int buf) {
@@ -846,9 +872,22 @@
                 for (int i = 0; i < AR; ++i)
                     if (lr + 32 * i < W3_WROWS) *reinterpret_cast<f32x4*>(sA + (lr + 32 * i) * LDR + kq * 4) = ra[i];
             }
-        } else
-#pragma unroll
-        for (int i = 0; i < AR; ++i) *reinterpret_cast<f32x4*>(sA + (lr + 32 * i) * LDR + kq * 4) = ra[i];
+        } else {
+            if constexpr (LR) {
+                if (ld_tail && p.in_scale) {
+                    const float* tb = s_sc + ld_ct + kq * 4;
+#pragma unroll
+                    for (int e = 0; e < 4; ++e) {
+                        const float sc = tb[e], sh = tb[p.Cin + e];
+#pragma unroll
+                        for (int i = 0; i < AR; ++i) ra[i][e] = osi_relu(__builtin_fmaf(ra[i][e], sc, sh));
+                        __builtin_amdgcn_sched_barrier(0);
+                    }
+                }
+            }
+#pragma unroll
+            for (int i = 0; i < AR; ++i) *reinterpret_cast<f32x4*>(sA + (lr + 32 * i) * LDR + kq * 4) = ra[i];
+        }
 #pragma unroll
         for (int i = 0; i < BRN; ++i) *reinterpret_cast<f32x4*>(sB + (bk_row + BRP * i) * LDC + bk_col) = rbv[i];
     };
@@ -893,6 +932,8 @@
     if constexpr (WM == 1 && WN == 1) {
         static_assert(BM * LDT <= STAGE, "transposed tile must fit the operand stage");
         float* tile = smem;
+        if constexpr (LR) tile64_to_lds<true, true>(tile, acc[0][0], wm, wn, lane, m0, Mc, p.lr_bw[n0 + wn * 32 + (lane & 31)]);
+        else
         tile64_to_lds<W3>(tile, acc[0][0], wm, wn, lane, m0, Mc);
         __syncthreads();
         if (KS && ks >= 0) {
@@ -1598,6 +1639,91 @@
     }
 }
 
+template <bool ACT>
+__global__ __launch_bounds__(256) void k_lr_gram(const float* a, int a_bytes, const float* sc, const float* sh, int M, int C, int kchunk, float* slab) {
+    constexpr int LD = 64 + 4;
+    __shared__ __attribute__((aligned(16))) float sI[BK * LD];
+    __shared__ __attribute__((aligned(16))) float sJ[BK * LD];
+    __shared__ f32x4 s_cs[16][16];
+    const int tid = threadIdx.x, lane = tid & 63, wave = tid >> 6, wm = wave >> 1, wn = wave & 1;
+    const int ct = C / 64, ti = blockIdx.x / ct, tj = blockIdx.x - ti * ct, split = blockIdx.y;
+    const bool same = ti == tj;
+    const int kbeg = split * kchunk, kend = min(M, kbeg + kchunk);
+    const int T = kend > kbeg ? (kend - kbeg + BK - 1) / BK : 0;
+    const int row = tid >> 4, c4 = (tid & 15) * 4;
+    const __amdgpu_buffer_rsrc_t ra = make_rsrc(a, a_bytes);
+    f32x4 isc = {1, 1, 1, 1}, ish = {0, 0, 0, 0}, jsc = isc, jsh = ish;
+    if (ACT) { isc = ld4(sc + ti * 64 + c4); ish = ld4(sh + ti * 64 + c4); jsc = ld4(sc + tj * 64 + c4); jsh = ld4(sh + tj * 64 + c4); }
+    f32x16 acc[1][1];
+#pragma unroll
+    for (int r = 0; r < 16; ++r) acc[0][0][r] = 0.f;
+    f32x4 vi[2], vj[2], cs = {0, 0, 0, 0};
+    auto gload = [&](int t) {
+#pragma unroll
+        for (int i = 0; i < 2; ++i) {
+            const int m = kbeg + t * BK + row + 16 * i;
+            const uint32_t off = m < kend ? (uint32_t)m * (uint32_t)(C * 4) : OOB;
+            vi[i] = bld4(ra, off, (uint32_t)((ti * 64 + c4) * 4));
+            if (!same) vj[i] = bld4(ra, off, (uint32_t)((tj * 64 + c4) * 4));
+        }
+    };
+    auto sstore = [&](int t) {
+#pragma unroll
+        for (int i = 0; i < 2; ++i) {
+            const bool ok = kbeg + t * BK + row + 16 * i < kend;
+            if (ACT) {
+#pragma unroll
+                for (int e = 0; e < 4; ++e) {
+                    vi[i][e] = ok ? osi_relu(__builtin_fmaf(vi[i][e], isc[e], ish[e])) : 0.f;
+                    if (!same) vj[i][e] = ok ? osi_relu(__builtin_fmaf(vj[i][e], jsc[e], jsh[e])) : 0.f;
+                }
+            }
+            cs += vi[i];
+            *reinterpret_cast<f32x4*>(sI + (row + 16 * i) * LD + c4) = vi[i];
+            if (!same) *reinterpret_cast<f32x4*>(sJ + (row + 16 * i) * LD + c4) = vj[i];
+        }
+    };
+    if (T > 0) {
+        gload(0);
+        sstore(0);
+        __syncthreads();
+        for (int t = 0; t < T; ++t) {
+            if (t + 1 < T) gload(t + 1);
+            mma_CC<1, 1, LD, LD>(sI, same ? sI : sJ, wm * 32, wn * 32, lane, acc);
+            __syncthreads();
+            if (t + 1 < T) sstore(t + 1);
+            __syncthreads();
+        }
+    }
+    float* out = slab + (size_t)split * (size_t)(C + 1) * C;
+#pragma unroll
+    for (int rr = 0; rr < 16; ++rr)
+        out[(size_t)(ti * 64 + wm * 32 + acc_row(rr, lane)) * C + tj * 64 + wn * 32 + (lane & 31)] = acc[0][0][rr];
+    if (tj == 0) {
+        s_cs[row][tid & 15] = cs;
+        __syncthreads();
+        if (row == 0) {
+            f32x4 v = s_cs[0][tid & 15];
+#pragma unroll
+            for (int k = 1; k < 16; ++k) v += s_cs[k][tid & 15];
+            *reinterpret_cast<f32x4*>(out + (size_t)C * C + ti * 64 + c4) = v;
+        }
+    }
+}
+__global__ __launch_bounds__(256) void k_lr_combine(float* dw, const float* w, const float* Ss, const float* alpha, const float* kappa,
+                                                    const float* beta, int Cin) {
+    extern __shared__ float s_w[];
+    const int n = blockIdx.x;
+    for (int j = threadIdx.x; j < Cin; j += 256) s_w[j] = w[(size_t)n * Cin + j];
+    __syncthreads();
+    const float al = alpha[n], ka = kappa[n], be = beta[n];
+    for (int c = threadIdx.x; c < Cin; c += 256) {
+        float ws = 0.f;
+        for (int j = 0; j < Cin; ++j) ws = __builtin_fmaf(s_w[j], Ss[(size_t)j * Cin + c], ws);
+        dw[(size_t)n * Cin + c] = al * dw[(size_t)n * Cin + c] - ka * ws - be * Ss[(size_t)Cin * Cin + c];
+    }
+}
+
 __global__ void k_stem_pack(const float* w, float* wp, int Cout) {
     int i = blockIdx.x * blockDim.x + threadIdx.x;
     if (i >= Cout * 224) return;
@@ -1727,7 +1853,7 @@
     return m == 2 || (d->Cin == 64 && (long)d->B * d->Ho * d->Wo >= 64L * 8 * hw_cus());
 }
 
-template <int WM, int WN, int NST, int FUSED, bool POOL = false, bool W3 = false, bool SPLIT = false>
+template <int WM, int WN, int NST, int FUSED, bool POOL = false, bool W3 = false, bool SPLIT = false, bool LR = false>
 static int launch_dgrad(ConvP p, hipStream_t st, const TailPlan* tp = nullptr, float* slab = nullptr) {
     constexpr int BM = 64 * WM, BN = 64 * WN;
     const int s = p.stride;
@@ -1742,10 +1868,11 @@
     p.MT = osi_cdiv((long)p.B * Hc * Wc, BM); p.NT = p.Cin / BN;
     size_t smem = 2 * (size_t)((W3 ? W3_WROWS : BM) * LDR + BK * (BN + 4)) * sizeof(float);
     smem = smem / 2 * NST;
+    if (LR) smem += (size_t)2 * p.Cin * sizeof(float);
     if (W3) p.cW[1] = make_fastdiv((uint32_t)p.W + 1);
-    if (int e = set_smem(k_conv_dgrad<WM, WN, NST, FUSED, SPLIT, POOL, W3>, smem)) return e;
+    if (int e = set_smem(k_conv_dgrad<WM, WN, NST, FUSED, SPLIT, POOL, W3, LR>, smem)) return e;
     const int grid = SPLIT ? set_tail_split(p, *tp, slab) : osi_cdiv(p.MT, 8) * 8 * p.NT;
-    hipLaunchKernelGGL((k_conv_dgrad<WM, WN, NST, FUSED, SPLIT, POOL, W3>), dim3(grid, s * s), dim3(256), smem, st, p, Hc, Wc);
+    hipLaunchKernelGGL((k_conv_dgrad<WM, WN, NST, FUSED, SPLIT, POOL, W3, LR>), dim3(grid, s * s), dim3(256), smem, st, p, Hc, Wc);
     OSI_LAUNCH_CHECK();
     if constexpr (SPLIT) {
         hipLaunchKernelGGL(k_conv_dgrad_tail_fixup<FUSED>, dim3(tp->tiles), dim3(256), 0, st, p);
@@ -2207,6 +2334,62 @@
     return conv_wgrad_impl(d, dy, x, dw, ws, ws_bytes, stream, in_scale, in_shift);
 }
 
+size_t osi_conv_lowrank_workspace(const osi_conv_desc* d) {
+    if (!desc_ok(d) || !lowrank_shape(d)) return 0;
+    return lowrank_layout(d).total * sizeof(float);
+}
+
+int osi_conv_dgrad_lowrank(const osi_conv_desc* d, const float* g, const float* a, const float* a_scale, const float* a_shift,
+                           const void* lr_ws, size_t lr_ws_bytes, float* dx, int accumulate, const osi_dgrad_fusion* f, int* P,
+                           osi_stream_t stream) {
+    OSI_REQUIRE(desc_ok(d) && lowrank_shape(d) && g && a && lr_ws && dx);
+    OSI_REQUIRE((a_scale == nullptr) == (a_shift == nullptr) && (accumulate == 0 || accumulate == 1));
+    const LowRankWs L = lowrank_layout(d);
+    OSI_REQUIRE(lr_ws_bytes >= L.total * sizeof(float));
+    const float* lw = (const float*)lr_ws;
+    ConvP p = make_p(d, DIR_DGRAD);
+    p.x = g; p.w = lw + L.wcat; p.y = dx;
+    p.w_bytes = (int)((size_t)(d->Cout + d->Cin) * d->Cin * 4);
+    p.lr_a = a; p.lr_a_bytes = (int)((size_t)p.M * d->Cin * 4); p.lr_bw = lw + L.bw; p.lr_tiles = d->Cin / BK;
+    p.in_scale = a_scale; p.in_shift = a_shift;
+    if (!f) {
+        p.addend = accumulate ? dx : nullptr;
+        return launch_dgrad<1, 1, 1, 0, false, false, false, true>(p, (hipStream_t)stream);
+    }
+    OSI_REQUIRE(!accumulate && f->scale0 && f->shift0 && f->y0 && !f->relu_mask && !f->y1 && !f->pool_idx && f->addend_stride <= 1);
+    p.escale0 = f->scale0; p.eshift0 = f->shift0; p.ey0 = f->y0;
+    if (f->partials) {
+        OSI_REQUIRE(P && f->mean0 && f->invstd0);
+        p.emean0 = f->mean0; p.einv0 = f->invstd0;
+        p.eP = osi_cdiv(p.M, 64);
+        OSI_REQUIRE(f->partials_bytes >= (size_t)3 * p.eP * d->Cin * sizeof(float));
+        p.esum = f->partials;
+        *P = p.eP;
+    }
+    return launch_dgrad<1, 1, 1, 2, false, false, false, true>(p, (hipStream_t)stream);
+}
+
+int osi_conv_wgrad_lowrank(const osi_conv_desc* d, const float* g, const float* a, const float* a_scale, const float* a_shift,
+                           const float* w, void* lr_ws, size_t lr_ws_bytes, float* dw, void* ws, size_t ws_bytes, osi_stream_t stream) {
+    OSI_REQUIRE(desc_ok(d) && lowrank_shape(d) && g && a && w && lr_ws && dw);
+    OSI_REQUIRE((a_scale == nullptr) == (a_shift == nullptr));
+    const LowRankWs L = lowrank_layout(d);
+    OSI_REQUIRE(lr_ws_bytes >= L.total * sizeof(float));
+    hipStream_t st = (hipStream_t)stream;
+    float* lw = (float*)lr_ws;
+    if (int e = conv_wgrad_impl(d, g, a, dw, ws, ws_bytes, stream, a_scale, a_shift)) return e;
+    const int C = d->Cin, M = d->B * d->H * d->W, ct = C / 64;
+    const int a_bytes = (int)((size_t)M * C * 4);
+    if (a_scale) hipLaunchKernelGGL(k_lr_gram<true>, dim3(ct * ct, L.splits), dim3(256), 0, st, a, a_bytes, a_scale, a_shift, M, C, L.kchunk, lw + L.slab);
+    else hipLaunchKernelGGL(k_lr_gram<false>, dim3(ct * ct, L.splits), dim3(256), 0, st, a, a_bytes, a_scale, a_shift, M, C, L.kchunk, lw + L.slab);
+    OSI_LAUNCH_CHECK();
+    const size_t n4 = (size_t)(C + 1) * C / 4;
+    if (int e = launch_slab_reduce(lw + L.slab, lw + L.Ss, n4, n4, L.splits, st)) return e;
+    hipLaunchKernelGGL(k_lr_combine, dim3(d->Cout), dim3(256), (size_t)C * sizeof(float), st, dw, w, lw + L.Ss, lw + L.alpha, lw + L.kappa, lw + L.beta, C);
+    OSI_LAUNCH_CHECK();
+    return OSI_OK;
+}
+
 int osi_stem_weight_pack(const float* w_krsc3, float* w_packed, int Cout, osi_stream_t stream) {
     OSI_REQUIRE(w_krsc3 && w_packed && Cout > 0);
     hipLaunchKernelGGL(k_stem_pack, dim3(osi_cdiv(Cout * 224, 256)), dim3(256), 0, (hipStream_t)stream, w_krsc3, w_packed, Cout);
diff --git a/openset-imagenet_amd/csrc/osi_common.h b/openset-imagenet_amd/csrc/osi_common.h
--- a/openset-imagenet_amd/csrc/osi_common.h
+++ b/openset-imagenet_amd/csrc/osi_common.h
@@ -47,7 +47,8 @@
     X(wgrad_wino, 1, 0, 1, 1)          \
     X(wino_wide, 1, 0, 1, 0)           \
     X(wino_streamk, 2, 0, 3, 0)        \
-    X(dp_reserved_cus, 0, 0, 128, 1)
+    X(dp_reserved_cus, 0, 0, 128, 1)   \
+    X(bn_lowrank, 1, 0, 2, 1)
 
 struct OsiTuning {
 #define OSI_KNOB_FIELD(name, def, lo, hi, plan) int name = def;
diff --git a/openset-imagenet_amd/csrc/resnet50_exec.hip b/openset-imagenet_amd/csrc/resnet50_exec.hip
--- a/openset-imagenet_amd/csrc/resnet50_exec.hip
+++ b/openset-imagenet_amd/csrc/resnet50_exec.hip
@@ -1,4 +1,4 @@
-#include "osi_common.h"
+#include "conv_common.h"
 #include <string>
 #include <vector>
 #include <cstring>
@@ -185,6 +185,17 @@
     float* dbet(float* grads, float* ws, const BN& b) const { return wants_grads(b.unit) ? grads + b.b_off : ws + b.dsink + b.C; }
     const float* dg_col(const float* ws, int col, int P, int C) const { return ws + dg_ws + (size_t)col * P * C; }
     bool stem_tail_fused() const { return !frozen && !rq.dimage && !rq.x_adv && stem_ws_bytes > 0; }
+    bool lowrank(const Block& k) const {
+        const int m = plan_knobs.bn_lowrank;
+        if (frozen || !m || (m == 1 && k.stage != 3)) return false;
+        size_t b = osi_conv_lowrank_workspace(&convs[k.c3].d);
+        if (k.ds >= 0) {
+            const size_t bd = osi_conv_lowrank_workspace(&convs[k.ds].d);
+            if (!bd) return false;
+            if (bd > b) b = bd;
+        }
+        return b > 0 && b <= scratch_floats * sizeof(float);
+    }
     bool eval_fused = true;
     bool stage_join = true;
     OsiTuning plan_knobs;
@@ -778,6 +789,52 @@
     return n->mark(OSI_PROF_BN_BWD, st);
 }
 
+static int bn_bwd_lowrank(osi_resnet50* n, int ci, const float* params, float* grads, float* ws, int lri, int which, hipStream_t st) {
+    Conv& c = n->convs[ci];
+    BN& b = n->bns[c.bn];
+    const int P = n->fused_P;
+    return osi_bn_backward_lowrank(&c.d, params + c.w_off, ws + b.mean, ws + b.invstd, params + b.g_off, n->dg_col(ws, 0, P, b.C),
+                                   n->dg_col(ws, 1 + which, P, b.C), P, n->dgam(grads, ws, b), n->dbet(grads, ws, b), ws + n->bn_ws, n->bn_ws_bytes,
+                                   ws + n->scratch[lri], n->scratch_floats * sizeof(float), st);
+}
+static int wgrad_lowrank(osi_resnet50* n, int ci, const float* params, float* grads, float* ws, int gi, int lri, const float* conv_in, int in_bn,
+                         hipStream_t st) {
+    Conv& c = n->convs[ci];
+    if (!n->wants_grads(c.unit)) return OSI_OK;
+    const bool async = n->async_wgrad();
+    hipStream_t ws_st = st;
+    if (async) {
+        OSI_TRY(n->fork_side(st));
+        ws_st = n->side;
+    }
+    OSI_TRY(osi_conv_wgrad_lowrank(&c.d, ws + n->scratch[gi], conv_in, in_bn >= 0 ? ws + n->bns[in_bn].scale : nullptr,
+                                   in_bn >= 0 ? ws + n->bns[in_bn].shift : nullptr, params + c.w_off,
+                                   ws + n->scratch[lri], n->scratch_floats * sizeof(float), grads + c.w_off, ws + n->wg_ws, n->wg_ws_bytes, ws_st));
+    if (async) {
+        const int held[2] = {gi, lri};
+        for (int i : held) {
+            if (hipEventRecord(n->buf_ev[i], n->side) != hipSuccess) return OSI_ERR_LAUNCH;
+            n->buf_pending[i] = true;
+        }
+        n->side_dirty = true;
+    }
+    return n->mark(OSI_PROF_CONV_WGRAD, ws_st);
+}
+static int dgrad_lowrank(osi_resnet50* n, int ci, int pc, float* ws, int gi, int lri, int dxi, hipStream_t st) {
+    Conv& c = n->convs[ci];
+    Conv& p0 = n->convs[pc];
+    BN& b0 = n->bns[p0.bn];
+    osi_dgrad_fusion f{};
+    f.scale0 = ws + b0.scale; f.shift0 = ws + b0.shift;
+    f.y0 = ws + p0.y; f.mean0 = ws + b0.mean; f.invstd0 = ws + b0.invstd;
+    f.partials = ws + n->dg_ws; f.partials_bytes = n->dg_ws_bytes;
+    int P = 0;
+    OSI_TRY(osi_conv_dgrad_lowrank(&c.d, ws + n->scratch[gi], ws + p0.y, ws + b0.scale, ws + b0.shift, ws + n->scratch[lri],
+                                   n->scratch_floats * sizeof(float), ws + n->scratch[dxi], 0, &f, &P, st));
+    n->fused_P = P;
+    return n->mark(OSI_PROF_CONV_DGRAD, st);
+}
+
 static int bn_bwd_fused_pair(osi_resnet50* n, int ci, int cj, const float* params, float* grads, float* ws, int gi, int dyi, int dyj,
                              hipStream_t st) {
     osi_bn_fused_consumer cs[2];
@@ -870,7 +927,7 @@
 }
 
 static int block_bwd_entry(osi_resnet50* n, const Block& k, const float* params, float* grads, float* ws, hipStream_t st, int* d3, int* t1,
-                           int* dxbase) {
+                           int* dxbase, int* gkeep) {
     const int go = n->cur_grad;
     const bool has_ds = k.ds >= 0;
     if (!n->go_fused) {
@@ -888,6 +945,12 @@
     }
     OSI_TRY(n->take(st, d3));
     if (n->frozen) OSI_TRY(bn_bwd_frozen(n, k.c3, k.ds, grads, ws, go, *d3, *t1, -1, false, st));
+    else if (n->lowrank(k)) {
+        OSI_TRY(bn_bwd_lowrank(n, k.c3, params, grads, ws, *d3, 0, st));
+        if (has_ds) OSI_TRY(bn_bwd_lowrank(n, k.ds, params, grads, ws, *t1, 1, st));
+        OSI_TRY(n->mark(OSI_PROF_BN_BWD, st));
+        if (has_ds) { *gkeep = go; return OSI_OK; }
+    }
     else if (has_ds) OSI_TRY(bn_bwd_fused_pair(n, k.c3, k.ds, params, grads, ws, go, *d3, *t1, st));
     else OSI_TRY(bn_bwd_fused(n, k.c3, params, grads, ws, go, *d3, 0, st));
     if (has_ds) n->give(go);
@@ -937,21 +1000,34 @@
     const Block& k = n->blocks[bi];
     Conv &c1 = n->convs[k.c1], &c2 = n->convs[k.c2];
     const float* x = ws + k.x_in;
-    int d3 = -1, t1 = -1, dxbase = -1, t2 = -1, t3 = -1;
-    OSI_TRY(block_bwd_entry(n, k, params, grads, ws, st, &d3, &t1, &dxbase));
+    int d3 = -1, t1 = -1, dxbase = -1, t2 = -1, t3 = -1, gkeep = -1;
+    const bool lr = n->go_fused && n->lowrank(k);
+    OSI_TRY(block_bwd_entry(n, k, params, grads, ws, st, &d3, &t1, &dxbase, &gkeep));
+    const int gi = gkeep >= 0 ? gkeep : dxbase;
     const bool ds_sparse = k.ds >= 0 && bi > 0 && n->convs[k.ds].d.stride == 2 && n->convs[k.ds].d.R == 1;
     if (k.ds >= 0) {
         Conv& cd = n->convs[k.ds];
-        OSI_TRY(wgrad(n, k.ds, grads, ws, t1, x, st));
+        if (lr) OSI_TRY(wgrad_lowrank(n, k.ds, params, grads, ws, gi, t1, x, -1, st));
+        else OSI_TRY(wgrad(n, k.ds, grads, ws, t1, x, st));
         if (!no_dx) {
             OSI_TRY(n->take(st, &dxbase));
+            if (lr) {
+                OSI_TRY(osi_conv_dgrad_lowrank(&cd.d, ws + n->scratch[gi], x, nullptr, nullptr, ws + n->scratch[t1], n->scratch_floats * sizeof(float),
+                                               ws + n->scratch[dxbase], 0, nullptr, nullptr, st));
+                OSI_TRY(n->mark(OSI_PROF_CONV_DGRAD, st));
+            } else
             OSI_TRY(dgrad_plain(n, &cd.d, ws + n->scratch[t1], params + cd.w_off, ws + n->scratch[dxbase], ds_sparse ? 2 : 0, st));
         }
         n->give(t1);
     }
-    OSI_TRY(wgrad(n, k.c3, grads, ws, d3, ws + c2.y, st, c2.bn));
+    if (lr) OSI_TRY(wgrad_lowrank(n, k.c3, params, grads, ws, gi, d3, ws + c2.y, c2.bn, st));
+    else OSI_TRY(wgrad(n, k.c3, grads, ws, d3, ws + c2.y, st, c2.bn));
     OSI_TRY(n->take(st, &t2));
-    OSI_TRY(dgrad_bn_inblock(n, k.c3, k.c2, params, grads, ws, d3, t2, st));
+    if (lr) {
+        OSI_TRY(dgrad_lowrank(n, k.c3, k.c2, ws, gi, d3, t2, st));
+        OSI_TRY(bn_bwd_fused(n, k.c2, params, grads, ws, t2, t2, 0, st));
+        if (gkeep >= 0) n->give(gkeep);
+    } else OSI_TRY(dgrad_bn_inblock(n, k.c3, k.c2, params, grads, ws, d3, t2, st));
     n->give(d3);
     OSI_TRY(wgrad(n, k.c2, grads, ws, t2, ws + c1.y, st, c1.bn));
     OSI_TRY(n->take(st, &t3));
diff --git a/openset-imagenet_amd/openset_imagenet/_native.py b/openset-imagenet_amd/openset_imagenet/_native.py
--- a/openset-imagenet_amd/openset_imagenet/_native.py
+++ b/openset-imagenet_amd/openset_imagenet/_native.py
@@ -266,6 +266,10 @@
     "osi_bn_frozen_coeffs_multi": (c_int, [POINTER(BnFrozenLayer), c_int, c_float, P]),
     "osi_conv_dgrad_fused_frozen": (c_int, [_PD, P, P, P, P, c_int, POINTER(c_int), P]),
     "osi_bn_backward_frozen": (c_int, [P, P, POINTER(BnFrozenConsumer), c_int, P, c_int, c_int, P, c_size_t, P]),
+    "osi_conv_lowrank_workspace": (c_size_t, [_PD]),
+    "osi_bn_backward_lowrank": (c_int, [_PD, P, P, P, P, P, P, c_int, P, P, P, c_size_t, P, c_size_t, P]),
+    "osi_conv_dgrad_lowrank": (c_int, [_PD, P, P, P, P, P, c_size_t, P, c_int, P, POINTER(c_int), P]),
+    "osi_conv_wgrad_lowrank": (c_int, [_PD, P, P, P, P, P, P, c_size_t, P, P, c_size_t, P]),
     "osi_bn_relu_maxpool_bwd_frozen": (c_int, [P, P, P, P, P, P, P, P, P, c_int, c_int, c_int, c_int, P, c_size_t, P]),
     "osi_resnet50_forward_frozen": (c_int, [c_void_p, P, P, P, P, P, P, P]),
     "osi_resnet50_backward": (c_int, [c_void_p, P, P, P, P, P, c_int, c_int, P]),
```
